# leggedrobotics/G-VOM

Hardware: AMD Instinct MI355X
Metric: M points/sec (process_pointcloud + combine_maps, 256^3 voxel grid); map Hz beside it (higher is better)
Workload: dtype int32 atomics + f32 ray state + f64 compares/maps; 1 GPU; 256x256x256 @0.2 m (metric grid), OS1-64 131,072-pt scan, buffer=1; buffer_size=1, poses=8, pose_motion=0.2 m per scan in +x (the window shifts every scan), input=device-resident f32 xyz, step=1 scan + 1 combine incl. the 4 maps in host memory, timing=2668 steps timed as one block after 5 warm-up steps

## Files before the change

### g-vom_amd/csrc/gvom_capi.hip

```cpp
#include "gvom_internal.h"
#include "gvom_ingest.h"
#include "../../include/gvom_hip.h"

#include <math.h>
#include <stdio.h>
#include <stdlib.h>
#include <string.h>
#include <time.h>
#include <unistd.h>
#include <immintrin.h>
#include <algorithm>
#include <atomic>
#include <mutex>
#include <string>
#include <vector>

#define VIS __attribute__((visibility("default")))

namespace {

struct Buf {
    void *p = nullptr;
    size_t bytes = 0;
    uint64_t gen = 0;
};

struct Slot {
    int32_t *state = nullptr;
    uint16_t *code16 = nullptr;
    uint32_t *tags = nullptr;
    uint32_t epoch = 0;
    Buf crows;
    Buf metrics, base, rowvox;
    int64_t origin[3] = {0, 0, 0};
    int64_t count = 0;
    bool filled = false;
    bool has_code16 = false;
    bool has_metrics = false;
    bool stats_valid = false;
    gvom_scan_stats stats = {0, 0, 0, 0};
};

struct Fused {
    int32_t *state = nullptr;
    uint32_t *tags = nullptr;
    uint32_t epoch = 0;
    Buf rows;
    Buf metrics;
    int64_t origin[3] = {0, 0, 0};
    int64_t count = 0;
    bool valid = false;
    bool has_metrics = false;
};

struct DevSet {
    char *mem = nullptr;
    size_t bytes = 0;
    int device = 0, xy = 0;
    int kind = 0, zs = 0;
    int64_t cap = 0;
    hipEvent_t ready = nullptr;
    int64_t id = -1;
    int exports = 0;
    std::vector<hipStream_t> rel_streams;
    std::vector<hipEvent_t> rel, rel_spare;
    bool orphan = false;
};
#define GVOM_MAX_DEVICE_SETS 8
#define GVOM_N_PRODUCT_KINDS 4
std::mutex g_set_mu;

struct DLDevice { int32_t device_type; int32_t device_id; };
struct DLDataType { uint8_t code; uint8_t bits; uint16_t lanes; };
struct DLTensor { void *data; DLDevice device; int32_t ndim; DLDataType dtype; int64_t *shape; int64_t *strides; uint64_t byte_offset; };
struct DLManagedTensor { DLTensor dl_tensor; void *manager_ctx; void (*deleter)(DLManagedTensor *); };
struct DLPackVersion { uint32_t major; uint32_t minor; };
struct DLManagedTensorVersioned { DLPackVersion version; void *manager_ctx; void (*deleter)(DLManagedTensorVersioned *); uint64_t flags; DLTensor dl_tensor; };
enum { kDLInt = 0, kDLUInt = 1, kDLFloat = 2, kDLROCM = 10 };

}

struct gvom_handle {
    gvom_params prm;
    int device = 0;
    int rank = 0, world = 1;
    bool sharded = false;
    int sy_lo = 0, sy_hi = 0;
    size_t V = 0, slabV = 0, cells2d = 0, ntiles = 0;
    int nseg = 1;
    uint32_t epoch = 0;
    hipStream_t stream = nullptr;
    std::mutex mu;
    std::mutex scan_mu;
    std::string err;

    uint32_t *hit = nullptr, *total = nullptr, *mh = nullptr;
    size_t acc_elems = 0;
    int tune_segs = 0, tune_ep_row = -2, tune_period = 0;
    int tune_prio = -1;
    int tune_ilv = 0;
    int last_knobs[5] = {0, 0, 0, 0, 1};
    int64_t last_n = -1;
    uint32_t probe_var_age = 0;
    int64_t probe_n = -1; uint32_t probe_age = 0;
    int tune_fuse1 = 0;
    int tune_flag_kernel = 0;
    int tune_churn = 0;
    uint64_t alloc_gen = 0;
    uint64_t handle_gen = 0;
    bool exported = false;
    bool holds_pooled = false;
    std::vector<Buf> retired;
    uint64_t fixed_gen[3] = {0, 0, 0};
    uint32_t *x_send_ids = nullptr, *x_recv_ids = nullptr;
    void *x_send_pay = nullptr, *x_recv_pay = nullptr;
    Buf x_send_eps, x_recv_eps;
    int64_t x_ep_cap = 0;
    std::vector<int64_t> x_recv_ep_off;
    uint32_t *x_qcnt = nullptr, *x_ecnt = nullptr, *x_spcnt = nullptr;
    unsigned long long *x_host = nullptr, *x_host_dev = nullptr;
    Buf x_send_sp, x_recv_sp;
    std::vector<int64_t> x_recv_sp_off;
    int pending_dtype = 0;
    size_t x_Q = 0, x_myQ = 0;
    ScanParams pending_P;
    unsigned resident_blocks = 2048;
    bool f32_sqrt = false;
    std::vector<Slot> slots;
    std::vector<int> ring;
    int staging = 0;
    int buffer_index = 0, last_buffer_index = 0;
    Buf in_pts, world_pts[2];
    uint32_t *counters = nullptr;
    uint32_t *counters_host = nullptr;
    uint32_t *counters_host_dev = nullptr;

    bool pending = false;
    bool pending_any = false;
    int64_t pending_origin[3] = {0, 0, 0};
    int64_t pending_n = 0;

    Fused fused[2];
    int cur = 0;
    bool has_combined = false;
    int64_t combined_cell_count = 0;
    MapDesc *descs_dev = nullptr, *descs_host = nullptr;
    uint32_t *blockcounts = nullptr;
    int fuse_blocks = 0;
    int cnt_blocks = 0;
    double *hmaps2 = nullptr;
    uint32_t *blockcounts2 = nullptr;
    bool spec_valid = false;
    int spec_nxt = 0, spec_slot = 0, spec_blocks = 0;
    uint32_t spec_epoch = 0;
    int64_t spec_origin[3] = {0, 0, 0};
    bool spec_has_metrics = false;
    Buf flink[2];
    bool fs_reads[2] = {false, false};
    FuseParams spec_FP;
    FuseDescs spec_KD;
    int tune_dirsort = 0;
    Buf dir_keys, dir_perm;
    uint32_t *dir_hist = nullptr;
    uint32_t dir_flip = 0;
    int last_dirsort = 0;
    int tune_encfuse = 0;
    int tune_fastdiv = -1;
    int fastdiv_ok = 0;
    int tune_eager = -1;
    int eager_waste = 0;
    int eager_stat[2] = {0, 0};
    int last_fuse = 0;
    bool last_scan_spec = false;
    bool solo_encoded = false;
    bool fresh_scan = false;

    double *hmaps = nullptr;
    double *height = nullptr, *inferred = nullptr;
    int hs = 0;
    double *slope_x = nullptr, *slope_y = nullptr, *rough = nullptr, *guessed = nullptr;
    hipStream_t own_stream = nullptr;
    hipStream_t stream_b = nullptr;
    hipStream_t stream_up = nullptr;
    hipEvent_t ev_up = nullptr;
    hipStream_t stream_s = nullptr;
    hipEvent_t ev_enc_s = nullptr, ev_fz_s = nullptr, ev_sdone = nullptr, ev_fsdone = nullptr;
    hipEvent_t ev_before[2] = {nullptr, nullptr};
    bool before_valid[2] = {false, false};
    uint32_t stats_scan = 0;
    bool stats_prev_committed = true;
    bool s_pending = false, fs_pending = false;
    hipEvent_t ev_fused = nullptr, ev_mapped = nullptr, ev_done = nullptr;
    std::mutex combine_mu;
    bool pending_combine = false;
    uint32_t combine_seq = 0;
    double last_wait_ns[2] = {0.0, 0.0};
    bool mapped_unjoined = false;
    hipEvent_t ev_fuse_b = nullptr;
    bool fuse_b_unjoined = false;
    uint64_t fuse_b_slots = 0;
    bool scan_inflight = false;
    std::vector<void *> out_bufs;
    void *last_checked_out = nullptr;
    void *out_host = nullptr;
    char *out_host_dev = nullptr;
    uint32_t scan_seq = 0;
    bool ev_scan = false, ev_fuse = false, ev_map = false;
    bool maps_valid = false;

    double ego[3] = {0, 0, 0};
    int in_off[3] = {0, 1, 2};
    bool in_f32 = false;

    Buf tl;
    int tl_grid[2] = {0, 0};
    double host_ns[8] = {0, 0, 0, 0, 0, 0, 0, 0};
    long host_calls = 0;
    bool host_timing = false;
    bool stats = false;
    bool stats_auto = false;
    int stats_idle = 0;
    bool stats_release = false;
    int acc_pad = 7, sxq = 0;
    bool profiling = false;
    hipEvent_t ev[8] = {nullptr};
    float stage_ms[GVOM_N_STAGES] = {0, 0, 0, 0, 0};
    std::vector<DevSet *> dsets;
    int64_t dset_seq = 0;
    std::vector<DevSet *> psets;
    int64_t pset_seq = 0;
    int tune_occ_clear = 0;
    bool count_pending = false;
    hipEvent_t ev_dcount = nullptr;
    Buf ri_model, ri_raw, ri_poses;
    void *ri_poses_pin = nullptr;
    size_t ri_poses_pin_bytes = 0;
    int32_t ri_H = 0, ri_W = 0;
    double ri_scale = 0.0, ri_min = 0.0, ri_max = 0.0;
};

namespace {

inline double now_ns() { timespec t; clock_gettime(CLOCK_MONOTONIC, &t); return t.tv_sec * 1e9 + t.tv_nsec; }
#define HT(h, slot, t0) do { if ((h)->host_timing) { double n_ = now_ns(); (h)->host_ns[slot] += n_ - (t0); (t0) = n_; } } while (0)

#define HIPCHK(h, call)                                                                         \
    do {                                                                                        \
        hipError_t e_ = (call);                                                                 \
        if (e_ != hipSuccess) {                                                                 \
            char b_[512];                                                                       \
            snprintf(b_, sizeof b_, "%s failed: %s (%s:%d)", #call, hipGetErrorString(e_),      \
                     __FILE__, __LINE__);                                                       \
            (h)->err = b_;                                                                      \
            return GVOM_ERR_HIP;                                                                \
        }                                                                                       \
    } while (0)

static std::atomic<uint64_t> g_alloc_generation{0};

inline size_t exportable_size(size_t bytes) { const size_t g = (size_t)2 << 20; return ((bytes ? bytes : 1) + g - 1) / g * g; }

#define GVOM_POOL_WARN_BYTES ((size_t)16 << 30)
struct ExportPool {
    std::mutex m;
    std::vector<Buf> v;
    size_t bytes = 0;
    bool warned = false;
};
static ExportPool g_pool;
void pool_put(void *p, size_t bytes, uint64_t gen)
{
    if (!p) return;
    std::lock_guard<std::mutex> lk(g_pool.m);
    Buf b; b.p = p; b.bytes = bytes; b.gen = gen;
    g_pool.v.push_back(b);
    g_pool.bytes += bytes;
    if (g_pool.bytes > GVOM_POOL_WARN_BYTES && !g_pool.warned) {
        g_pool.warned = true;
        fprintf(stderr, "libgvom_hip: %zu MiB of device memory that other processes may have mapped are parked (never freed while "
                        "the process lives; re-used by later sharded handles of the same sizes): create fewer exported handles per process\n",
                g_pool.bytes >> 20);
    }
}
hipError_t pool_get(size_t bytes, void **p, uint64_t *gen, bool *reused = nullptr)
{
    {
        std::lock_guard<std::mutex> lk(g_pool.m);
        for (size_t k = 0; k < g_pool.v.size(); ++k)
            if (g_pool.v[k].bytes == bytes) {
                *p = g_pool.v[k].p; *gen = g_pool.v[k].gen;
                if (reused) *reused = true;
                g_pool.bytes -= bytes;
                g_pool.v.erase(g_pool.v.begin() + (long)k);
                return hipSuccess;
            }
    }
    *gen = ++g_alloc_generation;
    return hipMalloc(p, bytes);
}

int ensure(gvom_handle *h, Buf &b, size_t bytes)
{
    if (b.bytes >= bytes) return GVOM_OK;
    size_t want = bytes + bytes / 2 + 256;
    const bool exported = &b == &h->x_send_eps || &b == &h->x_send_sp;
    if (exported) want = exportable_size(want);
    if (b.p && exported) { h->retired.push_back(b); b.p = nullptr; }
    if (b.p) HIPCHK(h, hipFree(b.p));
    b.p = nullptr; b.bytes = 0;
    if (exported) HIPCHK(h, pool_get(want, &b.p, &b.gen, &h->holds_pooled));
    else { HIPCHK(h, hipMalloc(&b.p, want)); b.gen = ++g_alloc_generation; }
    b.bytes = want;
    if (&b == &h->x_send_eps || &b == &h->x_send_sp) h->alloc_gen = b.gen;
    return GVOM_OK;
}

int ensure_keep(gvom_handle *h, Buf &b, size_t bytes)
{
    if (b.bytes >= bytes) return GVOM_OK;
    const size_t want = bytes + bytes / 2 + 256;
    void *np = nullptr;
// ... 43 lines not shown
    P.sy_lo = h->sy_lo; P.sy_hi = h->sy_hi;
    P.off[0] = h->in_off[0]; P.off[1] = h->in_off[1]; P.off[2] = h->in_off[2];
    P.in_f32 = h->in_f32 ? 1 : 0;
    P.nseg = h->nseg;
    {
        auto lg = [](int v) { int k = 0; while ((1 << k) < v) ++k; return (1 << k) == v ? k : -1; };
        P.lg_nseg = lg(h->nseg); P.lg_zs = lg(p.z_size);
        if (P.lg_nseg < 0 || P.lg_zs < 0) P.lg_nseg = P.lg_zs = -1;
    }
    P.sxq = h->sxq;
    P.shard_world = h->world; P.shard_rank = h->rank; P.shard_rows = h->world > 1 ? p.xy_size / h->world : p.xy_size;
    P.stat_e = p.xy_eigen_dist;
    {
        const int maxsteps = (p.xy_size > p.z_size ? p.xy_size : p.z_size) / 2 + 2;
        const bool many = n_points / 64 > 3 * (int64_t)h->resident_blocks;
        int nsegs = many ? 3 : 5;
        if (h->tune_segs > 0) nsegs = h->tune_segs;
        if (nsegs > 9) nsegs = 9;
        if (nsegs > maxsteps / 8) nsegs = maxsteps / 8 > 0 ? maxsteps / 8 : 1;
        P.nsegs = nsegs;
        P.lc_period = h->tune_period > 0 ? h->tune_period : (many ? 12 : 16);
        if (P.lc_period > 32) P.lc_period = 32;
        P.ep_row = h->tune_ep_row >= -1 ? h->tune_ep_row : (many ? -1 : 0);
        if (P.ep_row > P.nsegs) P.ep_row = P.nsegs;
        P.prio_div = h->tune_prio >= 0 ? h->tune_prio : 8;
        P.f32_sqrt = h->f32_sqrt ? 1 : 0;
        P.ilv_lg = 0; P.ilv_len = n_points;
        {
            int K = h->tune_ilv > 1 ? h->tune_ilv : 1;
            if (h->tune_ilv == 0 && h->counters_host) {
                const unsigned long long w = *(volatile unsigned long long *)(h->counters_host + 8);
                if ((int64_t)(w >> 8) == n_points) K = 1 << (int)(w & 7ull);
            }
            if (K > 64 || (K & (K - 1)) != 0 || n_points <= 0 || n_points % K != 0) K = 1;
            while ((1 << P.ilv_lg) < K) ++P.ilv_lg;
            P.ilv_len = n_points / K;
            if (K > 1 && h->tune_period <= 0) P.lc_period = 24;
        }
        P.dbg = gvom_diag_env("GVOM_TRACE_DEBUG");
        const double w_last = nsegs <= 3 ? 0.35 : 0.6;
        const double unit = nsegs >= 3 ? (double)maxsteps / ((nsegs - 2) + 0.85 + w_last) : (double)maxsteps / nsegs;
        double acc = 0.0;
        for (int k = 0; k < 10; ++k) {
            P.seg_start[k] = (int)(acc + 0.5);
            acc += (nsegs < 3 || k < nsegs - 2) ? unit : (k == nsegs - 2 ? 0.85 * unit : (k == nsegs - 1 ? w_last * unit : unit));
        }
    }
    P.epoch = 0;
}

__attribute__((target("fma"))) static bool verify_fastdiv_all(double d, double r)
{
    for (uint32_t m = 0; m < (1u << 23); ++m) {
        const uint32_t bits = 0x3f800000u | m;
        float xf;
        memcpy(&xf, &bits, 4);
        const double x = (double)xf;
        const double q = x * r;
        const double e = __builtin_fma(-q, d, x);
        const double q2 = __builtin_fma(e, r, q);
        if (q2 != x / d) return false;
    }
    return true;
}
static bool verify_fastdiv(double d)
{
    static std::mutex mu;
    static std::vector<std::pair<double, bool>> known;
    if (!(d > 0x1p-64 && d < 0x1p64)) return false;
    if (!__builtin_cpu_supports("fma")) return false;
    std::lock_guard<std::mutex> lk(mu);
    for (const auto &k : known) if (k.first == d) return k.second;
    const bool ok = verify_fastdiv_all(d, 1.0 / d);
    known.emplace_back(d, ok);
    return ok;
}

int create_impl(const gvom_params *params, int device_id, int rank, int world, bool sharded, gvom_t **out)
{
    if (!params || !out) return GVOM_ERR_INVALID;
    *out = nullptr;
    if (params->xy_size <= 0 || params->z_size <= 0 || params->buffer_size <= 0 ||
        !(params->xy_resolution > 0) || !(params->z_resolution > 0) || world <= 0 || rank < 0 ||
        rank >= world)
        return GVOM_ERR_INVALID;
    if (params->buffer_size >= GVOM_MAX_SLOTS || params->z_size > 1024 || world > GVOM_MAX_SLOTS) return GVOM_ERR_CAPACITY;
    if (sharded && params->xy_size % (4 * world) != 0) return GVOM_ERR_INVALID;
    const double Vd = (double)params->xy_size * params->xy_size * params->z_size;
    if (Vd >= 2147483648.0) return GVOM_ERR_CAPACITY;
    int ndev = 0;
    if (hipGetDeviceCount(&ndev) != hipSuccess || ndev <= 0 || device_id < 0 || device_id >= ndev)
        return GVOM_ERR_NO_DEVICE;
    gvom_handle *h = new gvom_handle();
    h->alloc_gen = h->handle_gen = ++g_alloc_generation;
    h->prm = *params;
    h->device = device_id;
    h->rank = rank; h->world = world; h->sharded = sharded;
    h->stats = (params->reserved0 & GVOM_FLAG_VOXEL_STATISTICS) != 0;
    h->stats_auto = !h->stats && !sharded && (params->reserved0 & GVOM_FLAG_STATISTICS_ON_DEMAND) != 0;
    if (h->stats_auto) h->stats = true;
    h->f32_sqrt = (params->reserved0 & GVOM_FLAG_CUDA_F32_SQRT) != 0;
    h->fastdiv_ok = (verify_fastdiv(params->xy_resolution) ? 1 : 0) | (verify_fastdiv(params->z_resolution) ? 2 : 0);
    if (const char *v = getenv("GVOM_VOXEL_STATISTICS")) { h->stats = atoi(v) != 0; h->stats_auto = false; }
    if (sharded && h->stats && world > 1 && 2 * params->xy_eigen_dist + 1 > params->xy_size / world) { delete h; return GVOM_ERR_INVALID; }
    if (const char *v = getenv("GVOM_HOST_TIMING")) h->host_timing = atoi(v) != 0;
    const int xy = params->xy_size, zs = params->z_size;
    h->sy_lo = (int)((int64_t)xy * rank / world);
    h->sy_hi = (int)((int64_t)xy * (rank + 1) / world);
    h->V = (size_t)xy * xy * zs;
    h->slabV = (size_t)(h->sy_hi - h->sy_lo) * xy * zs;
    h->cells2d = (size_t)xy * xy;
    h->nseg = (xy + 63) / 64;
    h->ntiles = (size_t)xy * zs * h->nseg;
#define CK(call)                                                                                \
    do {                                                                                        \
        hipError_t e_ = (call);                                                                 \
        if (e_ != hipSuccess) {                                                                 \
            fprintf(stderr, "gvom_create: %s failed: %s\n", #call, hipGetErrorString(e_));      \
            gvom_destroy(h);                                                                    \
            return GVOM_ERR_HIP;                                                                \
        }                                                                                       \
    } while (0)
    CK(hipSetDevice(device_id));
    CK(hipStreamCreateWithFlags(&h->stream, hipStreamNonBlocking));
    h->own_stream = h->stream;
    {
        int lo = 0, hi = 0;
        CK(hipDeviceGetStreamPriorityRange(&lo, &hi));
        CK(hipStreamCreateWithPriority(&h->stream_b, hipStreamNonBlocking, hi));
    }
    CK(hipEventCreateWithFlags(&h->ev_fused, hipEventDisableTiming));
    CK(hipEventCreateWithFlags(&h->ev_mapped, hipEventDisableTiming));
    CK(hipEventCreateWithFlags(&h->ev_done, hipEventDisableTiming));
    CK(hipEventCreateWithFlags(&h->ev_fuse_b, hipEventDisableTiming));
    CK(hipStreamCreateWithFlags(&h->stream_up, hipStreamNonBlocking));
    CK(hipStreamCreateWithFlags(&h->stream_s, hipStreamNonBlocking));
    for (hipEvent_t *e : {&h->ev_enc_s, &h->ev_fz_s, &h->ev_sdone, &h->ev_fsdone, &h->ev_before[0], &h->ev_before[1]})
        CK(hipEventCreateWithFlags(e, hipEventDisableTiming));
    CK(hipEventCreateWithFlags(&h->ev_up, hipEventDisableTiming));
    h->sxq = (xy + 3) / 4 + h->acc_pad;
    const size_t acc_elems = (size_t)h->sxq * ((xy + 3) / 4) * zs * 16 + 256;
    h->acc_elems = acc_elems;
    CK(hipMalloc((void **)&h->hit, acc_elems * 4));
    CK(hipMalloc((void **)&h->total, acc_elems * 4));
    CK(hipMalloc((void **)&h->mh, acc_elems * 4));
    CK(hipMemsetAsync(h->hit, 0, acc_elems * 4, h->stream));
    CK(hipMemsetAsync(h->total, 0, acc_elems * 4, h->stream));
    CK(hipMemsetAsync(h->mh, 0, acc_elems * 4, h->stream));
    {
        hipDeviceProp_t pr;
        CK(hipGetDeviceProperties(&pr, device_id));
        h->resident_blocks = (unsigned)pr.multiProcessorCount * 8u;
    }
    h->slots.resize(params->buffer_size + 1);
    for (auto &s : h->slots) {
        CK(hipMalloc((void **)&s.state, h->V * 4));
        if ((params->xy_size & 3) == 0) CK(hipMalloc((void **)&s.code16, h->V * 2));
        CK(hipMalloc((void **)&s.tags, h->ntiles * 4));
        CK(hipMemsetAsync(s.tags, 0, h->ntiles * 4, h->stream));
    }
    h->ring.resize(params->buffer_size);
    for (int i = 0; i < params->buffer_size; ++i) h->ring[i] = i;
    h->staging = params->buffer_size;
    for (int k = 0; k < 2; ++k) {
        CK(hipMalloc((void **)&h->fused[k].state, h->V * 4));
        CK(hipMalloc((void **)&h->fused[k].tags, h->ntiles * 4));
        CK(hipMemsetAsync(h->fused[k].tags, 0, h->ntiles * 4, h->stream));
    }
    CK(hipMalloc((void **)&h->dir_hist, 3 * GVOM_DIRBINS * 4));
    CK(hipMemsetAsync(h->dir_hist, 0, 3 * GVOM_DIRBINS * 4, h->stream));
    CK(hipMalloc((void **)&h->counters, GVOM_CNT_WORDS * 4));
    CK(hipHostMalloc((void **)&h->counters_host, 64, hipHostMallocMapped | hipHostMallocCoherent));
    CK(hipHostGetDevicePointer((void **)&h->counters_host_dev, h->counters_host, 0));
    memset(h->counters_host, 0, 64);
    CK(hipMemsetAsync(h->counters, 0, GVOM_CNT_WORDS * 4, h->stream));
    CK(hipMalloc((void **)&h->descs_dev, sizeof(MapDesc) * (GVOM_MAX_SLOTS + 1)));
    CK(hipHostMalloc((void **)&h->descs_host, sizeof(MapDesc) * (GVOM_MAX_SLOTS + 1)));
    h->fuse_blocks = ((xy + 63) / 64) * (h->sy_hi - h->sy_lo);
    CK(hipMalloc((void **)&h->blockcounts, (size_t)(h->fuse_blocks > 0 ? h->fuse_blocks : 1) * 4));
    CK(hipMemsetAsync(h->blockcounts, 0, (size_t)(h->fuse_blocks > 0 ? h->fuse_blocks : 1) * 4, h->stream));
    h->cnt_blocks = h->fuse_blocks;
    if (!sharded && params->buffer_size == 1 && xy % 16 == 0 && zs >= 4) {
        CK(hipMalloc((void **)&h->blockcounts2, (size_t)(h->fuse_blocks > 0 ? h->fuse_blocks : 1) * 4));
        CK(hipMemsetAsync(h->blockcounts2, 0, (size_t)(h->fuse_blocks > 0 ? h->fuse_blocks : 1) * 4, h->stream));
        CK(hipMalloc((void **)&h->hmaps2, h->cells2d * 24));
    }
    h->hs = 3 * xy;
    if (sharded) CK(pool_get(exportable_size(h->cells2d * 24), (void **)&h->hmaps, &h->fixed_gen[2], &h->holds_pooled));
    else CK(hipMalloc((void **)&h->hmaps, h->cells2d * 24));
    h->height = h->hmaps; h->inferred = h->hmaps + xy;
    double **maps[4] = {&h->slope_x, &h->slope_y, &h->rough, &h->guessed};
    for (auto m : maps) CK(hipMalloc((void **)m, h->cells2d * 8));

    CK(hipHostMalloc(&h->out_host, h->cells2d * 20, hipHostMallocMapped | hipHostMallocCoherent));
    CK(hipHostGetDevicePointer((void **)&h->out_host_dev, h->out_host, 0));
    if (sharded) {
        h->x_Q = (size_t)(xy / 4) * zs * h->nseg;
        h->x_myQ = h->x_Q / world;
        CK(pool_get(exportable_size(h->x_Q * 4), (void **)&h->x_send_ids, &h->fixed_gen[0], &h->holds_pooled));
        CK(pool_get(exportable_size(h->x_Q * 1024), &h->x_send_pay, &h->fixed_gen[1], &h->holds_pooled));
        CK(hipMalloc((void **)&h->x_recv_ids, h->x_Q * 4));
        CK(hipMalloc(&h->x_recv_pay, h->x_Q * 1024));
        CK(hipMalloc((void **)&h->x_qcnt, (size_t)world * 64));
        CK(hipMalloc((void **)&h->x_ecnt, (size_t)world * 64));
        CK(hipMalloc((void **)&h->x_spcnt, (size_t)world * 64));
        CK(hipMemsetAsync(h->x_qcnt, 0, (size_t)world * 64, h->stream));
        CK(hipMemsetAsync(h->x_ecnt, 0, (size_t)world * 64, h->stream));
        CK(hipMemsetAsync(h->x_spcnt, 0, (size_t)world * 64, h->stream));
        CK(hipHostMalloc((void **)&h->x_host, (size_t)(3 * world + 2) * 8, hipHostMallocMapped | hipHostMallocCoherent));
        CK(hipHostGetDevicePointer((void **)&h->x_host_dev, h->x_host, 0));
        memset(h->x_host, 0, (size_t)(3 * world + 2) * 8);
        h->x_recv_ep_off.assign(world + 1, 0);
        h->x_recv_sp_off.assign(world + 1, 0);
    }
    for (auto &e : h->ev) CK(hipEventCreate(&e));
    CK(hipStreamSynchronize(h->stream));
#undef CK
    *out = h;
    return GVOM_OK;
}

static void stats_demand(gvom_handle *h)
{
    h->stats_idle = 0;
    if (h->stats_auto && !h->stats) { h->stats = true; h->stats_release = false; }
}

static void release_statistics_buffers(gvom_handle *h)
{
    h->stats_release = false;
    (void)hipStreamSynchronize(h->stream_s);
    h->s_pending = h->fs_pending = false;
    h->before_valid[0] = h->before_valid[1] = false;
    auto fb = [](Buf &b) { if (b.p) (void)hipFree(b.p); b.p = nullptr; b.bytes = 0; };
    for (auto &sl : h->slots) { fb(sl.metrics); fb(sl.base); fb(sl.rowvox); sl.has_metrics = false; }
    for (int k = 0; k < 2; ++k) { fb(h->fused[k].metrics); h->fused[k].has_metrics = false; }
    fb(h->world_pts[0]); fb(h->world_pts[1]); fb(h->flink[0]); fb(h->flink[1]);
    h->spec_has_metrics = false;
}

void scan_abort(gvom_handle *h)
{
    (void)hipMemsetAsync(h->hit, 0, h->acc_elems * 4, h->stream);
    (void)hipMemsetAsync(h->total, 0, h->acc_elems * 4, h->stream);
    (void)hipMemsetAsync(h->mh, 0, h->acc_elems * 4, h->stream);
    (void)hipMemsetAsync(h->counters, 0, GVOM_CNT_WORDS * 4, h->stream);
    if (h->stream_s) (void)hipStreamSynchronize(h->stream_s);
    h->s_pending = h->fs_pending = false;
    h->before_valid[0] = h->before_valid[1] = false;
    (void)hipStreamSynchronize(h->stream);
    (void)hipGetLastError();
    h->pending = false;
    h->scan_inflight = false;
}

int renumber_epochs(gvom_handle *h);

hipError_t sync_streams(gvom_handle *h)
{
    if (h->mapped_unjoined || h->fuse_b_unjoined) {
        hipError_t e = hipStreamSynchronize(h->stream_b);
        if (e != hipSuccess) return e;
        h->mapped_unjoined = false;
        h->fuse_b_unjoined = false;
    }
    if (h->s_pending || h->fs_pending) {
        hipError_t e = hipStreamSynchronize(h->stream_s);
        if (e != hipSuccess) return e;
        h->s_pending = h->fs_pending = false;
        h->before_valid[0] = h->before_valid[1] = false;
    }
    return hipStreamSynchronize(h->stream);
}
hipError_t join_fuse_stream(gvom_handle *h)
{
    if (!h->fuse_b_unjoined) return hipSuccess;
    h->fuse_b_unjoined = false;
    return hipStreamWaitEvent(h->stream, h->ev_fuse_b, 0);
}
hipError_t join_map_stream(gvom_handle *h)
{
    if (!h->mapped_unjoined) return hipSuccess;
    h->mapped_unjoined = false;
    h->fuse_b_unjoined = false;
    return hipStreamWaitEvent(h->stream, h->ev_mapped, 0);
}

hipError_t join_second_stream(gvom_handle *h)
{
    hipError_t e = join_map_stream(h);
    if (e == hipSuccess) e = join_fuse_stream(h);
    if (e == hipSuccess && h->s_pending) e = hipStreamWaitEvent(h->stream, h->ev_sdone, 0);
    return e;
}

int enqueue_scan_stats(gvom_handle *h, const ScanParams &P, int dtype, Slot &st, int64_t n, int64_t nrows, const void *extra, int64_t n_extra)
{
    const uint32_t par = h->stats_scan & 1u;
    HIPCHK(h, hipEventRecord(h->ev_before[par], h->stream_s));
    h->before_valid[par] = true;
    ++h->stats_scan;
    HIPCHK(h, hipEventRecord(h->ev_enc_s, h->stream));
    HIPCHK(h, hipStreamWaitEvent(h->stream_s, h->ev_enc_s, 0));
    HIPCHK(h, gvom_launch_stats(h->stream_s, P, dtype, h->world_pts[par].p, n, st.state, st.tags,
                                h->prm.xy_eigen_dist, h->prm.z_eigen_dist, (double *)st.base.p, (double *)st.metrics.p,
                                (const uint32_t *)st.rowvox.p, nrows, extra, n_extra));
    HIPCHK(h, hipEventRecord(h->ev_sdone, h->stream_s));
    h->s_pending = true;
    return GVOM_OK;
}

bool wait_published(gvom_handle *h, std::unique_lock<std::mutex> &lk, volatile unsigned long long *flag, uint32_t seq,
                    bool high_half, double *last_ns)
{
    auto done = [&]() { return (uint32_t)(high_half ? (*flag >> 32) : *flag) == seq; };
    lk.unlock();
    const double start = now_ns();
    bool slept = false;
    if (last_ns && *last_ns > 6.0e5 && !done()) {
        const double margin = *last_ns * 0.2 > 2.5e5 ? *last_ns * 0.2 : 2.5e5;
        usleep((useconds_t)((*last_ns - margin) * 1e-3));
        slept = true;
    }
    const bool overslept = slept && done();
    unsigned spins = 0;
    bool ok = true;
    while (!done()) {
        _mm_pause();
        if ((++spins & 0x3ff) == 0) {
            const double waited = now_ns() - start;
            if (waited > 2.0e9) { ok = false; break; }
            if (waited > 2.0e7) usleep(50);
        }
    }
    if (last_ns) {
        const double est = overslept ? *last_ns * 0.5 : now_ns() - start;
        *last_ns = est < 2.0e7 ? est : 2.0e7;
    }
    lk.lock();
    return ok;
}

void fill_fuse_frame(const gvom_handle *h, const int64_t origin[3], FuseParams &P)
{
    const gvom_params &p = h->prm;
    memset(&P, 0, sizeof P);
    P.xy = p.xy_size; P.zs = p.z_size;
    P.om[0] = (int)floor_mod(origin[0], p.xy_size);
    P.om[1] = (int)floor_mod(origin[1], p.xy_size);
    P.om[2] = (int)floor_mod(origin[2], p.z_size);
    P.sy_lo = h->sy_lo; P.sy_hi = h->sy_hi;
    P.nseg = h->nseg;
    P.hs = h->hs;
    for (int k = 0; k < 3; ++k) { P.origin[k] = (double)origin[k]; P.ego[k] = h->ego[k]; }
    P.xy_res = p.xy_resolution; P.z_res = p.z_resolution;
    P.radius2 = p.robot_radius * p.robot_radius;
    P.ground_to_lidar_height = p.ground_to_lidar_height;
}

int eager_launch(gvom_handle *h, const ScanParams &P, Slot &st, const int64_t origin[3], uint32_t seq)
{
    const gvom_params &p = h->prm;
    const int nxt = h->has_combined ? 1 - h->cur : 0;
    Fused &F = h->fused[nxt];
    const Fused *prev = (h->has_combined && h->fused[h->cur].valid) ? &h->fused[h->cur] : nullptr;
    FuseParams FP;
    fill_fuse_frame(h, origin, FP);
    FP.nslots = 1; FP.has_prev = prev ? 1 : 0;
    FP.nz = h->tune_encfuse & 15; FP.cpw = (h->tune_encfuse >> 4) & 1;
    MapDesc pd;
    memset(&pd, 0, sizeof pd);
    if (prev) {
        pd.state = prev->state; pd.rows = (const uint4 *)prev->rows.p;
        pd.d[0] = clamp_delta(origin[0] - prev->origin[0], p.xy_size);
        pd.d[1] = clamp_delta(origin[1] - prev->origin[1], p.xy_size);
        pd.d[2] = clamp_delta(origin[2] - prev->origin[2], p.z_size);
        pd.epoch = prev->epoch; pd.tags = prev->tags;
    }
    int nw, nblocks; size_t row_cap;
    gvom_encfuse_shape(p.xy_size, p.z_size, FP.nz, &nw, &nblocks, &row_cap);
    if (row_cap >= 2147483648ull) { h->err = "fused row space exceeds 31 bits"; return GVOM_ERR_CAPACITY; }
    int rc;
    if ((rc = ensure(h, F.rows, row_cap * 16))) return rc;
    F.valid = false;
    FP.epoch = ++h->epoch;
    if (h->fs_pending && h->fs_reads[nxt]) HIPCHK(h, hipStreamWaitEvent(h->stream, h->ev_fsdone, 0));
    h->spec_has_metrics = false;
    int32_t *flink = nullptr;
    if (h->stats) {
        if ((rc = ensure(h, h->flink[nxt], row_cap * 4))) return rc;
        flink = (int32_t *)h->flink[nxt].p;
        if ((rc = ensure(h, F.metrics, row_cap * 40))) return rc;
        h->spec_FP = FP;
        memset(&h->spec_KD, 0, sizeof h->spec_KD);
        MapDesc &sd = h->spec_KD.d[0];
        sd.state = st.state; sd.rows = (const uint4 *)st.crows.p; sd.epoch = st.epoch; sd.tags = st.tags; sd.metrics = st.metrics.p;
        if (prev) { h->spec_KD.d[1] = pd; h->spec_KD.d[1].metrics = prev->has_metrics ? prev->metrics.p : nullptr; h->spec_KD.d[1].link = flink; }
        h->spec_has_metrics = true;
    }
    HIPCHK(h, gvom_launch_encfuse(h->stream, P, FP, pd, flink, h->hit, h->total, h->mh, st.state, (uint4 *)st.crows.p, st.tags,
                                  F.state, (uint4 *)F.rows.p, F.tags, h->blockcounts2, h->hmaps2, h->hmaps2 + p.xy_size,
                                  h->counters, (unsigned long long *)h->counters_host_dev, seq));
    h->spec_valid = true; h->spec_nxt = nxt; h->spec_slot = h->staging; h->spec_blocks = nblocks; h->spec_epoch = FP.epoch;
    h->spec_origin[0] = origin[0]; h->spec_origin[1] = origin[1]; h->spec_origin[2] = origin[2];
    h->last_scan_spec = true;
    return GVOM_OK;
}

int scan_launch(gvom_handle *h, std::unique_lock<std::mutex> &lk, const void *dev_pts, int64_t n, int64_t stride_elems,
                int dtype, const double *tf, bool shard_local = false)
{
    const gvom_params &p = h->prm;
    int64_t origin[3];
    origin[0] = (int64_t)floor((h->ego[0] / p.xy_resolution) - p.xy_size / 2.0);
    origin[1] = (int64_t)floor((h->ego[1] / p.xy_resolution) - p.xy_size / 2.0);
    origin[2] = (int64_t)floor((h->ego[2] / p.z_resolution) - p.z_size / 2.0);
    int rc;
    if (h->epoch >= 0xFFFFFF00u && (rc = renumber_epochs(h))) return rc;
    ScanParams P;
    fill_scan_params(h, origin, tf, P, n);
    if (h->pending_combine && h->tune_prio < 0) P.prio_div = 0;
    h->last_knobs[0] = P.nsegs; h->last_knobs[1] = P.lc_period; h->last_knobs[2] = P.ep_row; h->last_knobs[3] = P.prio_div;
    h->last_knobs[4] = 1 << P.ilv_lg;
    Slot &st = h->slots[h->staging];
    if (h->fuse_b_unjoined && ((h->fuse_b_slots >> h->staging) & 1ull)) HIPCHK(h, join_fuse_stream(h));
    st.epoch = ++h->epoch;
    P.epoch = st.epoch;
    st.has_metrics = h->stats;
    h->scan_inflight = true;
    const size_t esz = dtype == GVOM_DTYPE_F32 ? 4 : 8;
    const size_t cap = std::max<size_t>(1, (size_t)n);
    if ((rc = ensure(h, st.crows, cap * 16))) return rc;
    Buf &wpts = h->world_pts[h->stats_scan & 1u];
    const size_t scap = h->sharded ? 2 * cap : cap;
    if (h->stats && ((rc = ensure(h, wpts, (size_t)(n > 0 ? n : 1) * 3 * esz)) || (rc = ensure(h, st.metrics, scap * 80)) ||
                     (rc = ensure(h, st.base, scap * 8 * GVOM_BASE_PITCH)) || (rc = ensure(h, st.rowvox, scap * 4)))) return rc;
    double t0 = now_ns();
    const uint32_t seq = ++h->scan_seq;
    if (h->profiling) HIPCHK(h, hipEventRecord(h->ev[0], h->stream));
    bool big = false;
    for (int k = 0; k < 3; ++k)
        if (origin[k] >= (1ll << 30) || origin[k] <= -(1ll << 30)) big = true;
    if (h->stats) {
        const uint32_t prev_par = (h->stats_scan + 1u) & 1u;
        if (!h->stats_prev_committed && h->s_pending) HIPCHK(h, hipStreamWaitEvent(h->stream, h->ev_sdone, 0));
        else if (h->before_valid[prev_par]) {
            if (hipEventQuery(h->ev_before[prev_par]) == hipSuccess) h->before_valid[prev_par] = false;
            else { (void)hipGetLastError(); HIPCHK(h, hipStreamWaitEvent(h->stream, h->ev_before[prev_par], 0)); }
        }
        HIPCHK(h, hipMemsetAsync(st.rowvox.p, 0xFF, st.rowvox.bytes, h->stream));
    }
    ShardExchange X;
    X.ep_send = nullptr; X.ep_cnt = nullptr; X.ep_cap = 0; X.sp_send = nullptr; X.sp_cnt = nullptr;
    if (h->sharded) {
#ifdef GVOM_HOOKS
        if (h->tune_churn > 0 && h->x_send_eps.p) {
            h->retired.push_back(h->x_send_eps);
            h->x_send_eps.p = nullptr; h->x_send_eps.bytes = 0;
        }
#endif
        if ((rc = ensure(h, h->x_send_eps, (size_t)h->world * (size_t)(n > 0 ? n : 1) * 8))) return rc;
        h->x_ep_cap = n > 0 ? n : 1;
        X.ep_send = (uint2 *)h->x_send_eps.p; X.ep_cnt = h->x_ecnt; X.ep_cap = (long)h->x_ep_cap;
        if (h->stats && h->world > 1) {
            if ((rc = ensure(h, h->x_send_sp, (size_t)h->world * (size_t)h->x_ep_cap * 3 * esz))) return rc;
            X.sp_send = h->x_send_sp.p; X.sp_cnt = h->x_spcnt;
        }
    }
    P.tl = nullptr; P.tl_words = 0;
#ifdef GVOM_DIAG
    if (gvom_diag_env("GVOM_TRACE_TIMELINE") && n > 0) {
        h->tl_grid[0] = (int)((n + 511) / 512); h->tl_grid[1] = P.nsegs + (P.ep_row >= 0 ? 1 : 0);
        P.prof_on = gvom_diag_env("GVOM_TRACE_STEPPROF");
        const size_t bytes = (size_t)h->tl_grid[0] * h->tl_grid[1] * 8 * 32 + 64 + ((size_t)h->tl_grid[0] * h->tl_grid[1] * 8 / 64 + 1) * 1024;
        P.tl_words = (long)h->tl_grid[0] * h->tl_grid[1] * 8 * 4;
        if ((rc = ensure(h, h->tl, bytes))) return rc;
        HIPCHK(h, hipMemsetAsync(h->tl.p, 0, bytes, h->stream));
        P.tl = (unsigned long long *)h->tl.p;
    }
#endif
    hipError_t le = hipSuccess;
    const unsigned long long probe_word = h->counters_host ? *(volatile unsigned long long *)(h->counters_host + 8) : 0ull;
    if (h->tune_ilv == 0 && n >= 8192) {
        const bool stable = n == h->last_n && (n != h->probe_n || ++h->probe_age >= 32);
        const bool varying = n != h->last_n && ++h->probe_var_age >= 8;
        if (stable || varying) {
            if (stable) { h->probe_n = n; h->probe_age = 0; }
            h->probe_var_age = 0;
            le = gvom_launch_layout_probe(h->stream, P, dtype, dev_pts, stride_elems, n, 2, (unsigned long long *)(h->counters_host_dev + 8));
            if (le != hipSuccess) { scan_abort(h); HIPCHK(h, le); }
        }
        h->last_n = n;
    }
    P.perm = nullptr;
    {
        int sort = h->tune_dirsort == 1 || h->tune_dirsort == 2 ? h->tune_dirsort : 0;
        if (h->tune_dirsort == 0 && h->tune_ilv == 0 && h->counters_host) {
            const unsigned long long w = probe_word;
            const int64_t np_ = (int64_t)(w >> 8);
            if (np_ > 0 && (np_ == n || (n > np_ - np_ / 4 && n < np_ + np_ / 4))) sort = (int)((w >> 3) & 3ull);
        }
        h->last_dirsort = 0;
        if (sort && n >= 256 && n < (1ll << 31)) {
            if ((rc = ensure(h, h->dir_keys, (size_t)n * 2)) || (rc = ensure(h, h->dir_perm, (size_t)n * 4))) return rc;
            uint32_t *hist = h->dir_hist + (h->dir_flip & 1u) * GVOM_DIRBINS, *next = h->dir_hist + ((h->dir_flip + 1u) & 1u) * GVOM_DIRBINS;
            ++h->dir_flip;
            le = gvom_launch_dirbin(h->stream, P, sort == 2 ? 2 : 1, dtype, dev_pts, stride_elems, n, (uint16_t *)h->dir_keys.p, hist, next,
                                    h->dir_hist + 2 * GVOM_DIRBINS, (uint32_t *)h->dir_perm.p);
            if (le != hipSuccess) { scan_abort(h); HIPCHK(h, le); }
            P.perm = (const uint32_t *)h->dir_perm.p;
            P.ilv_lg = 0; P.ilv_len = n;
            h->last_dirsort = sort == 2 ? 2 : 1;
            h->last_knobs[4] = 1;
        }
    }
    le = gvom_launch_trace(h->stream, P, X, dtype, big, dev_pts, stride_elems, n,
                                      h->stats ? wpts.p : nullptr, h->hit, h->total, h->mh, st.state,
                                      st.tags, h->counters, h->stats ? (double *)st.metrics.p : nullptr,
                                      h->stats ? (double *)st.base.p : nullptr,
                                      h->stats ? (uint32_t *)st.rowvox.p : nullptr);
    if (le != hipSuccess) { scan_abort(h); HIPCHK(h, le); }
    if (h->profiling) HIPCHK(h, hipEventRecord(h->ev[1], h->stream));
    const bool solo = shard_local && h->world == 1;
    h->solo_encoded = solo;
    if (shard_local && !solo) {
        le = gvom_launch_pack(h->stream, P, h->total, st.tags, h->x_send_ids, h->x_send_pay, h->x_qcnt, h->x_ecnt, h->x_spcnt,
                              h->counters, h->x_host_dev, seq);
        if (le != hipSuccess) { scan_abort(h); HIPCHK(h, le); }
        volatile unsigned long long *flag = (volatile unsigned long long *)(h->x_host + 2 * h->world + 1);
        if (!wait_published(h, lk, flag, seq, false, &h->last_wait_ns[0])) {
            hipError_t se = hipStreamSynchronize(h->stream);
            if (se != hipSuccess || (uint32_t)*flag != seq) {
                scan_abort(h);
                h->err = "sharded scan: pack counts were never published";
                return GVOM_ERR_HIP;
            }
        }
        h->pending_any = h->x_host[2 * h->world] != 0;
        h->pending_P = P;
        h->pending_dtype = dtype;
        st.count = -1;
        st.origin[0] = origin[0]; st.origin[1] = origin[1]; st.origin[2] = origin[2];
        st.stats_valid = false;
        st.stats.points = n;
        h->pending = true;
        h->pending_n = n;
        return GVOM_OK;
    }
    const bool eager = h->hmaps2 && h->tune_eager != 0 && (h->tune_eager == 1 || h->eager_waste < 3) && !gvom_diag_env("GVOM_TRACE_DEBUG");
    h->last_scan_spec = false;
    if (eager) {
        if ((rc = eager_launch(h, P, st, origin, seq))) { scan_abort(h); return rc; }
        st.has_code16 = false;
    } else {
        const bool codes = st.code16 && (p.buffer_size > 1 || h->tune_fuse1 == 1 || h->sharded);
        le = gvom_launch_encode(h->stream, P, h->hit, h->total, h->mh, st.state, codes ? st.code16 : nullptr, (uint4 *)st.crows.p,
                                st.tags, h->counters,
                                (unsigned long long *)h->counters_host_dev, seq, h->resident_blocks);
        if (le != hipSuccess) { scan_abort(h); HIPCHK(h, le); }
        st.has_code16 = codes;
    }
    if (h->profiling) { HIPCHK(h, hipEventRecord(h->ev[2], h->stream)); h->ev_scan = true; }
    if (h->stats && (rc = enqueue_scan_stats(h, P, dtype, st, n, n, nullptr, 0))) return rc;
    if (eager && h->spec_has_metrics) {
        Fused &F = h->fused[h->spec_nxt];
        HIPCHK(h, gvom_launch_fuse_stats(h->stream_s, h->spec_FP, h->spec_KD, nullptr, F.state, F.tags, (float *)F.metrics.p));
        HIPCHK(h, hipEventRecord(h->ev_fsdone, h->stream_s));
        HIPCHK(h, hipEventRecord(h->ev_sdone, h->stream_s));
        h->s_pending = h->fs_pending = true;
        h->fs_reads[h->spec_nxt] = true; h->fs_reads[1 - h->spec_nxt] = false;
    }
    HT(h, 0, t0);
    {
        volatile unsigned long long *flag = (volatile unsigned long long *)h->counters_host;
        if (!wait_published(h, lk, flag, seq, true, &h->last_wait_ns[0])) {
            hipError_t se = hipStreamSynchronize(h->stream);
            if (se != hipSuccess || (uint32_t)(*flag >> 32) != seq) {
                scan_abort(h);
                h->err = se != hipSuccess ? std::string("scan failed: ") + hipGetErrorString(se)
                                          : "scan completion was never published";
                return GVOM_ERR_HIP;
            }
        }
    }
    HT(h, 1, t0);
    if (h->host_timing) h->host_calls++;
    {
        const unsigned long long fl = *(volatile unsigned long long *)h->counters_host;
        h->pending_any = (fl & 0x80000000ull) != 0;
    }
    st.count = -1;
    st.origin[0] = origin[0]; st.origin[1] = origin[1]; st.origin[2] = origin[2];
    st.stats_valid = false;
    st.stats.points = n;
    h->pending = true;
    h->pending_n = n;
    return GVOM_OK;
}

void scan_commit(gvom_handle *h, bool accept)
{
    h->scan_inflight = false;
    if (!h->pending) return;
    h->pending = false;
    h->stats_prev_committed = accept;
    if (!accept) { h->spec_valid = false; h->last_scan_spec = false; return; }
    const int b = h->buffer_index;
    const int old = h->ring[b];
    h->ring[b] = h->staging;
    h->staging = old;
    h->slots[h->ring[b]].filled = true;
    h->fresh_scan = true;
    h->slots[old].filled = false;
    h->last_buffer_index = b;
    h->buffer_index = (b + 1 >= h->prm.buffer_size) ? 0 : b + 1;
}

int renumber_epochs(gvom_handle *h)
{
    HIPCHK(h, sync_streams(h));
    h->spec_valid = false;
    uint32_t next = 0;
    for (size_t k = 0; k < h->slots.size(); ++k) {
        Slot &sl = h->slots[k];
        const bool inflight = (int)k == h->staging && (h->scan_inflight || h->pending);
        const uint32_t fresh = (sl.filled || inflight) ? ++next : 0u;
        HIPCHK(h, gvom_launch_retag(h->stream, sl.tags, h->ntiles, sl.epoch, fresh));
        sl.epoch = fresh;
        if (inflight) h->pending_P.epoch = fresh;
    }
    for (int k = 0; k < 2; ++k) {
        Fused &f = h->fused[k];
        const uint32_t fresh = f.valid ? ++next : 0u;
        HIPCHK(h, gvom_launch_retag(h->stream, f.tags, h->ntiles, f.epoch, fresh));
        f.epoch = fresh;
    }
    h->epoch = next;
    HIPCHK(h, sync_streams(h));
    return GVOM_OK;
}

int scan_begin(gvom_handle *h, const double ego[3], const int64_t *off_bytes, size_t esz, bool widen_f32, bool defer, int64_t n)
{
    HIPCHK(h, hipSetDevice(h->device));
    for (int k = 0; k < 3; ++k) h->in_off[k] = off_bytes ? (int)(off_bytes[k] / (int64_t)esz) : k;
    h->in_f32 = widen_f32;
    h->ego[0] = ego[0]; h->ego[1] = ego[1]; h->ego[2] = ego[2];
    if (h->pending && h->sharded) scan_abort(h);
    h->pending = false;
    if (h->spec_valid) {
        h->spec_valid = false;
        if (h->eager_waste < 4) ++h->eager_waste;
        ++h->eager_stat[1];
    }
    if (h->sharded && !defer) { h->err = "a sharded handle scans through gvom_shard_scan_local / gvom_shard_scan_merge"; return GVOM_ERR_INVALID; }
    if (n == 0 && !defer) return GVOM_EMPTY_CLOUD;
    return GVOM_OK;
}

struct Upload { void *dst; const void *src; size_t bytes; };
int scan_upload(gvom_handle *h, std::unique_lock<std::mutex> &lk, const Upload *up, int count)
{
    if (hipStreamQuery(h->stream) == hipErrorNotReady) {
        lk.unlock();
        hipError_t ue = hipSuccess;
        for (int k = 0; k < count && ue == hipSuccess; ++k)
            ue = hipMemcpyAsync(up[k].dst, up[k].src, up[k].bytes, hipMemcpyHostToDevice, h->stream_up);
        lk.lock();
        HIPCHK(h, ue);
        HIPCHK(h, hipEventRecord(h->ev_up, h->stream_up));
        HIPCHK(h, hipStreamWaitEvent(h->stream, h->ev_up, 0));
    } else {
        (void)hipGetLastError();
        for (int k = 0; k < count; ++k)
            HIPCHK(h, hipMemcpyAsync(up[k].dst, up[k].src, up[k].bytes, hipMemcpyHostToDevice, h->stream));
    }
    return GVOM_OK;
}

int scan_finish(gvom_handle *h, std::unique_lock<std::mutex> &lk, const void *dev, int64_t n, int64_t stride_elems, int dtype,
                const double *tf, bool defer)
{
    int rc = scan_launch(h, lk, dev, n, stride_elems, dtype, tf, defer);
    if (rc) return rc;
    if (defer) return GVOM_OK;
    const bool accept = h->pending_any;
    scan_commit(h, accept);
    return accept ? GVOM_OK : GVOM_NO_OVERLAP;
}

int process_impl(gvom_handle *h, const void *xyz, bool on_device, int64_t n, int64_t row_stride_bytes,
                 int dtype, const double ego[3], const double *tf, bool defer, const int64_t *off_bytes = nullptr,
                 bool widen_f32 = false)
{
    if (!h || !ego || n < 0 || (dtype != GVOM_DTYPE_F32 && dtype != GVOM_DTYPE_F64))
        return GVOM_ERR_INVALID;
    const size_t esz = (dtype == GVOM_DTYPE_F32 || widen_f32) ? 4 : 8;
    if (widen_f32 && dtype != GVOM_DTYPE_F64) return GVOM_ERR_INVALID;
    if (n > 0 && (!xyz || row_stride_bytes < (int64_t)(3 * esz) || row_stride_bytes % esz != 0))
        return GVOM_ERR_INVALID;
    if (n >= 2147483647LL) return GVOM_ERR_CAPACITY;
    int64_t last_field = 2 * (int64_t)esz;
    if (off_bytes) {
        last_field = 0;
        for (int k = 0; k < 3; ++k) {
            if (off_bytes[k] < 0 || off_bytes[k] % (int64_t)esz != 0 || off_bytes[k] + (int64_t)esz > row_stride_bytes)
                return GVOM_ERR_INVALID;
            if (off_bytes[k] > last_field) last_field = off_bytes[k];
        }
    }
    std::lock_guard<std::mutex> scan_lk(h->scan_mu);
    std::unique_lock<std::mutex> lk(h->mu);
    int rc = scan_begin(h, ego, off_bytes, esz, widen_f32, defer, n);
    if (rc) return rc;
    const void *dev = xyz;
    if (!on_device && n > 0) {
        if ((rc = ensure(h, h->in_pts, (size_t)n * row_stride_bytes))) return rc;
        const Upload up = {h->in_pts.p, xyz, (size_t)(n - 1) * row_stride_bytes + (size_t)last_field + esz};
        if ((rc = scan_upload(h, lk, &up, 1))) return rc;
        dev = h->in_pts.p;
    }
    return scan_finish(h, lk, dev, n, row_stride_bytes / (int64_t)esz, dtype, tf, defer);
}

int range_image_impl(gvom_handle *h, const void *raw, bool on_device, int range_dtype, int64_t row_stride_bytes,
                     const double *col_poses, int cloud_dtype, const double ego[3], const double *tf)
{
    if (!h || !ego || !raw || (cloud_dtype != GVOM_DTYPE_F32 && cloud_dtype != GVOM_DTYPE_F64)) return GVOM_ERR_INVALID;
    if (range_dtype != GVOM_RANGE_U16 && range_dtype != GVOM_RANGE_U32 && range_dtype != GVOM_RANGE_F32) return GVOM_ERR_INVALID;
    const int64_t rsz = range_dtype == GVOM_RANGE_U16 ? 2 : 4;
    std::lock_guard<std::mutex> scan_lk(h->scan_mu);
    std::unique_lock<std::mutex> lk(h->mu);
    if (h->sharded) { h->err = "range images are not supported on a sharded handle"; return GVOM_ERR_INVALID; }
    if (h->ri_H <= 0) { h->err = "gvom_process_range_image: no sensor model (gvom_sensor_model_set)"; return GVOM_ERR_INVALID; }
    const int64_t H = h->ri_H, W = h->ri_W, n = H * W;
    if (row_stride_bytes < W * rsz || row_stride_bytes % rsz != 0) { h->err = "gvom_process_range_image: bad row stride"; return GVOM_ERR_INVALID; }
    int rc = scan_begin(h, ego, nullptr, 0, false, false, n);
    if (rc) return rc;
    const size_t tsz = cloud_dtype == GVOM_DTYPE_F32 ? 4 : 8;
    if ((rc = ensure(h, h->in_pts, (size_t)n * 3 * tsz))) return rc;
    Upload up[2];
    int ups = 0;
    if (col_poses) {
        const size_t bytes = (size_t)W * 96;
        if ((rc = ensure(h, h->ri_poses, bytes))) return rc;
        if (h->ri_poses_pin_bytes < bytes) {
            if (h->ri_poses_pin) HIPCHK(h, hipHostFree(h->ri_poses_pin));
            h->ri_poses_pin = nullptr; h->ri_poses_pin_bytes = 0;
            HIPCHK(h, hipHostMalloc(&h->ri_poses_pin, bytes + bytes / 2, hipHostMallocDefault));
            h->ri_poses_pin_bytes = bytes + bytes / 2;
        }
        memcpy(h->ri_poses_pin, col_poses, bytes);
        up[ups++] = {h->ri_poses.p, h->ri_poses_pin, bytes};
    }
    if (!on_device) {
        const size_t bytes = (size_t)(H - 1) * row_stride_bytes + (size_t)(W * rsz);
        if ((rc = ensure(h, h->ri_raw, bytes))) return rc;
        up[ups++] = {h->ri_raw.p, raw, bytes};
    }
    if (ups && (rc = scan_upload(h, lk, up, ups))) return rc;
    UnprojectParams U;
    U.raw = on_device ? raw : h->ri_raw.p; U.row_stride = row_stride_bytes;
    U.dir = (const double *)h->ri_model.p; U.off = U.dir + (size_t)n * 3;
    U.poses = col_poses ? (const double *)h->ri_poses.p : nullptr;
    U.out = h->in_pts.p;
    U.scale = h->ri_scale; U.min_range = h->ri_min; U.max_range = h->ri_max;
    U.W = (uint32_t)W; U.n = (uint32_t)n;
    HIPCHK(h, gvom_launch_unproject(h->stream, U, range_dtype, cloud_dtype));
    return scan_finish(h, lk, h->in_pts.p, n, 3, cloud_dtype, tf, false);
}

int choose_nz(int zs, int *zc, int *cpw)
{
    int nchunks = (zs + 15) / 16;
    if (nchunks < 1) nchunks = 1;
    if (nchunks > 16) nchunks = 16;
    *zc = (zs + nchunks - 1) / nchunks;
    nchunks = (zs + *zc - 1) / *zc;
    int want_waves = 4;
    *cpw = (nchunks + want_waves - 1) / want_waves;
// ... 153 lines not shown
    const size_t n2 = h->cells2d;
    int32_t *o_pos = (int32_t *)out_dev, *o_neg = o_pos + n2, *o_vis = o_neg + n2;
    double *o_rgh = (double *)(o_vis + n2);
    if (dev_set) {
        const size_t S = dev_map_stride(p.xy_size);
        P.out_dev = 1;
        o_rgh = (double *)out_dev;
        o_pos = (int32_t *)(o_rgh + 6 * S); o_neg = o_pos + S; o_vis = o_neg + S;
    }
    if (h->profiling) HIPCHK(h, hipEventRecord(h->ev[6], ms));
    HIPCHK(h, gvom_launch_map2d(ms, P, F.state, F.tags, (const uint4 *)F.rows.p,
                                h->height, h->inferred, h->slope_x,
                                h->slope_y, h->rough, h->guessed, o_pos, o_neg, o_rgh, o_vis,
                                h->blockcounts, h->cnt_blocks,
                                publish ? (unsigned long long *)(h->counters_host_dev + 2) : nullptr));
    if (h->profiling) { HIPCHK(h, hipEventRecord(h->ev[7], ms)); h->ev_map = true; }
    h->maps_valid = true;
    return GVOM_OK;
}

int posdens_impl(gvom_handle *h)
{
    const gvom_params &p = h->prm;
    const Fused &F = h->fused[h->cur];
    Map2dParams P;
    memset(&P, 0, sizeof P);
    P.xy = p.xy_size; P.zs = p.z_size;
    P.om[2] = (int)floor_mod(F.origin[2], p.z_size);
    P.y_lo = h->sy_lo; P.y_hi = h->sy_hi;
    P.origin_z = (double)F.origin[2];
    P.z_res = p.z_resolution;
    P.pos_thr = p.positive_obstacle_threshold; P.robot_height = p.robot_height;
    P.nseg = h->nseg; P.hs = h->hs; P.epoch = F.epoch;
    HIPCHK(h, gvom_launch_posdens(h->stream, P, F.state, F.tags, (const uint4 *)F.rows.p,
                                  h->hmaps, h->blockcounts, h->fuse_blocks,
                                  (unsigned long long *)(h->counters_host_dev + 2),
                                  (unsigned long long *)(h->counters + 10)));
    return GVOM_OK;
}

void collect_stage_ms(gvom_handle *h)
{
    if (h->ev_scan) {
        hipEventElapsedTime(&h->stage_ms[0], h->ev[0], h->ev[1]);
        hipEventElapsedTime(&h->stage_ms[1], h->ev[1], h->ev[2]);
        h->stage_ms[2] = 0.0f;
    }
    if (h->ev_fuse) hipEventElapsedTime(&h->stage_ms[3], h->ev[4], h->ev[5]);
    if (h->ev_map && hipEventSynchronize(h->ev[7]) == hipSuccess) hipEventElapsedTime(&h->stage_ms[4], h->ev[6], h->ev[7]);
    h->ev_scan = h->ev_fuse = h->ev_map = false;
    (void)hipGetLastError();
}

int finish_combine(gvom_handle *h, std::unique_lock<std::mutex> &lk, uint32_t seq)
{
    if (h->tune_flag_kernel) HIPCHK(h, gvom_launch_publish_seq(h->stream, (unsigned long long *)(h->counters_host_dev + 4), seq));
    HIPCHK(h, hipEventRecord(h->ev_done, h->stream));
    h->pending_combine = true;
    hipError_t e = hipSuccess;
    if (!wait_published(h, lk, (volatile unsigned long long *)(h->counters_host + 4), seq, false, &h->last_wait_ns[1])) {
        lk.unlock();
        e = hipEventSynchronize(h->ev_done);
        lk.lock();
    }
    h->pending_combine = false;
    HIPCHK(h, e);
    Fused &F = h->fused[h->cur];
    unsigned long long c;
    memcpy(&c, h->counters_host + 2, 8);
    F.count = (int64_t)c;
    h->combined_cell_count = F.count;
    h->count_pending = false;
    collect_stage_ms(h);
    return GVOM_OK;
}

int finish_combine(gvom_handle *h)
{
    HIPCHK(h, sync_streams(h));
    Fused &F = h->fused[h->cur];
    unsigned long long c;
    memcpy(&c, h->counters_host + 2, 8);
    F.count = (int64_t)c;
    h->combined_cell_count = F.count;
    h->count_pending = false;
    collect_stage_ms(h);
    return GVOM_OK;
}

int settle_count(gvom_handle *h)
{
    if (!h->count_pending) return GVOM_OK;
    HIPCHK(h, hipSetDevice(h->device));
    HIPCHK(h, hipEventSynchronize(h->ev_dcount));
    h->count_pending = false;
    Fused &F = h->fused[h->cur];
    unsigned long long c;
    memcpy(&c, h->counters_host + 2, 8);
    F.count = (int64_t)c;
    h->combined_cell_count = F.count;
    return GVOM_OK;
}

void set_free(DevSet *s)
{
    int dev = 0;
    hipGetDevice(&dev);
    hipSetDevice(s->device);
    for (hipEvent_t e : s->rel) { hipEventSynchronize(e); hipEventDestroy(e); }
    for (hipEvent_t e : s->rel_spare) hipEventDestroy(e);
    if (s->ready) { hipEventSynchronize(s->ready); hipEventDestroy(s->ready); }
    if (s->mem) hipFree(s->mem);
    hipSetDevice(dev);
    (void)hipGetLastError();
    delete s;
}

}

extern "C" {

VIS int gvom_create(const gvom_params *params, int device_id, gvom_t **out)
{
    return create_impl(params, device_id, 0, 1, false, out);
}

VIS int gvom_create_sharded(const gvom_params *params, int device_id, int rank, int world, gvom_t **out)
{
    return create_impl(params, device_id, rank, world, true, out);
}

VIS void gvom_destroy(gvom_t *h)
{
    if (!h) return;
    hipSetDevice(h->device);
    if (h->stream_b) hipStreamSynchronize(h->stream_b);
    if (h->stream) hipStreamSynchronize(h->stream);
    auto fb = [](Buf &b) { if (b.p) hipFree(b.p); b.p = nullptr; b.bytes = 0; };
    hipFree(h->hit); hipFree(h->total); hipFree(h->mh);
    auto park = [&](void *ptr, size_t bytes, uint64_t gen) {
        if (!ptr) return;
        if (h->exported || h->holds_pooled) pool_put(ptr, bytes, gen); else hipFree(ptr);
    };
    for (Buf &r : h->retired) park(r.p, r.bytes, r.gen);
    if (h->sharded) {
        park(h->x_send_ids, exportable_size(h->x_Q * 4), h->fixed_gen[0]); park(h->x_send_pay, exportable_size(h->x_Q * 1024), h->fixed_gen[1]);
        park(h->x_send_eps.p, h->x_send_eps.bytes, h->x_send_eps.gen); park(h->x_send_sp.p, h->x_send_sp.bytes, h->x_send_sp.gen);
        park(h->hmaps, exportable_size(h->cells2d * 24), h->fixed_gen[2]); h->hmaps = nullptr;
    }
    h->x_send_eps.p = nullptr; h->x_send_sp.p = nullptr;
    hipFree(h->x_recv_ids); hipFree(h->x_recv_pay);
    hipFree(h->x_qcnt); hipFree(h->x_ecnt); hipFree(h->x_spcnt); fb(h->x_recv_eps); fb(h->x_recv_sp);
    if (h->x_host) hipHostFree(h->x_host);
    for (auto &s : h->slots) { hipFree(s.state); hipFree(s.code16); hipFree(s.tags); fb(s.crows); fb(s.metrics); fb(s.base); fb(s.rowvox); }
    for (auto &f : h->fused) { hipFree(f.state); hipFree(f.tags); fb(f.rows); fb(f.metrics); }
    fb(h->in_pts); fb(h->ri_model); fb(h->ri_raw); fb(h->ri_poses); if (h->ri_poses_pin) hipHostFree(h->ri_poses_pin); fb(h->world_pts[0]); fb(h->world_pts[1]); fb(h->flink[0]); fb(h->flink[1]); fb(h->tl); fb(h->dir_keys); fb(h->dir_perm); hipFree(h->dir_hist);
    hipFree(h->counters); if (h->counters_host) hipHostFree(h->counters_host);
    hipFree(h->descs_dev); if (h->descs_host) hipHostFree(h->descs_host);
    hipFree(h->blockcounts); hipFree(h->blockcounts2); hipFree(h->hmaps2);
    hipFree(h->hmaps); hipFree(h->slope_x); hipFree(h->slope_y);
    hipFree(h->rough); hipFree(h->guessed);
    if (h->out_host) hipHostFree(h->out_host);
    {
        std::vector<DevSet *> idle;
        {
            std::lock_guard<std::mutex> g(g_set_mu);
            for (std::vector<DevSet *> *v : {&h->dsets, &h->psets})
                for (DevSet *s : *v) { if (s->exports > 0) s->orphan = true; else idle.push_back(s); }
        }
        for (DevSet *s : idle) set_free(s);
        h->dsets.clear(); h->psets.clear();
        if (h->ev_dcount) hipEventDestroy(h->ev_dcount);
    }
    for (auto &e : h->ev) if (e) hipEventDestroy(e);
    if (h->ev_fused) hipEventDestroy(h->ev_fused);
    if (h->ev_mapped) hipEventDestroy(h->ev_mapped);
    if (h->ev_done) hipEventDestroy(h->ev_done);
    if (h->ev_fuse_b) hipEventDestroy(h->ev_fuse_b);
    if (h->ev_up) hipEventDestroy(h->ev_up);
    if (h->stream_up) { hipStreamSynchronize(h->stream_up); hipStreamDestroy(h->stream_up); }
    if (h->stream_s) { hipStreamSynchronize(h->stream_s); hipStreamDestroy(h->stream_s); }
    for (hipEvent_t e : {h->ev_enc_s, h->ev_fz_s, h->ev_sdone, h->ev_fsdone, h->ev_before[0], h->ev_before[1]}) if (e) hipEventDestroy(e);
    if (h->stream_b) hipStreamDestroy(h->stream_b);
    if (h->own_stream) hipStreamDestroy(h->own_stream);
    delete h;
}

VIS int gvom_process_pointcloud(gvom_t *h, const void *xyz, int64_t n, int64_t row_stride_bytes,
                                int dtype, const double ego[3], const double *transform_4x4)
{
    return process_impl(h, xyz, false, n, row_stride_bytes, dtype, ego, transform_4x4, false);
}

VIS int gvom_process_pointcloud_device(gvom_t *h, const void *xyz_dev, int64_t n,
                                       int64_t row_stride_bytes, int dtype, const double ego[3],
                                       const double *transform_4x4)
{
    return process_impl(h, xyz_dev, true, n, row_stride_bytes, dtype, ego, transform_4x4, false);
}

VIS int gvom_process_pointcloud2(gvom_t *h, const void *data, int64_t n_points, int64_t point_step,
                                 int64_t off_x, int64_t off_y, int64_t off_z, int dtype,
                                 const double ego[3], const double *transform_4x4)
{
    const int64_t off[3] = {off_x, off_y, off_z};
    return process_impl(h, data, false, n_points, point_step, GVOM_DTYPE_F64, ego, transform_4x4, false, off,
                        dtype == GVOM_DTYPE_F32);
}

VIS int gvom_sensor_model_set(gvom_t *h, int32_t H, int32_t W, const double *dir, const double *off,
                              double range_scale, double min_range, double max_range)
{
    if (!h || H < 1 || W < 1 || (int64_t)H * W >= (1ll << 31) || !dir) return GVOM_ERR_INVALID;
    if (!(range_scale > 0.0) || !std::isfinite(range_scale) || std::isnan(min_range) || std::isnan(max_range)) return GVOM_ERR_INVALID;
    std::lock_guard<std::mutex> scan_lk(h->scan_mu);
    std::unique_lock<std::mutex> lk(h->mu);
    HIPCHK(h, hipSetDevice(h->device));
    HIPCHK(h, hipStreamSynchronize(h->stream));
    const size_t half = (size_t)H * W * 24;
    h->ri_H = h->ri_W = 0;
    int rc = ensure(h, h->ri_model, 2 * half);
    if (rc) return rc;
    char *m = (char *)h->ri_model.p;
    HIPCHK(h, hipMemcpyAsync(m, dir, half, hipMemcpyHostToDevice, h->stream));
    if (off) HIPCHK(h, hipMemcpyAsync(m + half, off, half, hipMemcpyHostToDevice, h->stream));
    else HIPCHK(h, hipMemsetAsync(m + half, 0, half, h->stream));
    HIPCHK(h, hipStreamSynchronize(h->stream));
    h->ri_H = H; h->ri_W = W;
    h->ri_scale = range_scale; h->ri_min = min_range; h->ri_max = max_range;
    return GVOM_OK;
}

VIS int gvom_process_range_image(gvom_t *h, const void *raw, int on_device, int range_dtype, int64_t row_stride_bytes,
                                 const double *col_poses, int cloud_dtype, const double ego[3], const double *transform_4x4)
{
    return range_image_impl(h, raw, on_device != 0, range_dtype, row_stride_bytes, col_poses, cloud_dtype, ego, transform_4x4);
}

VIS int gvom_shard_scan_local(gvom_t *h, const void *xyz, int on_device, int64_t n, int64_t row_stride_bytes,
                              int dtype, const double ego[3], const double *transform_4x4,
                              int64_t *send_quads, int64_t *send_eps, int *any_ingrid)
{
    if (!h || !h->sharded) return GVOM_ERR_INVALID;
    int rc = process_impl(h, xyz, on_device != 0, n, row_stride_bytes, dtype, ego, transform_4x4, true);
    if (rc) return rc;
    std::lock_guard<std::mutex> lk(h->mu);
    for (int d = 0; d < h->world; ++d) {
        if (send_quads) send_quads[d] = h->solo_encoded ? 0 : (int64_t)h->x_host[d];
        if (send_eps) send_eps[d] = h->solo_encoded ? 0 : (int64_t)h->x_host[h->world + d];
    }
    if (any_ingrid) *any_ingrid = h->pending_any ? 1 : 0;
    return GVOM_OK;
}

VIS int gvom_shard_recv_reserve(gvom_t *h, const int64_t *recv_eps)
{
    if (!h || !h->sharded || !recv_eps) return GVOM_ERR_INVALID;
    std::lock_guard<std::mutex> lk(h->mu);
    HIPCHK(h, hipSetDevice(h->device));
    int64_t tot = 0;
    for (int sidx = 0; sidx < h->world; ++sidx) {
        h->x_recv_ep_off[sidx] = tot;
        if (recv_eps[sidx] < 0) return GVOM_ERR_INVALID;
        tot += sidx == h->rank ? 0 : recv_eps[sidx];
    }
    h->x_recv_ep_off[h->world] = tot;
    return ensure(h, h->x_recv_eps, (size_t)(tot > 0 ? tot : 1) * 8);
}

VIS int gvom_shard_stats_counts(gvom_t *h, int64_t *send_returns)
{
    if (!h || !h->sharded || !send_returns) return GVOM_ERR_INVALID;
    std::lock_guard<std::mutex> lk(h->mu);
    for (int d = 0; d < h->world; ++d) send_returns[d] = (h->stats && h->pending && !h->solo_encoded) ? (int64_t)h->x_host[2 * h->world + 2 + d] : 0;
    return GVOM_OK;
}

VIS int gvom_shard_stats_reserve(gvom_t *h, const int64_t *recv_returns, int dtype)
{
    if (!h || !h->sharded || !recv_returns || (dtype != GVOM_DTYPE_F32 && dtype != GVOM_DTYPE_F64)) return GVOM_ERR_INVALID;
    std::lock_guard<std::mutex> lk(h->mu);
    HIPCHK(h, hipSetDevice(h->device));
    if (h->pending_n > 0 && dtype != h->pending_dtype) { h->err = "the ranks' clouds differ in type"; return GVOM_ERR_INVALID; }
    h->pending_dtype = dtype;
    int64_t tot = 0;
    for (int sidx = 0; sidx < h->world; ++sidx) {
        h->x_recv_sp_off[sidx] = tot;
        if (recv_returns[sidx] < 0) return GVOM_ERR_INVALID;
        tot += sidx == h->rank ? 0 : recv_returns[sidx];
    }
    h->x_recv_sp_off[h->world] = tot;
    const size_t esz3 = (h->pending_dtype == GVOM_DTYPE_F32 ? 4 : 8) * 3;
    return ensure(h, h->x_recv_sp, (size_t)(tot > 0 ? tot : 1) * esz3);
}

VIS int gvom_shard_buffer(gvom_t *h, int which, int peer, void **ptr, int64_t *capacity_bytes)
{
    if (!h || !h->sharded || !ptr || peer < 0 || peer >= h->world) return GVOM_ERR_INVALID;
    std::lock_guard<std::mutex> lk(h->mu);
    const size_t myQ = h->x_myQ;
    int64_t cap = 0;
    switch (which) {
    case GVOM_XBUF_SEND_IDS: *ptr = h->x_send_ids + (size_t)peer * myQ; cap = (int64_t)myQ * 4; break;
    case GVOM_XBUF_SEND_QUADS: *ptr = (char *)h->x_send_pay + (size_t)peer * myQ * 1024; cap = (int64_t)myQ * 1024; break;
    case GVOM_XBUF_SEND_EPS: *ptr = (char *)h->x_send_eps.p + (size_t)peer * (size_t)h->x_ep_cap * 8; cap = h->x_ep_cap * 8; break;
    case GVOM_XBUF_RECV_IDS: *ptr = h->x_recv_ids + (size_t)peer * myQ; cap = (int64_t)myQ * 4; break;
    case GVOM_XBUF_RECV_QUADS: *ptr = (char *)h->x_recv_pay + (size_t)peer * myQ * 1024; cap = (int64_t)myQ * 1024; break;
// ... 942 lines not shown
    if (!h->has_combined) return GVOM_NO_DATA;
    HIPCHK(h, hipSetDevice(h->device));
    const Fused &F = h->fused[h->cur];
    OccParams P;
    occ_params(h, F, P);
    uint8_t *tmp = nullptr;
    HIPCHK(h, hipMalloc((void **)&tmp, h->V));
    hipError_t e = join_second_stream(h);
    if (e == hipSuccess) e = gvom_launch_occupancy(h->stream, P, F.state, F.tags, tmp, h->tune_occ_clear != 0);
    if (e == hipSuccess) e = sync_streams(h);
    if (e == hipSuccess) e = hipMemcpy(out_xyz, tmp, h->V, hipMemcpyDeviceToHost);
    hipFree(tmp);
    HIPCHK(h, e);
    return GVOM_OK;
}

static int debug_maps(gvom_t *h, float *out7, float *out3)
{
    if (!h) return GVOM_ERR_INVALID;
    std::lock_guard<std::mutex> lk(h->mu);
    if (!h->has_combined || !h->maps_valid) return GVOM_NO_DATA;
    HIPCHK(h, hipSetDevice(h->device));
    const Fused &F = h->fused[h->cur];
    const size_t n2 = h->cells2d;
    float *tmp = nullptr;
    HIPCHK(h, hipMalloc((void **)&tmp, n2 * 7 * 4));
    double org[3] = {(double)F.origin[0], (double)F.origin[1], (double)F.origin[2]};
    hipError_t e = join_second_stream(h);
    if (e == hipSuccess) e = gvom_launch_debug_height(h->stream, h->prm.xy_size, (int)floor_mod(F.origin[0], h->prm.xy_size),
                                            (int)floor_mod(F.origin[1], h->prm.xy_size), org,
                                            h->prm.xy_resolution, h->prm.z_resolution, h->height, h->hs, h->rough,
                                            h->slope_x, h->slope_y, out7 ? tmp : nullptr, h->guessed,
                                            out3 ? tmp : nullptr);
    if (e == hipSuccess) e = sync_streams(h);
    if (e == hipSuccess) e = hipMemcpy(out7 ? out7 : out3, tmp, n2 * (out7 ? 7 : 3) * 4, hipMemcpyDeviceToHost);
    hipFree(tmp);
    HIPCHK(h, e);
    return GVOM_OK;
}

VIS int gvom_debug_voxel_map(gvom_t *h, float *out, int64_t max_rows, int64_t *rows)
{
    return gvom_debug_voxel_eigen(h, out, nullptr, max_rows, rows);
}

VIS int gvom_debug_voxel_eigen(gvom_t *h, float *out, float *eigen, int64_t max_rows, int64_t *rows)
{
    if (!h || !out || max_rows < 0) return GVOM_ERR_INVALID;
    std::lock_guard<std::mutex> lk(h->mu);
    stats_demand(h);
    if (!h->has_combined || !h->fused[h->cur].has_metrics) return GVOM_NO_DATA;
    HIPCHK(h, hipSetDevice(h->device));
    const gvom_params &p = h->prm;
    const Fused &F = h->fused[h->cur];
    Map2dParams P;
    memset(&P, 0, sizeof P);
    P.xy = p.xy_size; P.zs = p.z_size;
    P.om[0] = (int)floor_mod(F.origin[0], p.xy_size);
    P.om[1] = (int)floor_mod(F.origin[1], p.xy_size);
    P.om[2] = (int)floor_mod(F.origin[2], p.z_size);
    P.y_lo = h->sy_lo; P.y_hi = h->sy_hi;
    P.xy_res = p.xy_resolution; P.z_res = p.z_resolution;
    P.nseg = h->nseg; P.epoch = F.epoch;
    float *tmp = nullptr;
    const size_t mr = (size_t)(max_rows > 0 ? max_rows : 1);
    HIPCHK(h, hipMalloc((void **)&tmp, mr * 44));
    float *tmp_e = eigen ? tmp + mr * 8 : nullptr;
    hipError_t e = join_second_stream(h);
    if (e == hipSuccess) e = hipMemsetAsync(h->counters + 12, 0, 8, h->stream);
    if (e == hipSuccess)
        e = gvom_launch_voxel_cloud(h->stream, P, (double)F.origin[0], (double)F.origin[1], (double)F.origin[2],
                                    F.state, F.tags, (const uint4 *)F.rows.p,
                                    (const float *)F.metrics.p, tmp, tmp_e, max_rows,
                                    (unsigned long long *)(h->counters + 12));
    unsigned long long cnt = 0;
    if (e == hipSuccess) e = sync_streams(h);
    if (e == hipSuccess) e = hipMemcpy(&cnt, h->counters + 12, 8, hipMemcpyDeviceToHost);
    const int64_t nrows = (int64_t)cnt < max_rows ? (int64_t)cnt : max_rows;
    if (e == hipSuccess && nrows > 0) e = hipMemcpy(out, tmp, (size_t)nrows * 32, hipMemcpyDeviceToHost);
    if (e == hipSuccess && nrows > 0 && eigen) e = hipMemcpy(eigen, tmp_e, (size_t)nrows * 12, hipMemcpyDeviceToHost);
    hipFree(tmp);
    HIPCHK(h, e);
    if (rows) *rows = (int64_t)cnt;
    return GVOM_OK;
}

VIS int gvom_debug_height_map(gvom_t *h, float *out) { return out ? debug_maps(h, out, nullptr) : GVOM_ERR_INVALID; }
VIS int gvom_debug_inferred_height_map(gvom_t *h, float *out) { return out ? debug_maps(h, nullptr, out) : GVOM_ERR_INVALID; }

VIS int gvom_get_scan_stats(gvom_t *h, gvom_scan_stats *out)
{
    if (!h || !out) return GVOM_ERR_INVALID;
    int slot;
    {
        std::lock_guard<std::mutex> lk(h->mu);
        slot = h->last_buffer_index;
        if (!h->slots[h->ring[slot]].filled) return GVOM_NO_DATA;
    }
    const size_t V = h->V;
    std::vector<int32_t> hit(V), total(V);
    int64_t cells = 0;
    int rc = gvom_read_dense(h, slot, nullptr, hit.data(), nullptr, nullptr, nullptr, &cells);
    if (rc) return rc;
    std::vector<int32_t> state(V);
    rc = gvom_read_dense(h, slot, state.data(), nullptr, total.data(), nullptr, nullptr, nullptr);
    if (rc) return rc;
    int64_t sh = 0, st = 0;
    for (size_t i = 0; i < V; ++i) {
        sh += hit[i];
        st += state[i] >= 0 ? (int64_t)total[i] : (int64_t)(-(int64_t)state[i] - 1);
    }
    std::lock_guard<std::mutex> lk(h->mu);
    out->points = h->slots[h->ring[slot]].stats.points;
    out->cells = cells; out->sum_hit = sh; out->sum_total = st;
    return GVOM_OK;
}

VIS int gvom_last_stage_ms(gvom_t *h, float ms[GVOM_N_STAGES])
{
    if (!h || !ms) return GVOM_ERR_INVALID;
    std::lock_guard<std::mutex> lk(h->mu);
    if (h->ev_scan || h->ev_fuse || h->ev_map) {
        HIPCHK(h, hipSetDevice(h->device));
        HIPCHK(h, sync_streams(h));
        collect_stage_ms(h);
    }
    for (int k = 0; k < GVOM_N_STAGES; ++k) ms[k] = h->stage_ms[k];
    return GVOM_OK;
}

VIS int gvom_host_timing(gvom_t *h, double us[8])
{
    if (!h || !us) return GVOM_ERR_INVALID;
    std::lock_guard<std::mutex> lk(h->mu);
    for (int k = 0; k < 8; ++k) us[k] = h->host_calls ? h->host_ns[k] / h->host_calls / 1e3 : 0.0;
    return GVOM_OK;
}

VIS int gvom_set_tuning(gvom_t *h, const char *name, int value)
{
    if (!h || !name) return GVOM_ERR_INVALID;
    std::lock_guard<std::mutex> lk(h->mu);
    if (!strcmp(name, "segs")) h->tune_segs = value;
    else if (!strcmp(name, "ep_row")) h->tune_ep_row = value;
    else if (!strcmp(name, "period")) h->tune_period = value;
    else if (!strcmp(name, "prio")) h->tune_prio = value;
    else if (!strcmp(name, "interleave")) h->tune_ilv = value;
    else if (!strcmp(name, "flag_kernel")) h->tune_flag_kernel = value;
    else if (!strcmp(name, "fuse1")) h->tune_fuse1 = value;
    else if (!strcmp(name, "encfuse")) h->tune_encfuse = value;
    else if (!strcmp(name, "dirsort")) h->tune_dirsort = value;
    else if (!strcmp(name, "fastdiv")) h->tune_fastdiv = value;
    else if (!strcmp(name, "eager")) { h->tune_eager = value; h->eager_waste = 0; }
    else if (!strcmp(name, "occupancy_clear")) h->tune_occ_clear = value;
    else if (!strcmp(name, "exported")) h->exported = value != 0;
#ifdef GVOM_HOOKS
    else if (!strcmp(name, "churn")) h->tune_churn = value;
    else if (!strcmp(name, "epoch_bias")) h->epoch += (uint32_t)value;
#endif
    else return GVOM_ERR_INVALID;
    return GVOM_OK;
}

VIS int gvom_get_tuning(gvom_t *h, const char *name, int *value)
{
    if (!h || !name || !value) return GVOM_ERR_INVALID;
    std::lock_guard<std::mutex> lk(h->mu);
    static const char *const names[5] = {"segs", "period", "ep_row", "prio", "interleave"};
    for (int k = 0; k < 5; ++k)
        if (!strcmp(name, names[k])) { *value = h->last_knobs[k]; return GVOM_OK; }
    if (!strcmp(name, "dirsort")) { *value = h->last_dirsort; return GVOM_OK; }
    if (!strcmp(name, "eager_adopted")) { *value = h->eager_stat[0]; return GVOM_OK; }
    if (!strcmp(name, "eager_dropped")) { *value = h->eager_stat[1]; return GVOM_OK; }
    if (!strcmp(name, "fuse_kernel")) { *value = h->last_fuse; return GVOM_OK; }
    if (!strcmp(name, "device_map_sets")) { *value = (int)h->dsets.size(); return GVOM_OK; }
    if (!strcmp(name, "device_product_sets")) { *value = (int)h->psets.size(); return GVOM_OK; }
    if (!strcmp(name, "occupancy_clear")) { *value = h->tune_occ_clear; return GVOM_OK; }
    if (!strcmp(name, "range_image")) { *value = h->ri_H > 0 ? 1 : 0; return GVOM_OK; }
    if (!strcmp(name, "fastdiv")) { *value = h->tune_fastdiv == 0 ? 0 : h->fastdiv_ok; return GVOM_OK; }
    return GVOM_ERR_INVALID;
}

VIS int gvom_set_profiling(gvom_t *h, int on)
{
    if (!h) return GVOM_ERR_INVALID;
    std::lock_guard<std::mutex> lk(h->mu);
    h->profiling = on != 0;
    return GVOM_OK;
}

VIS void *gvom_stream(gvom_t *h) { return h ? (void *)h->stream : nullptr; }
VIS uint64_t gvom_alloc_generation(gvom_t *h) { return h ? h->alloc_gen : 0; }
VIS int gvom_shard_renew_region(gvom_t *h, int which)
{
    if (!h || !h->sharded) return GVOM_ERR_INVALID;
    std::lock_guard<std::mutex> lk(h->mu);
    HIPCHK(h, hipSetDevice(h->device));
    void **pp = nullptr;
    size_t bytes = 0;
    uint64_t *gen = nullptr;
    switch (which) {
    case GVOM_XBUF_SEND_IDS: pp = (void **)&h->x_send_ids; bytes = exportable_size(h->x_Q * 4); gen = &h->fixed_gen[0]; break;
    case GVOM_XBUF_SEND_QUADS: pp = &h->x_send_pay; bytes = exportable_size(h->x_Q * 1024); gen = &h->fixed_gen[1]; break;
    case GVOM_XBUF_SEND_EPS: pp = &h->x_send_eps.p; bytes = h->x_send_eps.bytes; gen = &h->x_send_eps.gen; break;
    case GVOM_XBUF_SEND_RETURNS: pp = &h->x_send_sp.p; bytes = h->x_send_sp.bytes; gen = &h->x_send_sp.gen; break;
    case -1: pp = (void **)&h->hmaps; bytes = exportable_size(h->cells2d * 24); gen = &h->fixed_gen[2]; break;
    default: return GVOM_ERR_INVALID;
    }
    if (!*pp || !bytes) return GVOM_NO_DATA;
    void *np = nullptr;
    HIPCHK(h, hipMalloc(&np, bytes));
    HIPCHK(h, hipStreamSynchronize(h->stream));
    HIPCHK(h, hipMemcpy(np, *pp, bytes, hipMemcpyDeviceToDevice));
    HIPCHK(h, hipDeviceSynchronize());
    Buf old; old.p = *pp; old.bytes = bytes; old.gen = *gen;
    h->retired.push_back(old);
    *pp = np;
    *gen = ++g_alloc_generation;
    if (which == -1) { h->height = h->hmaps; h->inferred = h->hmaps + h->prm.xy_size; }
    if (which == GVOM_XBUF_SEND_EPS || which == GVOM_XBUF_SEND_RETURNS) h->alloc_gen = *gen;
    return GVOM_OK;
}

VIS uint64_t gvom_region_generation(gvom_t *h, int which)
{
    if (!h) return 0;
    if (which == GVOM_XBUF_SEND_EPS) return h->x_send_eps.gen ? h->x_send_eps.gen : h->handle_gen;
    if (which == GVOM_XBUF_SEND_RETURNS) return h->x_send_sp.gen ? h->x_send_sp.gen : h->handle_gen;
    if (which == GVOM_XBUF_SEND_IDS && h->fixed_gen[0]) return h->fixed_gen[0];
    if (which == GVOM_XBUF_SEND_QUADS && h->fixed_gen[1]) return h->fixed_gen[1];
    if (which == -1 && h->fixed_gen[2]) return h->fixed_gen[2];
    return h->handle_gen;
}

VIS const char *gvom_last_error(gvom_t *h) { return h ? h->err.c_str() : "null handle"; }

VIS int gvom_backend_info(char *buf, size_t len)
{
    if (!buf || len == 0) return GVOM_ERR_INVALID;
    int ndev = 0;
    if (hipGetDeviceCount(&ndev) != hipSuccess || ndev <= 0) {
        snprintf(buf, len, "libgvom_hip abi %d (gfx950 code object); no HIP device visible", GVOM_ABI_VERSION);
        return GVOM_ERR_NO_DEVICE;
    }
    hipDeviceProp_t pr;
    if (hipGetDeviceProperties(&pr, 0) != hipSuccess) return GVOM_ERR_HIP;
    snprintf(buf, len, "libgvom_hip abi %d; device0=%s arch=%s CUs=%d; %d device(s)", GVOM_ABI_VERSION,
             pr.name, pr.gcnArchName, pr.multiProcessorCount, ndev);
    return GVOM_OK;
}

VIS int gvom_abi_version(void) { return GVOM_ABI_VERSION; }

#ifdef GVOM_DIAG
VIS int gvom_diag_timeline(gvom_t *h, unsigned long long *out, int64_t max_words, int grid[2])
{
    if (!h || !out || !grid) return GVOM_ERR_INVALID;
    std::lock_guard<std::mutex> lk(h->mu);
    HIPCHK(h, hipSetDevice(h->device));
    HIPCHK(h, sync_streams(h));
    grid[0] = h->tl_grid[0]; grid[1] = h->tl_grid[1];
    const int64_t words = (int64_t)grid[0] * grid[1] * 8 * 4 + 8 +
                          ((int64_t)grid[0] * grid[1] * 8 / 64 + 1) * 128;
    if (!h->tl.p || words <= 8) return GVOM_NO_DATA;
    HIPCHK(h, hipMemcpy(out, h->tl.p, (size_t)(words < max_words ? words : max_words) * 8, hipMemcpyDeviceToHost));
    return GVOM_OK;
}
#endif

}
```

### g-vom_amd/csrc/gvom_fuse.hip

```cpp
#include "gvom_device.h"

template <int ENC_T>
__global__ __launch_bounds__(ENC_T) void k_encode(const ScanParams P, uint32_t t_begin, uint32_t t_end,
                                                uint32_t *hit, uint32_t *total, uint32_t *mh, int32_t *state,
                                                uint16_t *code16, uint4 *crows,
                                                const uint32_t *__restrict__ tags, uint32_t epoch,
                                                uint32_t *counters, unsigned long long *host_flag,
                                                uint32_t seq)
{
    const int xy = P.xy, nseg = P.nseg;
    if (blockIdx.x == 0 && threadIdx.x == 0) {
        const uint32_t any = counters[GVOM_CNT_INGRID] ? 0x80000000u : 0u;
        counters[GVOM_CNT_INGRID] = 0;
        __hip_atomic_store(host_flag, ((unsigned long long)seq << 32) | any, __ATOMIC_RELEASE,
                           __HIP_MEMORY_SCOPE_SYSTEM);
    }
    const int lane = threadIdx.x & (WAVE - 1);
    const uint32_t wid = __builtin_amdgcn_readfirstlane((blockIdx.x * blockDim.x + threadIdx.x) >> 6);
    const uint32_t nw = (gridDim.x * blockDim.x) >> 6;
    const int p4 = lane >> 2, r = lane & 3;
    const bool vec_state = (xy & 3) == 0;
    for (uint32_t u0 = t_begin + wid * 2; u0 < t_end; u0 += nw * 2) {
        uint32_t dmask;
        {
// ... 647 lines not shown
    }
    const uint32_t colbase = (uint32_t)sy * P.zs * P.xy + (col_ok ? sxb : 0);
    const uint32_t tbase = (uint32_t)sy * P.zs * P.nseg + blockIdx.x;
    uint32_t running = 0;
    int zfree[4] = {INT_MAX, INT_MAX, INT_MAX, INT_MAX};
    s_zh[w][lane] = ((unsigned long long)INT_MAX << 32) | 0x3f800000ull;
    s_zf[w][lane] = (uint32_t)INT_MAX;
    const uint32_t rbase = ((blockIdx.y * gridDim.x + blockIdx.x) * (uint32_t)P.nz + w) * (uint32_t)(WAVE * P.zc * P.cpw);

    {
        const int cc_l = lane >> 4, k_l = lane & 15;
        const int zl = (cc_l * P.nz + w) * P.zc + k_l;
        const bool valid_l = cc_l < P.cpw && k_l < P.zc && zl < P.zs;
        const uint32_t tl = tbase + (uint32_t)wrap_add(valid_l ? zl : 0, P.om[2], P.zs) * P.nseg;
        const uint32_t ts = ((gptr_u32)descs[0].tags)[tl];
        const uint32_t tp = has_prev ? ((gptr_u32)descs[1].tags)[tl] : 0u;
        const unsigned long long ms = __ballot(valid_l && ts == descs[0].epoch);
        const unsigned long long mp = __ballot(has_prev && valid_l && tp == descs[1].epoch);
        if (lane == 0) { s_live[w][0] = ms; s_live[w][1] = mp; }
    }
    const gptr_i32 ss = (gptr_i32)descs[0].state;
    const gptr_i32 sp = (gptr_i32)descs[has_prev ? 1 : 0].state;

    for (int cc = 0; cc < P.cpw; ++cc) {
        const int z0 = (cc * P.nz + w) * P.zc;
        if (z0 >= P.zs) break;
        const int z1 = min(z0 + P.zc, P.zs);
        const uint32_t lives = (uint32_t)(s_live[w][0] >> (16 * cc)) & 0xffffu;
        const uint32_t livep = (uint32_t)(s_live[w][1] >> (16 * cc)) & 0xffffu;
        if (__builtin_amdgcn_readfirstlane(lives | livep) == 0) continue;

        uint32_t roff[4];
        v4i vs[4], vp[4];
#pragma unroll
        for (int j = 0; j < 4; ++j) {
            const int zq = z0 + 4 * j + q;
            roff[j] = colbase + (uint32_t)wrap_add(zq < P.zs ? zq : 0, P.om[2], P.zs) * P.xy;
            vs[j] = *(gptr_v4i)(ss + (((lives >> (4 * j + q)) & 1u) ? roff[j] : (uint32_t)(4 * lane)));
            vp[j] = *(gptr_v4i)(sp + (((livep >> (4 * j + q)) & 1u) ? roff[j] : (uint32_t)(4 * lane)));
        }
        uint32_t n = 0;
        auto emit = [&]() {
            for (uint32_t base = 0; base < n; base += WAVE) {
                const uint32_t t = base + (uint32_t)lane;
                const bool on = t < n;
                const uint32_t e = s_list[w][on ? t : 0u];
                const int sts = on ? s_sts[w][t] : -1, stp = on ? s_stp[w][t] : -1;
                const int ci = (int)(e & 3u), go = (int)((e >> 2) & 15u), qo = (int)((e >> 6) & 3u), jo = (int)(e >> 8);
                const int zv = z0 + 4 * jo + qo;
                const int col = 4 * go + ci;
                const int sxc = blockIdx.x * WAVE + col;
                const uint32_t off = (uint32_t)sy * P.zs * P.xy + (uint32_t)wrap_add(zv, P.om[2], P.zs) * P.xy + (uint32_t)sxc;
                const v4u rs = ((gptr_v4u)descs[0].rows)[sts >= 0 ? (uint32_t)sts : 0u];
                const v4u rp = ((gptr_v4u)descs[has_prev ? 1 : 0].rows)[stp >= 0 ? (uint32_t)stp : 0u];
                uint32_t hh = 0, tt = 0, mm = 0x3f800000u;
                if (sts >= 0) { hh += rs.x; tt += rs.y; mm = min(mm, rs.z); }
                if (stp >= 0) { hh += rp.x; tt += rp.y; mm = min(mm, rp.z); }
                const unsigned long long ob = __ballot(on);
                if (on) {
                    const uint32_t row = rbase + running + (uint32_t)__popcll(ob & lanemask_lt());
                    fstate[off] = (int32_t)row;
                    frows[row] = make_uint4(hh, tt, mm, 0u);
                    atomicMin(&s_zh[w][col], ((unsigned long long)(uint32_t)zv << 32) | mm);
                }
                running += (uint32_t)__popcll(ob);
            }
            n = 0;
        };
#pragma unroll
        for (int j = 0; j < 4; ++j) {
            const int zq = z0 + 4 * j + q;
            const bool zs_in = ((lives >> (4 * j + q)) & 1u) && zq < z1 && zq + dsz >= 0 && zq + dsz < P.zs;
            const bool zp_in = ((livep >> (4 * j + q)) & 1u) && zq < z1 && zq + dpz >= 0 && zq + dpz < P.zs;
            const int a[4] = {vs[j].x, vs[j].y, vs[j].z, vs[j].w}, b[4] = {vp[j].x, vp[j].y, vp[j].z, vp[j].w};
            int c[4];
            uint32_t occ = 0;
            int sts_[4], stp_[4];
#pragma unroll
            for (int i = 0; i < 4; ++i) {
                const int st = (zs_in && ((oks >> i) & 1u)) ? a[i] : -1;
                const int pv = (zp_in && ((okp >> i) & 1u)) ? b[i] : -1;
                sts_[i] = st; stp_[i] = pv;
                c[i] = -1;
                if (st >= 0) occ |= 1u << i;
                else if (st < -1) c[i] = add_free(c[i], st + 1);
                if (!((occ >> i) & 1u)) {
                    if (pv >= 0 && c[i] >= -11) occ |= 1u << i;
                    else if (pv < -1) c[i] = add_free(c[i], pv + 1);
                }
            }
            if (!col_ok) occ = 0;
            const bool inside = col_ok && zq < z1;
            const bool nonempty = occ != 0u || c[0] != -1 || c[1] != -1 || c[2] != -1 || c[3] != -1;
            const unsigned long long nb = __ballot(inside && nonempty);
            if (((nb >> (16 * q)) & 0xffffull) && !GVOM_DBG(P, 1)) {
                if (g == 0 && zq < z1) ftags[tbase + (uint32_t)wrap_add(zq, P.om[2], P.zs) * P.nseg] = P.epoch;
                if (inside) {
                    *reinterpret_cast<int4 *>(fstate + roff[j]) = make_int4(c[0], c[1], c[2], c[3]);
#pragma unroll
                    for (int i = 0; i < 4; ++i)
                        if (!((occ >> i) & 1u) && c[i] < -1 && zfree[i] == INT_MAX) zfree[i] = zq;
                }
            }
            if (__any(occ != 0u)) {
#pragma unroll
                for (int i = 0; i < 4; ++i) {
                    const bool o = (occ >> i) & 1u;
                    const unsigned long long bm = __ballot(o);
                    if (o) {
                        const uint32_t at = n + (uint32_t)__popcll(bm & lanemask_lt());
                        s_list[w][at] = (uint16_t)(((uint32_t)j << 8) | ((uint32_t)lane << 2) | (uint32_t)i);
                        s_sts[w][at] = sts_[i]; s_stp[w][at] = stp_[i];
                    }
                    n += (uint32_t)__popcll(bm);
                    if (n > FUSE1_LIST - WAVE) emit();
                }
            }
        }
        if (n) emit();
    }

#pragma unroll
    for (int i = 0; i < 4; ++i)
        if (zfree[i] != INT_MAX) atomicMin(&s_zf[w][4 * g + i], (uint32_t)zfree[i]);
    if (lane == 0) s_cnt[w] = running;
    __syncthreads();
    if (threadIdx.x == 0) {
        uint32_t tot = 0;
        for (int k = 0; k < P.nz; ++k) tot += s_cnt[k];
        blockcounts[blockIdx.y * gridDim.x + blockIdx.x] = tot;
    }
    const int sx = blockIdx.x * WAVE + lane;
    if (w == 0 && sx < P.xy && !GVOM_DBG(P, 16)) {
        const int x = wrap_sub(sx, P.om[0], P.xy);
        unsigned long long zh = ((unsigned long long)INT_MAX << 32) | 0x3f800000ull;
        uint32_t zfu = (uint32_t)INT_MAX;
        for (int k = 0; k < P.nz; ++k) { zh = min(zh, s_zh[k][lane]); zfu = min(zfu, s_zf[k][lane]); }
        const int zo = (int)(zh >> 32), zf = (int)zfu;
        const uint32_t hb = (uint32_t)zh;
        double hval = -1000.0;
        const double xp = ((P.origin[0] + (double)x) * P.xy_res) - P.ego[0];
        const double yp = ((P.origin[1] + (double)y) * P.xy_res) - P.ego[1];
        if (xp * xp + yp * yp <= P.radius2) hval = P.ego[2] - P.ground_to_lidar_height;
        if (zo != INT_MAX)
            hval = (((double)__uint_as_float(hb) + (double)zo) + P.origin[2]) * P.z_res;
        height[(size_t)sy * P.hs + sx] = hval;
        inferred[(size_t)sy * P.hs + sx] =
            (zf != INT_MAX) ? ((double)zf + P.origin[2]) * P.z_res : -1000.0;
    }
}

#define ENCFUSE_MAXIT 8
#define ENCFUSE_LIST 128
__global__ __launch_bounds__(512) __attribute__((amdgpu_waves_per_eu(7, 8))) void k_encfuse(
    const ScanParams P, const FuseParams F, const MapDesc prev, int32_t *flink, uint32_t *hit, uint32_t *total, uint32_t *mh,
    int32_t *state, uint4 *crows, const uint32_t *__restrict__ stags, int32_t *fstate, uint4 *frows, uint32_t *ftags,
    uint32_t *blockcounts, double *height, double *inferred, uint32_t *counters, unsigned long long *host_flag, uint32_t seq)
{
    __shared__ unsigned long long s_zh[8][WAVE];
    __shared__ uint32_t s_zf[8][WAVE];
    __shared__ uint32_t s_cnt[8];
    __shared__ uint32_t s_eL[8][ENCFUSE_LIST], s_eA[8][ENCFUSE_LIST], s_eh[8][ENCFUSE_LIST], s_et[8][ENCFUSE_LIST], s_em[8][ENCFUSE_LIST];
    __shared__ int32_t s_ep[8][ENCFUSE_LIST];
    if (blockIdx.x == 0 && threadIdx.x == 0) {
        const uint32_t any = counters[GVOM_CNT_INGRID] ? 0x80000000u : 0u;
        counters[GVOM_CNT_INGRID] = 0;
        __hip_atomic_store(host_flag, ((unsigned long long)seq << 32) | any, __ATOMIC_RELEASE, __HIP_MEMORY_SCOPE_SYSTEM);
    }
    const int lane = threadIdx.x & (WAVE - 1);
    const int w = __builtin_amdgcn_readfirstlane(threadIdx.x >> 6);
    const int nw = (int)(blockDim.x >> 6);
    const int xy = P.xy, zs = P.zs, nseg = P.nseg;
    const uint32_t nbx = (uint32_t)xy >> 4;
    uint32_t M = blockIdx.x;
    if ((gridDim.x & 15u) == 0u && !(F.cpw & 1)) { const uint32_t slot = M >> 3, xcd = M & 7u; M = ((slot >> 1) << 4) + (xcd << 1) + (slot & 1u); }
    const uint32_t bx = M % nbx, Q = M / nbx;
    const int zl = lane >> 4, p4 = (lane >> 2) & 3, r = lane & 3;
    const uint32_t sx0 = bx * 16u + (uint32_t)p4 * 4u, sy = Q * 4u + (uint32_t)r;
    const uint32_t seg = sx0 >> 6;
    const uint32_t col0 = (uint32_t)(r * 16 + p4 * 4);
    const int y = wrap_sub((int)sy, F.om[1], xy);
    const bool has_prev = F.has_prev != 0;
    const int dpx = has_prev ? prev.d[0] : 0, dpy = has_prev ? prev.d[1] : 0, dpz = has_prev ? prev.d[2] : 0;
    uint32_t okp = 0;
    {
        const bool yp = has_prev && y + dpy >= 0 && y + dpy < xy;
#pragma unroll
        for (int i = 0; i < 4; ++i) {
            const int xw = wrap_sub((int)sx0 + i, F.om[0], xy);
            if (yp && xw + dpx >= 0 && xw + dpx < xy) okp |= 1u << i;
        }
    }
    const gptr_i32 sp = has_prev ? (gptr_i32)prev.state : (gptr_i32)state;
    const gptr_u32 ptags = has_prev ? (gptr_u32)prev.tags : (gptr_u32)stags;
    const gptr_v4u prows = has_prev ? (gptr_v4u)prev.rows : (gptr_v4u)crows;
    const int niter = (zs + 4 * nw - 1) / (4 * nw);
    const uint32_t rbase = (M * (uint32_t)nw + (uint32_t)w) * (uint32_t)(niter * 256);
    uint32_t running = 0, n = 0;
    uint32_t zf[4] = {(uint32_t)INT_MAX, (uint32_t)INT_MAX, (uint32_t)INT_MAX, (uint32_t)INT_MAX};
    s_zh[w][lane] = ((unsigned long long)INT_MAX << 32) | 0x3f800000ull;
    auto emit = [&]() {
        __builtin_amdgcn_fence(__ATOMIC_ACQ_REL, "wavefront");
        __builtin_amdgcn_wave_barrier();
        for (uint32_t base = 0; base < n; base += WAVE) {
            const uint32_t e = base + (uint32_t)lane;
            const bool on = e < n;
            const uint32_t ei = on ? e : 0u;
            const uint32_t L = s_eL[w][ei], A = s_eA[w][ei], h_ = s_eh[w][ei], t_ = s_et[w][ei], meta = s_em[w][ei];
            const int stp = on ? s_ep[w][ei] : -1;
            const bool so = on && ((meta >> 16) & 1u);
            const int32_t row_s = state[so ? L : 0u];
            const uint32_t mraw = mh[so ? A : 0u];
            const v4u rp = prows[stp >= 0 ? (uint32_t)stp : 0u];
            uint32_t hh = 0, tt = 0, mn = 0x3f800000u;
            if (so) {
                const uint32_t mbits = 0x3f800000u - mraw;
                crows[row_s] = make_uint4(h_, t_, mbits, 0u);
                mh[A] = 0u;
                hh += h_; tt += t_; mn = min(mn, mbits);
            }
            if (stp >= 0) { hh += rp.x; tt += rp.y; mn = min(mn, rp.z); }
            const unsigned long long ob = __ballot(on);
            if (on) {
                const uint32_t row = rbase + running + (uint32_t)__popcll(ob & lanemask_lt());
                frows[row] = make_uint4(hh, tt, mn, 0u);
                fstate[L] = (int32_t)row;
                if (flink) flink[row] = stp;
                atomicMin(&s_zh[w][(meta >> 10) & 63u], ((unsigned long long)(meta & 1023u) << 32) | mn);
            }
            running += (uint32_t)__popcll(ob);
        }
        n = 0;
        __builtin_amdgcn_wave_barrier();
    };

    for (int it0 = 0; it0 < niter; it0 += ENCFUSE_MAXIT) {
        uint32_t tv_[ENCFUSE_MAXIT];
#pragma unroll
        for (int k = 0; k < ENCFUSE_MAXIT; ++k) {
            const int szt = ((it0 + k) * nw + w) * 4 + ((lane >> 2) & 3);
            const bool okt = it0 + k < niter && lane < 32 && szt < zs && (lane < 16 || has_prev);
            const uint32_t ti = ((Q * 4u + (uint32_t)(lane & 3)) * (uint32_t)zs + (uint32_t)(okt ? szt : 0)) * (uint32_t)nseg + seg;
            tv_[k] = okt ? (lane < 16 ? stags[ti] : ptags[ti]) : 0u;
        }
        uint32_t lmv = 0u;
#pragma unroll
        for (int k = 0; k < ENCFUSE_MAXIT; ++k) {
            const uint32_t b_ = (uint32_t)__ballot(it0 + k < niter && lane < 32 && tv_[k] != 0u && tv_[k] == (lane < 16 ? P.epoch : prev.epoch));
            if (lane == k) lmv = b_;
        }
        const int kend = min(ENCFUSE_MAXIT, niter - it0);
#pragma unroll 1
        for (int k = 0; k < kend; ++k) {
            const uint32_t m = (uint32_t)__builtin_amdgcn_readlane((int)lmv, k);
            if (m == 0u) continue;
            const int sz = ((it0 + k) * nw + w) * 4 + zl;
            const bool zok = sz < zs;
            const bool live_s = zok && ((m >> (zl * 4 + r)) & 1u);
            const bool live_p = zok && ((m >> (16 + zl * 4 + r)) & 1u);
            const uint32_t A0 = acc_idx((int)sx0, (int)sy, zok ? sz : 0, zs, P.sxq);
            const uint32_t L0 = (sy * (uint32_t)zs + (uint32_t)(zok ? sz : 0)) * (uint32_t)xy + sx0;
            const v4u hv = *(gptr_v4u)(hit + (live_s ? A0 : (uint32_t)(4 * lane)));
            const v4u tv = *(gptr_v4u)(total + (live_s ? A0 : (uint32_t)(4 * lane)));
            const v4i pv = *(gptr_v4i)(sp + (live_p ? L0 : (uint32_t)(4 * lane)));
            const int zw = wrap_sub(zok ? sz : 0, F.om[2], zs);
            const bool zp_in = live_p && zw + dpz >= 0 && zw + dpz < zs;
            const uint32_t h[4] = {hv.x, hv.y, hv.z, hv.w};
            const uint32_t t[4] = {tv.x + hv.x, tv.y + hv.y, tv.z + hv.z, tv.w + hv.w};
            const int b[4] = {pv.x, pv.y, pv.z, pv.w};
            const uint32_t any_h = live_s ? (h[0] | h[1] | h[2] | h[3]) : 0u;
            const uint32_t any_t = live_s ? (tv.x | tv.y | tv.z | tv.w) : 0u;
            int st[4], c[4], stp[4];
            uint32_t occ = 0, socc = 0;
#pragma unroll
            for (int i = 0; i < 4; ++i) {
                st[i] = live_s ? -(int32_t)t[i] - 1 : -1;
                if (live_s && h[i] > 0u) socc |= 1u << i;
                stp[i] = (zp_in && ((okp >> i) & 1u)) ? b[i] : -1;
                c[i] = -1;
                if ((socc >> i) & 1u) occ |= 1u << i;
                else if (st[i] < -1) c[i] = add_free(c[i], st[i] + 1);
                if (!((occ >> i) & 1u)) {
                    if (stp[i] >= 0 && c[i] >= -11) occ |= 1u << i;
                    else if (stp[i] < -1) c[i] = add_free(c[i], stp[i] + 1);
                }
            }
            if (live_s) {
                if (socc == 0u) *reinterpret_cast<int4 *>(state + L0) = make_int4(st[0], st[1], st[2], st[3]);
                else {
#pragma unroll
                    for (int i = 0; i < 4; ++i) if (!((socc >> i) & 1u)) state[L0 + i] = st[i];
                }
                if (any_t) *reinterpret_cast<uint4 *>(total + A0) = make_uint4(0, 0, 0, 0);
                if (any_h) *reinterpret_cast<uint4 *>(hit + A0) = make_uint4(0, 0, 0, 0);
            }
            if (live_s || live_p) {
                if (occ == 0u) *reinterpret_cast<int4 *>(fstate + L0) = make_int4(c[0], c[1], c[2], c[3]);
                else {
#pragma unroll
                    for (int i = 0; i < 4; ++i) if (!((occ >> i) & 1u)) fstate[L0 + i] = c[i];
                }
                if ((sx0 & 63u) == 0u) ftags[(sy * (uint32_t)zs + (uint32_t)sz) * (uint32_t)nseg + seg] = F.epoch;
#pragma unroll
                for (int i = 0; i < 4; ++i)
                    if (!((occ >> i) & 1u) && c[i] < -1) zf[i] = min(zf[i], (uint32_t)zw);
            }
            if (__builtin_amdgcn_readfirstlane((int)(__ballot(occ != 0u) != 0ull))) {
#pragma unroll
                for (int i = 0; i < 4; ++i) {
                    const bool o = (occ >> i) & 1u;
                    const unsigned long long bm = __ballot(o);
                    if (o) {
                        const uint32_t at = n + (uint32_t)__popcll(bm & lanemask_lt());
                        s_eL[w][at] = L0 + (uint32_t)i; s_eA[w][at] = A0 + (uint32_t)i; s_eh[w][at] = h[i]; s_et[w][at] = t[i];
                        s_ep[w][at] = stp[i];
                        s_em[w][at] = (uint32_t)zw | ((col0 + (uint32_t)i) << 10) | (((socc >> i) & 1u) << 16);
                    }
                    n += (uint32_t)__popcll(bm);
                    if (n > ENCFUSE_LIST - WAVE) emit();
                }
            }
        }
    }
    if (n) emit();

#pragma unroll
    for (int i = 0; i < 4; ++i) {
        zf[i] = min(zf[i], (uint32_t)__shfl_xor((int)zf[i], 16));
        zf[i] = min(zf[i], (uint32_t)__shfl_xor((int)zf[i], 32));
    }
    if (zl == 0) {
#pragma unroll
        for (int i = 0; i < 4; ++i) s_zf[w][col0 + i] = zf[i];
    }
    if (lane == 0) s_cnt[w] = running;
    __syncthreads();
    if (threadIdx.x == 0) {
        uint32_t tot = 0;
        for (int k = 0; k < nw; ++k) tot += s_cnt[k];
        blockcounts[M] = tot;
    }
    if (w == 0) {
        const int csx = (int)(bx * 16u) + (lane & 15), csy = (int)(Q * 4u) + (lane >> 4);
        unsigned long long zhm = ((unsigned long long)INT_MAX << 32) | 0x3f800000ull;
        uint32_t zfm = (uint32_t)INT_MAX;
        for (int k = 0; k < nw; ++k) { zhm = min(zhm, s_zh[k][lane]); zfm = min(zfm, s_zf[k][lane]); }
        const int x = wrap_sub(csx, F.om[0], xy), yy = wrap_sub(csy, F.om[1], xy);
        const int zo = (int)(zhm >> 32), zfi = (int)zfm;
        double hval = -1000.0;
        const double xp = ((F.origin[0] + (double)x) * F.xy_res) - F.ego[0];
        const double yp = ((F.origin[1] + (double)yy) * F.xy_res) - F.ego[1];
        if (xp * xp + yp * yp <= F.radius2) hval = F.ego[2] - F.ground_to_lidar_height;
        if (zo != INT_MAX) hval = (((double)__uint_as_float((uint32_t)zhm) + (double)zo) + F.origin[2]) * F.z_res;
        height[(size_t)csy * F.hs + csx] = hval;
        inferred[(size_t)csy * F.hs + csx] = (zfi != INT_MAX) ? ((double)zfi + F.origin[2]) * F.z_res : -1000.0;
    }
}

hipError_t gvom_launch_encode(hipStream_t s, const ScanParams &P, uint32_t *hit, uint32_t *total, uint32_t *mh,
                              int32_t *state, uint16_t *code16, uint4 *crows, const uint32_t *tags,
                              uint32_t *counters, unsigned long long *host_flag, uint32_t seq, unsigned resident_blocks)
{
    const uint32_t q_lo = (uint32_t)P.sy_lo >> 2, q_hi = ((uint32_t)P.sy_hi + 3) >> 2;
    const uint32_t t_begin = q_lo * P.zs * P.nseg, t_end = q_hi * P.zs * P.nseg;
    const uint32_t ntiles = t_end - t_begin;
    const unsigned T = ntiles <= 262144u ? 64u : 256u;
    unsigned enc_blocks = (ntiles + (T / 32) - 1) / (T / 32);
    const unsigned enc_cap = (resident_blocks > 0 ? 4u * resident_blocks : 8192u) * 256u / T;
    if (enc_blocks > enc_cap) enc_blocks = enc_cap;
    if (enc_blocks < 1) enc_blocks = 1;
    if (T == 64u)
        hipLaunchKernelGGL(k_encode<64>, dim3(enc_blocks), dim3(64), 0, s, P, t_begin, t_end, hit, total, mh, state,
                           code16, crows, tags, P.epoch, counters, host_flag, seq);
    else
        hipLaunchKernelGGL(k_encode<256>, dim3(enc_blocks), dim3(256), 0, s, P, t_begin, t_end, hit, total, mh, state,
                           code16, crows, tags, P.epoch, counters, host_flag, seq);
    return hipGetLastError();
}

__global__ void k_publish_seq(unsigned long long *host_flag, uint32_t seq)
{
    __hip_atomic_store(host_flag, (unsigned long long)seq, __ATOMIC_RELEASE, __HIP_MEMORY_SCOPE_SYSTEM);
}
hipError_t gvom_launch_publish_seq(hipStream_t s, unsigned long long *host_flag, uint32_t seq)
{
    hipLaunchKernelGGL(k_publish_seq, dim3(1), dim3(1), 0, s, host_flag, seq);
    return hipGetLastError();
}

__global__ void k_retag(uint32_t *tags, size_t n, uint32_t old_epoch, uint32_t new_epoch)
{
    for (size_t i = (size_t)blockIdx.x * blockDim.x + threadIdx.x; i < n; i += (size_t)gridDim.x * blockDim.x)
        tags[i] = (new_epoch != 0u && tags[i] == old_epoch) ? new_epoch : 0u;
}

hipError_t gvom_launch_retag(hipStream_t s, uint32_t *tags, size_t n, uint32_t old_epoch, uint32_t new_epoch)
{
    hipLaunchKernelGGL(k_retag, dim3(1024), dim3(256), 0, s, tags, n, old_epoch, new_epoch);
    return hipGetLastError();
}

hipError_t gvom_launch_fuse(hipStream_t s, const FuseParams &P, const FuseDescs &KD,
                            const MapDesc *descs_dev, int32_t *fstate, uint4 *frows,
                            uint32_t *ftags, uint32_t *blockcounts,
                            double *height, double *inferred, int *route)
{
    const dim3 grid((P.xy + 63) / 64, P.sy_hi - P.sy_lo);
    if (grid.y == 0) return hipSuccess;
#define FUSE_LAUNCH(...) hipLaunchKernelGGL((__VA_ARGS__), grid, dim3(64 * P.nz), 0, s, P, KD, descs_dev, fstate, frows, \
                                          ftags, blockcounts, height, inferred)
    const bool mem = descs_dev != nullptr;
    if (P.one_slot) {
        hipLaunchKernelGGL(k_fuse1, grid, dim3(64 * P.nz), 0, s, P, KD, fstate, frows, ftags, blockcounts, height, inferred);
        *route = GVOM_ROUTE_FUSE1;
        return hipGetLastError();
    }
    if (P.zc == 16 && (P.xy & 3) == 0 && !GVOM_DBG(P, 8)) {
        if (P.nslots <= 2) { if (mem) FUSE_LAUNCH(k_fuse4<2, true>); else FUSE_LAUNCH(k_fuse4<2, false>); *route = GVOM_ROUTE_FUSE4_2; }
        else { if (mem) FUSE_LAUNCH(k_fuse4<4, true>); else FUSE_LAUNCH(k_fuse4<4, false>); *route = GVOM_ROUTE_FUSE4_4; }
    } else if (P.zc <= 16) {
        if (mem) FUSE_LAUNCH(k_fuse<true, true>); else FUSE_LAUNCH(k_fuse<true, false>);
        *route = GVOM_ROUTE_FUSE_SHORT;
    } else {
        if (mem) FUSE_LAUNCH(k_fuse<false, true>); else FUSE_LAUNCH(k_fuse<false, false>);
        *route = GVOM_ROUTE_FUSE_TALL;
    }
    if (mem) *route |= GVOM_ROUTE_DESCS_MEM;
#undef FUSE_LAUNCH
    return hipGetLastError();
}

void gvom_encfuse_shape(int xy, int zs, int nw_override, int *nw, int *nblocks, size_t *row_cap)
{
    int w = (zs + 3) / 4;
    if (w > 4) w = 4;
    if (w < 1) w = 1;
    if (nw_override > 0 && nw_override <= w) w = nw_override;
    const int niter = (zs + 4 * w - 1) / (4 * w);
    *nw = w; *nblocks = (xy / 16) * (xy / 4);
    *row_cap = (size_t)*nblocks * (size_t)w * (size_t)niter * 256;
}
hipError_t gvom_launch_encfuse(hipStream_t s, const ScanParams &P, const FuseParams &F, const MapDesc &prev, int32_t *flink, uint32_t *hit,
                               uint32_t *total, uint32_t *mh, int32_t *state, uint4 *crows, const uint32_t *stags,
                               int32_t *fstate, uint4 *frows, uint32_t *ftags, uint32_t *blockcounts, double *height,
                               double *inferred, uint32_t *counters, unsigned long long *host_flag, uint32_t seq)
{
    int nw, nblocks; size_t cap;
    gvom_encfuse_shape(P.xy, P.zs, F.nz, &nw, &nblocks, &cap);
    hipLaunchKernelGGL(k_encfuse, dim3((unsigned)nblocks), dim3(64u * (unsigned)nw), 0, s, P, F, prev, flink, hit, total, mh, state, crows,
                       stags, fstate, frows, ftags, blockcounts, height, inferred, counters, host_flag, seq);
    return hipGetLastError();
}
```

### g-vom_amd/csrc/gvom_internal.h

```cpp
#pragma once
#include <hip/hip_runtime.h>
#include <stdint.h>

#define GVOM_MAX_SLOTS 64

#include <stdlib.h>
#include <string.h>
#if defined(GVOM_DIAG) || defined(GVOM_TEST_HOOKS)
#define GVOM_HOOKS 1
#endif
#ifdef GVOM_DIAG
#define GVOM_DBG(P, bits) ((P).dbg & (bits))
static inline int gvom_diag_env(const char *name) { const char *v = getenv(name); return v ? atoi(v) : 0; }
#else
#define GVOM_DBG(P, bits) 0
static inline int gvom_diag_env(const char *) { return 0; }
#endif

#define GVOM_CNT_INGRID 64
#define GVOM_CNT_MAPDONE 32
#define GVOM_CNT_WORDS 192

struct ScanParams {
    double xy_res, z_res;
    double min_d2;
    double origin[3];
    double tf[12];
    float  pt0[3];
    float  rinv[2];
    double drcp[2];
    int    fastdiv;
    float  win_lo[3], win_hi[3];
    int    has_tf;
    int    xy, zs;
    int    om[3];
    int    sy_lo, sy_hi;
    int    nseg;
    int    lg_nseg, lg_zs;
    int    nsegs;
    int    seg_start[10];
    int    ep_row;
    int    prio_div;
    int    lc_period;
    int    ilv_lg;
    long   ilv_len;
    const uint32_t *perm;
    int    f32_sqrt;
    int    sxq;
    uint32_t epoch;
    int    off[3];
    int    in_f32;
    int    stat_e;
    int    shard_world, shard_rank, shard_rows;
    int    dbg;
    int    prof_on;
    long   tl_words;
    unsigned long long *tl;
};

struct ShardExchange {
    uint2    *ep_send;
    uint32_t *ep_cnt;
    long      ep_cap;
    void     *sp_send;
    uint32_t *sp_cnt;
};

#define GVOM_PACK_CHUNK 64
#define GVOM_BASE_PITCH 16
struct ShardUnpack { uint32_t q_off[GVOM_MAX_SLOTS + 1]; };

struct MapDesc {
    const int32_t  *state;
    const uint4 *rows;
    int d[3];
    uint32_t epoch;
    const uint32_t *tags;
    const void *metrics;
    union {
        const uint16_t *code16;
        const int32_t *link;
    };
};

#define GVOM_KARG_DESCS 17
struct FuseDescs { MapDesc d[GVOM_KARG_DESCS]; };

struct FuseParams {
    int xy, zs;
    int om[3];
    int nslots;
    int has_prev;
    int sy_lo, sy_hi;
    int nseg;
    int hs;
    uint32_t epoch;
    int nz;
    int zc;
    int cpw;
    int one_slot;
    int dbg;
    double origin[3];
    double ego[3];
    double xy_res, z_res;
    double radius2;
    double ground_to_lidar_height;
};

struct Map2dParams {
    int xy, zs;
    int om[3];
    int y_lo, y_hi;
    int nseg;
    int hs;
    int gathered_pos;
    uint32_t epoch;
    int dbg;
    int out_yx;
    double origin_z;
    double xy_res, z_res;
    double pos_thr, neg_thr, slope_thr, robot_height;
    int occ;
    double occ_density_thr, occ_min_rough, occ_max_rough;
    unsigned long long *done_flag;
    uint32_t *done_count;
    uint32_t done_seq;
    int out_dev;
};
__host__ __device__ __forceinline__ size_t dev_map_stride(int xy) { return ((size_t)xy * xy + 31) & ~(size_t)31; }

#define GVOM_OCC_ZC 128
struct OccParams {
    int xy, zs;
    int om[3];
    int y_lo, y_hi;
    int nseg;
    uint32_t epoch;
};

hipError_t gvom_launch_trace(hipStream_t s, const ScanParams &P, const ShardExchange &X, int dtype, bool big_origin, const void *pts,
                             int64_t stride_elems, int64_t n, void *world, uint32_t *hit,
                             uint32_t *total, uint32_t *mh, int32_t *state, uint32_t *tags,
                             uint32_t *counters, double *stat_sums, double *stat_base,
                             uint32_t *stat_rowvox);
hipError_t gvom_launch_pack(hipStream_t s, const ScanParams &P, uint32_t *total, const uint32_t *tags, uint32_t *send_ids,
                            void *send_pay, uint32_t *qcnt, uint32_t *ecnt, uint32_t *spcnt, uint32_t *counters,
                            unsigned long long *host_out, uint32_t seq);
hipError_t gvom_launch_unpack(hipStream_t s, const ScanParams &P, const ShardUnpack &X, const uint32_t *ids_all,
                              const void *pay_all, uint32_t my_quads, uint32_t ne, const void *eps, long row_base,
                              uint32_t *hit, uint32_t *total, uint32_t *mh, int32_t *state, uint32_t *tags,
                              double *stat_sums, double *stat_base, uint32_t *stat_rowvox);
hipError_t gvom_launch_encode(hipStream_t s, const ScanParams &P, uint32_t *hit, uint32_t *total, uint32_t *mh,
                              int32_t *state, uint16_t *code16, uint4 *crows, const uint32_t *tags,
                              uint32_t *counters, unsigned long long *host_flag, uint32_t seq, unsigned resident_blocks);
hipError_t gvom_launch_layout_probe(hipStream_t s, const ScanParams &P, int dtype, const void *pts, int64_t stride_elems, int64_t n,
                                    int max_lg, unsigned long long *host_word);
hipError_t gvom_launch_publish_seq(hipStream_t s, unsigned long long *host_flag, uint32_t seq);
#define GVOM_DIRBINS 8192
hipError_t gvom_launch_dirbin(hipStream_t s, const ScanParams &P, int mode, int dtype, const void *pts, int64_t stride_elems, int64_t n,
                              uint16_t *keys, uint32_t *hist, uint32_t *hist_next, uint32_t *cursor, uint32_t *perm);
enum { GVOM_ROUTE_FUSE1 = 1, GVOM_ROUTE_FUSE4_2 = 2, GVOM_ROUTE_FUSE4_4 = 3, GVOM_ROUTE_FUSE_SHORT = 4, GVOM_ROUTE_FUSE_TALL = 5,
       GVOM_ROUTE_ENCFUSE = 6, GVOM_ROUTE_DESCS_MEM = 16 };
hipError_t gvom_launch_fuse(hipStream_t s, const FuseParams &P, const FuseDescs &KD,
                            const MapDesc *descs_dev, int32_t *fstate, uint4 *frows,
                            uint32_t *ftags, uint32_t *blockcounts, double *height, double *inferred, int *route);
void gvom_encfuse_shape(int xy, int zs, int nw_override, int *nw, int *nblocks, size_t *row_cap);
hipError_t gvom_launch_encfuse(hipStream_t s, const ScanParams &P, const FuseParams &F, const MapDesc &prev, int32_t *flink, uint32_t *hit,
                               uint32_t *total, uint32_t *mh, int32_t *state, uint4 *crows, const uint32_t *stags,
                               int32_t *fstate, uint4 *frows, uint32_t *ftags, uint32_t *blockcounts, double *height,
                               double *inferred, uint32_t *counters, unsigned long long *host_flag, uint32_t seq);
hipError_t gvom_launch_map2d(hipStream_t s, const Map2dParams &P, const int32_t *fstate, const uint32_t *ftags,
                             const uint4 *frows, const double *height,
                             const double *inferred, double *slope_x, double *slope_y,
                             double *rough, double *guessed, int32_t *out_pos, int32_t *out_neg,
                             double *out_rough, int32_t *out_vis, const uint32_t *blockcounts,
                             int nblocks, unsigned long long *host_counter);
hipError_t gvom_launch_stats(hipStream_t s, const ScanParams &P, int dtype, const void *world, int64_t n,
                             const int32_t *state, const uint32_t *tags, int xy_e, int z_e, double *base,
                             double *sums, const uint32_t *rowvox, int64_t nrows, const void *extra, int64_t n_extra);
hipError_t gvom_launch_fuse_stats(hipStream_t s, const FuseParams &P, const FuseDescs &KD, const MapDesc *descs_dev,
                                  const int32_t *fstate, const uint32_t *ftags, float *fmetrics);
hipError_t gvom_launch_voxel_cloud(hipStream_t s, const Map2dParams &P, double o0, double o1, double o2,
                                   const int32_t *fstate, const uint32_t *ftags, const uint4 *frows,
                                   const float *fmetrics, float *out, float *eig, int64_t max_rows,
                                   unsigned long long *row_counter);
hipError_t gvom_launch_gather_rows10(hipStream_t s, int is_f64, const void *src, const int32_t *rows, int64_t n, void *out);
hipError_t gvom_launch_retag(hipStream_t s, uint32_t *tags, size_t n, uint32_t old_epoch, uint32_t new_epoch);
hipError_t gvom_launch_read_dense(hipStream_t s, int xy, int zs, const int om[3], int sy_lo, int sy_hi,
                                  const uint32_t *tags, uint32_t epoch, const int32_t *state, const uint4 *crows,
                                  int32_t *o_state,
                                  int32_t *o_hit, int32_t *o_total, float *o_minh, int32_t *o_row);
hipError_t gvom_launch_occupancy(hipStream_t s, const OccParams &P, const int32_t *fstate, const uint32_t *ftags, uint8_t *out,
                                 bool clear_first);
hipError_t gvom_launch_unwrap_f64(hipStream_t s, int xy, int om0, int om1, const double *in, int in_stride, double *out_xy);
hipError_t gvom_launch_posdens(hipStream_t s, const Map2dParams &P, const int32_t *fstate,
                               const uint32_t *ftags, const uint4 *frows,
                               double *hmaps, const uint32_t *blockcounts, int nblocks,
                               unsigned long long *host_counter, unsigned long long *dev_counter);
hipError_t gvom_launch_debug_height(hipStream_t s, int xy, int om0, int om1, const double origin[3], double xy_res,
                                    double z_res, const double *height, int hs, const double *rough,
                                    const double *sx, const double *sy, float *out7,
                                    const double *guessed, float *out3);
```

### g-vom_amd/csrc/gvom_trace.hip

```cpp
#include "gvom_device.h"

#define LC_EMPTY 0xFFFFFFFFu
#define LC_LD(p) __hip_atomic_load((p), __ATOMIC_RELAXED, __HIP_MEMORY_SCOPE_WAVEFRONT)
#define LC_ST(p, v) __hip_atomic_store((p), (v), __ATOMIC_RELAXED, __HIP_MEMORY_SCOPE_WAVEFRONT)
#define LC_KEYPOS(s) ((((s) & 3u) << 4) | ((s) >> 2))
__device__ __forceinline__ void lc_flush(const ScanParams &P, uint32_t *keys, uint32_t *cnt, uint32_t *total, int lane)
{
    const int g = lane >> 4, c = lane & 15;
#pragma unroll
    for (int half = 0; half < 2; ++half) {
        uint32_t v[8], k[8];
#pragma unroll
        for (int q = 0; q < 2; ++q) {
            const v4i kk = *(const v4i *)&keys[g * 16 + half * 8 + q * 4];
            k[q * 4 + 0] = (uint32_t)kk.x; k[q * 4 + 1] = (uint32_t)kk.y; k[q * 4 + 2] = (uint32_t)kk.z; k[q * 4 + 3] = (uint32_t)kk.w;
        }
#pragma unroll
        for (int it = 0; it < 8; ++it) v[it] = LC_LD(&cnt[(half * 8 + it) * 64 + lane]);
#pragma unroll
        for (int it = 0; it < 8; ++it) {
            if (v[it] != 0u) {
                if (!GVOM_DBG(P, 1)) atomicAdd(&total[(k[it] << 4) + (uint32_t)c], v[it]);
                LC_ST(&cnt[(half * 8 + it) * 64 + lane], 0u);
            }
        }
    }
    LC_ST(&keys[lane], LC_EMPTY);
}

template <typename T>
__device__ __forceinline__ void load_return(const ScanParams &P, const T *__restrict__ in, long stride, long i,
                                            T &x, T &y, T &z)
{
    if (sizeof(T) == 8 && P.in_f32) {
        const float *p = reinterpret_cast<const float *>(in) + i * stride;
        x = (T)p[P.off[0]]; y = (T)p[P.off[1]]; z = (T)p[P.off[2]];
    } else {
        const T *p = in + i * stride;
        x = p[P.off[0]]; y = p[P.off[1]]; z = p[P.off[2]];
    }
    if (P.has_tf) {
        const double dx = (double)x, dy = (double)y, dz = (double)z;
        const double o0 = ((dx * P.tf[0] + dy * P.tf[1]) + dz * P.tf[2]) + P.tf[3];
        const double o1 = ((dx * P.tf[4] + dy * P.tf[5]) + dz * P.tf[6]) + P.tf[7];
        const double o2 = ((dx * P.tf[8] + dy * P.tf[9]) + dz * P.tf[10]) + P.tf[11];
        x = (T)o0; y = (T)o1; z = (T)o2;
    }
}

template <bool LIT>
__device__ __forceinline__ bool window_voxel(const ScanParams &P, float px, float py, float pz,
                                             uint32_t &wx, uint32_t &wy, uint32_t &wz,
                                             uint32_t o0 = 0, uint32_t o1 = 0, uint32_t o2 = 0, uint32_t uxy_ = 0, uint32_t zpad = 0)
{
    if (LIT) {
        const double fx = floor((double)px - P.origin[0]);
        const double fy = floor((double)py - P.origin[1]);
        const double fz = floor((double)pz - P.origin[2]);
        const bool in = fx >= 0.0 && fx < (double)P.xy && fy >= 0.0 && fy < (double)P.xy && fz >= 0.0 && fz < (double)P.zs;
        wx = in ? (uint32_t)(int)fx : 0u; wy = in ? (uint32_t)(int)fy : 0u; wz = in ? (uint32_t)(int)fz : 0u;
        return in;
    }
    wx = (uint32_t)cvt_floor_i32(px) - o0;
    wy = (uint32_t)cvt_floor_i32(py) - o1;
    wz = (uint32_t)cvt_floor_i32(pz) - o2;
    return max(max(wx, wy), __builtin_elementwise_add_sat(wz, zpad)) < uxy_;
}
__device__ __forceinline__ uint32_t ray_steps(double lim, double step_len, double inv_step, uint32_t cap)
{
    if (!(0.0 < lim)) return 0u;
    const double q = lim * inv_step;
    if (!(q < (double)cap + 2.0)) return cap + 1u;
    const double jc = ceil(q);
    const double e = (jc * jc) * step_len * 0x1p-51 + step_len * 0x1p-50;
    const double lo = (jc - 1.0) * step_len, hi = jc * step_len;
    if (lo + e < lim && hi - e >= lim) return (uint32_t)jc;
    uint32_t n = 0;
    double length = 0.0;
    while (length < lim && n <= cap) { length += step_len; ++n; }
    return n;
}

template <typename T>
__device__ __forceinline__ double div_by_res(T x, double d, double r, bool fast)
{
    if (sizeof(T) == 4 && fast) {
        const double xd = (double)x;
        const double q = xd * r;
        const double e = __builtin_fma(-q, d, xd);
        const double q2 = __builtin_fma(e, r, q);
        return (fabs(xd) < INFINITY && xd != 0.0) ? q2 : q;
    }
    return (double)x / d;
}

struct Endpoint { bool ingrid; uint32_t L, A, mbits; int sy; };
template <typename T>
__device__ __forceinline__ Endpoint endpoint_of(const ScanParams &P, bool pass, T x, T y, T z)
{
    Endpoint E;
    E.ingrid = false; E.L = 0; E.A = 0; E.mbits = 0; E.sy = 0;
    if (pass) {
        const double fx = floor(div_by_res<T>(x, P.xy_res, P.drcp[0], P.fastdiv & 1) - P.origin[0]);
        const double fy = floor(div_by_res<T>(y, P.xy_res, P.drcp[0], P.fastdiv & 1) - P.origin[1]);
        const double az = div_by_res<T>(z, P.z_res, P.drcp[1], P.fastdiv & 2) - P.origin[2];
        const double fz = floor(az);
        if (fx >= 0.0 && fx < (double)P.xy && fy >= 0.0 && fy < (double)P.xy && fz >= 0.0 && fz < (double)P.zs) {
            E.ingrid = true;
            const int sx = wrap_add((int)fx, P.om[0], P.xy);
            const int sy = wrap_add((int)fy, P.om[1], P.xy);
            const int sz = wrap_add((int)fz, P.om[2], P.zs);
            E.sy = sy;
            E.L = ((uint32_t)sy * P.zs + sz) * P.xy + sx;
            E.A = acc_idx(sx, sy, sz, P.zs, P.sxq);
            E.mbits = 0x3f800000u - __float_as_uint((float)(az - fz));
        }
    }
    return E;
}

__device__ __forceinline__ void endpoint_commit(const ScanParams &P, int lane, long row, bool ingrid, uint32_t L, uint32_t A,
                                                uint32_t mbits, uint32_t *hit, uint32_t *total, uint32_t *mh, int32_t *state,
                                                uint32_t *tags, double *stat_sums, double *stat_base, uint32_t *stat_rowvox)
{
    const uint32_t key = ingrid ? A : (0xFFFFFF00u | (uint32_t)lane);
    const uint32_t leftk = (uint32_t)__builtin_amdgcn_update_dpp((int)~key, (int)key, 0x138 , 0xf, 0xf, false);
    const bool ehead = ingrid && leftk != key;
    const unsigned long long followers = lanes(ingrid) & ~lanes(ehead);
    if (ingrid && mbits && !GVOM_DBG(P, 4)) atomicMax(&mh[A], mbits);
    if (ehead && !GVOM_DBG(P, 4)) {
        const uint32_t run = (uint32_t)__ffsll((long long)~((followers >> lane) >> 1));
        atomicAdd(&hit[A], run);
        tags[(L / P.xy) * P.nseg + ((L % P.xy) >> 6)] = P.epoch;
        state[L] = (int32_t)row;
        if (stat_sums) {
            for (int m = 0; m < 10; ++m) { stat_sums[(size_t)row * 10 + m] = 0.0; stat_base[(size_t)row * GVOM_BASE_PITCH + m] = 0.0; }
            stat_rowvox[row] = L;
        }
    }
}

struct RaySetup { float incx, incy, incz; double step_len, inv_step, lim; bool finite; };
template <typename T>
__device__ __forceinline__ RaySetup ray_setup(const ScanParams &P, T x, T y, T z)
{
    const float e0 = (float)div_by_res<T>(x, P.xy_res, P.drcp[0], P.fastdiv & 1);
    const float e1 = (float)div_by_res<T>(y, P.xy_res, P.drcp[0], P.fastdiv & 1);
    const float e2 = (float)div_by_res<T>(z, P.z_res, P.drcp[1], P.fastdiv & 2);
    float s0 = e0 - P.pt0[0], s1 = e1 - P.pt0[1], s2 = e2 - P.pt0[2];
    const float ss = (s0 * s0 + s1 * s1) + s2 * s2;
    const double ray_length = P.f32_sqrt ? (double)sqrtf(ss) : sqrt((double)ss);
    s0 = (float)((double)s0 / ray_length);
    s1 = (float)((double)s1 / ray_length);
    s2 = (float)((double)s2 / ray_length);
    const float a0 = fabsf(s0), a1 = fabsf(s1), a2 = fabsf(s2);
    const float smax = py_maxf(a0, py_maxf(a1, a2));
    int si = 0;
    if (smax == a1) si = 1;
    if (smax == a2) si = 2;
    const float sd  = si == 0 ? s0 : (si == 1 ? s1 : s2);
    const float so1 = si == 0 ? s1 : (si == 1 ? s2 : s0);
    const float so2 = si == 0 ? s2 : (si == 1 ? s0 : s1);
    const float adom = fabsf(sd);
    const float dir = sd / adom;
    const float inc1 = so1 / adom;
    const float inc2 = so2 / adom;
    const double step_len = fabs(1.0 / (double)sd);
    const double lim = ray_length - 1.0;
    const float incx = si == 0 ? dir : (si == 1 ? inc2 : inc1);
    const float incy = si == 0 ? inc1 : (si == 1 ? dir : inc2);
    const float incz = si == 0 ? inc2 : (si == 1 ? inc1 : dir);
    const bool finite = fabsf(incx) < INFINITY && fabsf(incy) < INFINITY && fabsf(incz) < INFINITY;
    RaySetup R;
    R.incx = incx; R.incy = incy; R.incz = incz; R.step_len = step_len; R.inv_step = fabs((double)sd); R.lim = lim; R.finite = finite;
    return R;
}

struct WalkConsts { uint32_t uxy, uzs, usxq, unseg, om0, om1, om2, o0, o1, o2, zpad, epoch;
#ifdef GVOM_DIAG
    unsigned long long *prof;
    uint32_t prof_n;
#endif
};
__device__ __forceinline__ WalkConsts walk_consts(const ScanParams &P)
{
    WalkConsts C;
    C.uxy = (uint32_t)P.xy; C.uzs = (uint32_t)P.zs; C.usxq = (uint32_t)P.sxq; C.unseg = (uint32_t)P.nseg;
    C.om0 = (uint32_t)P.om[0]; C.om1 = (uint32_t)P.om[1]; C.om2 = (uint32_t)P.om[2];
    C.o0 = (uint32_t)(int)P.origin[0]; C.o1 = (uint32_t)(int)P.origin[1]; C.o2 = (uint32_t)(int)P.origin[2];
    C.zpad = C.uxy - C.uzs; C.epoch = P.epoch;
    return C;
}

template <bool LIT, bool P2, bool NOWIN>
__device__ __forceinline__ void walk_steps(const ScanParams &P, int lane, uint32_t &j, uint32_t cnt, float &px_, float &py_, float &pz,
                                           float incx, float incy, float incz, bool &active, int steps,
                                           uint32_t *lck, uint32_t *lcc, uint32_t *total, uint32_t *tags, const WalkConsts &C)
{
    const uint32_t uxy = C.uxy, uzs = C.uzs, usxq = C.usxq, unseg = C.unseg, om0 = C.om0, om1 = C.om1, om2 = C.om2;
    const uint32_t o0 = C.o0, o1 = C.o1, o2 = C.o2, zpad = C.zpad, epoch = C.epoch;
    lds_u32 *const keys3 = (lds_u32 *)lck;
    lds_u32 *const cnt3 = (lds_u32 *)lcc;
    glb_u32 *const total1 = (glb_u32 *)total;
    uint32_t memo = LC_EMPTY;
    uint32_t ju = (uint32_t)__builtin_amdgcn_readfirstlane((int)j);
    const uint32_t cnt_run = min(cnt, ju + (uint32_t)steps);
    unsigned long long alive = lanes(active);
    v2f pxy = {px_, py_};
    const v2f incxy = {incx, incy};
    uint32_t leftk = 0xFFFFFFFFu;
    unsigned long long cmask;
#ifdef GVOM_DIAG
    WalkConsts &CW = const_cast<WalkConsts &>(C);
#define PROF_STAMP(k) do { if (CW.prof && CW.prof_n < 32u) { const unsigned long long t_ = __builtin_amdgcn_s_memtime(); if (lane == 0) CW.prof[CW.prof_n * 4u + (k)] = t_; } } while (0)
#else
#define PROF_STAMP(k) do { } while (0)
#endif
    do {
        PROF_STAMP(0);
        ++ju;
        pxy += incxy; pz += incz;
        uint32_t sx, sy, sz;
        uint32_t wx, wy, wz;
        if (NOWIN && P2) {
            sx = ((uint32_t)cvt_floor_i32(pxy.x) + (om0 - o0)) & (uxy - 1u);
            sy = ((uint32_t)cvt_floor_i32(pxy.y) + (om1 - o1)) & (uxy - 1u);
            sz = ((uint32_t)cvt_floor_i32(pz) + (om2 - o2)) & (uzs - 1u);
            cmask = alive;
        } else {
            const bool inwin = window_voxel<LIT>(P, pxy.x, pxy.y, pz, wx, wy, wz, o0, o1, o2, uxy, zpad);
            if (P2) { sx = (wx + om0) & (uxy - 1u); sy = (wy + om1) & (uxy - 1u); sz = (wz + om2) & (uzs - 1u); }
            else { sx = min(wx + om0, wx + om0 - uxy); sy = min(wy + om1, wy + om1 - uxy); sz = min(wz + om2, wz + om2 - uzs); }
            cmask = NOWIN ? alive : (lanes(inwin) & alive);
        }
        const uint32_t line = mad24s(mad24s(sy >> 2, uzs, sz), usxq, sx >> 2);
        const uint32_t low4 = ((sy & 3u) << 2) | (sx & 3u);
        const uint32_t Ls = (line << 4) | low4;
        leftk = (uint32_t)__builtin_amdgcn_update_dpp((int)leftk, (int)Ls, 0x138 , 0xf, 0xf, false);
        const unsigned long long hm = (lanes(leftk != Ls) | ~(cmask << 1) | (1ull << 32)) & cmask;
        const unsigned long long ends = ((hm | ~cmask) >> 1) | (1ull << 63) | (1ull << 31);
        PROF_STAMP(1);
        if (__builtin_amdgcn_inverse_ballot_w64(hm) && !GVOM_DBG(P, 16)) {
            const uint32_t lrow = Ls >> 2;
            const bool miss = lrow != memo;
            const uint32_t hh = ((sz & 3u) << 4) | (((sy >> 2) & 3u) << 2) | ((sx >> 2) & 3u);
            uint32_t was = LC_EMPTY;
            if (miss) {
                __hip_atomic_compare_exchange_strong(&keys3[LC_KEYPOS(hh)], &was, line, __ATOMIC_RELAXED, __ATOMIC_RELAXED,
                                                     __HIP_MEMORY_SCOPE_WORKGROUP);
                if (!GVOM_DBG(P, 2)) tags[mad24s(mad24s(sy, uzs, sz), unseg, sx >> 6)] = epoch;
            }
            const uint32_t run = 1u + (uint32_t)__builtin_ctz((uint32_t)(ends >> lane));
            const bool ok = (was == LC_EMPTY) | (was == line);
            memo = ok ? lrow : memo;
            if (!GVOM_DBG(P, 128))
            __hip_atomic_fetch_add(&cnt3[ok ? hh * 16u + low4 : 1024u], run, __ATOMIC_RELAXED, __HIP_MEMORY_SCOPE_WORKGROUP);
            if (!ok) __hip_atomic_fetch_add(&total1[Ls], run, __ATOMIC_RELAXED, __HIP_MEMORY_SCOPE_AGENT);
        }
        PROF_STAMP(2);
        alive = cmask & lanes(ju < cnt_run);
        PROF_STAMP(3);
#ifdef GVOM_DIAG
        if (CW.prof) ++CW.prof_n;
#endif
    } while (alive != 0ull);
#undef PROF_STAMP
    j = ju;
    px_ = pxy.x; py_ = pxy.y;
    active = ((cmask >> lane) & 1ull) != 0ull && ju < cnt;
    lc_flush(P, lck, lcc, total, lane);
}

__device__ __forceinline__ void prio_by_remaining(uint32_t rem, uint32_t div)
{
    const uint32_t q = rem / div;
    if (q >= 3u) __builtin_amdgcn_s_setprio(3);
    else if (q == 2u) __builtin_amdgcn_s_setprio(2);
    else if (q == 1u) __builtin_amdgcn_s_setprio(1);
    else __builtin_amdgcn_s_setprio(0);
}

template <bool BIG>
__device__ __forceinline__ void walk_item(const ScanParams &P, int lane, uint32_t j, uint32_t cnt, float px, float py, float pz,
                                          float incx, float incy, float incz, bool active, int steps, int period,
                                          uint32_t *lck, uint32_t *lcc, uint32_t *total, uint32_t *tags, uint32_t jend, const WalkConsts &C)
{
    const bool p2 = ((P.xy & (P.xy - 1)) | (P.zs & (P.zs - 1))) == 0;
    while (steps > 0 && lanes(active) != 0ull) {
        const int run = min(steps, period);
        steps -= run;
        if (P.prio_div > 0) {
            const uint32_t ju = (uint32_t)__builtin_amdgcn_readfirstlane((int)j);
            prio_by_remaining(jend > ju ? jend - ju : 0u, (uint32_t)P.prio_div);
        }
        bool lit = BIG || P.zs > P.xy;
        bool nowin = false;
        if (!lit) {
            const float fs = (float)min((uint32_t)run, cnt - j);
            const float ax = px + incx, ay = py + incy, az = pz + incz;
            const float qx = px + fs * incx, qy = py + fs * incy, qz = pz + fs * incz;
            const float lx = fminf(ax, qx), hx = fmaxf(ax, qx), ly = fminf(ay, qy), hy = fmaxf(ay, qy), lz = fminf(az, qz), hz = fmaxf(az, qz);
            const bool nz = (lx <= 1e-4f && hx >= -1e-4f && !(incx >= 0.0f && ax >= 0.0f)) ||
                            (ly <= 1e-4f && hy >= -1e-4f && !(incy >= 0.0f && ay >= 0.0f)) ||
                            (lz <= 1e-4f && hz >= -1e-4f && !(incz >= 0.0f && az >= 0.0f));
            lit = lanes(active & nz) != 0ull;
            const bool safe = lx >= P.win_lo[0] && hx <= P.win_hi[0] && ly >= P.win_lo[1] && hy <= P.win_hi[1] && lz >= P.win_lo[2] && hz <= P.win_hi[2];
            nowin = p2 && !lit && lanes(active & !safe) == 0ull;
        }
        if (lit) {
            if (p2) walk_steps<true, true, false>(P, lane, j, cnt, px, py, pz, incx, incy, incz, active, run, lck, lcc, total, tags, C);
            else walk_steps<true, false, false>(P, lane, j, cnt, px, py, pz, incx, incy, incz, active, run, lck, lcc, total, tags, C);
        } else if (nowin) {
            walk_steps<false, true, true>(P, lane, j, cnt, px, py, pz, incx, incy, incz, active, run, lck, lcc, total, tags, C);
        } else {
            if (p2) walk_steps<false, true, false>(P, lane, j, cnt, px, py, pz, incx, incy, incz, active, run, lck, lcc, total, tags, C);
            else walk_steps<false, false, false>(P, lane, j, cnt, px, py, pz, incx, incy, incz, active, run, lck, lcc, total, tags, C);
        }
    }
}

#ifdef GVOM_DIAG
#define TL_MARK(P, widx, k) do { if ((P).tl && (threadIdx.x & 63) == 0) (P).tl[(size_t)(widx) * 4 + (k)] = __builtin_amdgcn_s_memrealtime(); } while (0)
#define TL_WHERE(P, widx, pos) do { if ((P).tl && (threadIdx.x & 63) == 0) (P).tl[(size_t)(widx) * 4 + 3] = \
    (unsigned long long)(__builtin_amdgcn_s_getreg((31 << 11) | 4) & 0xffffu) | ((unsigned long long)(__builtin_amdgcn_s_getreg((31 << 11) | 20) & 15u) << 32) | \
    ((unsigned long long)(pos) << 40); } while (0)
#else
#define TL_MARK(P, widx, k) do { } while (0)
#define TL_WHERE(P, widx, pos) do { } while (0)
#endif

template <typename T, bool BIG>
__device__ __forceinline__ void trace_item(const ScanParams &P, const ShardExchange &X, const T *__restrict__ in, long stride, long n,
                                           T *__restrict__ world, uint32_t *hit, uint32_t *total, uint32_t *mh, int32_t *state,
                                           uint32_t *tags, uint32_t *counters, double *stat_sums, double *stat_base,
                                           uint32_t *stat_rowvox, int row, long bundle, int lane, uint32_t *lck, uint32_t *lcc,
                                           size_t widx, const WalkConsts &C)
{
    const long pos = bundle * 64 + lane;
    const bool live = pos < n;
    const long i = P.perm ? (live ? (long)P.perm[pos] : pos) : (P.ilv_lg ? (pos & ((1L << P.ilv_lg) - 1)) * P.ilv_len + (pos >> P.ilv_lg) : pos);
    T x = 0, y = 0, z = 0;
    if (live) load_return(P, in, stride, i, x, y, z);
    const T d2 = (x * x + y * y) + z * z;
    const bool pass = live && !((double)d2 < P.min_d2);
    const bool ep_here = P.ep_row >= 0 ? row == P.ep_row : row == 0;
    if (ep_here) {
        if (live && world) { world[3 * i + 0] = x; world[3 * i + 1] = y; world[3 * i + 2] = z; }
        const Endpoint E = endpoint_of<T>(P, pass, x, y, z);
        if (lanes(E.ingrid) != 0ull && lane == 0) counters[GVOM_CNT_INGRID] = 1u;
        bool mine = E.ingrid;
        if (P.shard_world > 1) {
            const int d = E.sy / P.shard_rows;
            const bool foreign = E.ingrid && d != P.shard_rank;
            mine = E.ingrid && !foreign;
            unsigned long long fm = lanes(foreign);
            while (fm != 0ull) {
                const int first = __ffsll((long long)fm) - 1;
                const int dd = __builtin_amdgcn_readlane(d, first);
                const unsigned long long m = lanes(foreign && d == dd);
                uint32_t base = 0;
                if (lane == first) base = atomicAdd(&X.ep_cnt[dd * 16], (uint32_t)__popcll(m));
                base = (uint32_t)__builtin_amdgcn_readlane((int)base, first);
                if (foreign && d == dd) X.ep_send[(size_t)dd * X.ep_cap + base + (uint32_t)__popcll(m & lanemask_lt())] = make_uint2(E.L, E.mbits);
                fm &= ~m;
            }
            if (X.sp_send) {
                int t0 = -1, t1 = -1;
                const double ay = floor((double)y / P.xy_res - P.origin[1]);
                if (pass && fabs(ay) < 1e9) {
                    const int yb = (int)ay, lo = max(yb - P.stat_e, 0), hi = min(yb + P.stat_e, P.xy - 1);
                    if (lo <= hi) {
                        t0 = wrap_add(lo, P.om[1], P.xy) / P.shard_rows;
                        t1 = wrap_add(hi, P.om[1], P.xy) / P.shard_rows;
                        if (t1 == t0) t1 = -1;
                    }
                }
#pragma unroll 1
                for (int pass_k = 0; pass_k < 2; ++pass_k) {
                    const int d = pass_k == 0 ? t0 : t1;
                    const bool go = d >= 0 && d != P.shard_rank;
                    unsigned long long gm = lanes(go);
                    while (gm != 0ull) {
                        const int first = __ffsll((long long)gm) - 1;
                        const int dd = __builtin_amdgcn_readlane(d, first);
                        const unsigned long long m = lanes(go && d == dd);
                        uint32_t base = 0;
                        if (lane == first) base = atomicAdd(&X.sp_cnt[dd * 16], (uint32_t)__popcll(m));
                        base = (uint32_t)__builtin_amdgcn_readlane((int)base, first);
                        if (go && d == dd) {
                            T *dst = (T *)X.sp_send + ((size_t)dd * X.ep_cap + base + (uint32_t)__popcll(m & lanemask_lt())) * 3;
                            dst[0] = x; dst[1] = y; dst[2] = z;
                        }
                        gm &= ~m;
                    }
                }
            }
        }
        endpoint_commit(P, lane, i, mine, E.L, E.A, E.mbits, hit, total, mh, state, tags, stat_sums, stat_base, stat_rowvox);
        if (P.ep_row >= 0) { TL_MARK(P, widx, 2); return; }
    }
    int seg = P.ep_row >= 0 ? row - (row > P.ep_row ? 1 : 0) : row;
    uint32_t j0 = 0;
#ifdef GVOM_DIAG
    if (seg >= P.nsegs) { seg = P.nsegs; j0 = 0x3ffffff0u; }
    else
#endif
    j0 = (uint32_t)P.seg_start[seg];
    if (P.prio_div > 0) __builtin_amdgcn_s_setprio(3);
    if (seg > 0) {
        const float ax = (float)x * P.rinv[0], ay = (float)y * P.rinv[0], az = (float)z * P.rinv[1];
        const float ux = ax - P.pt0[0], uy = ay - P.pt0[1], uz = az - P.pt0[2];
        const float r = sqrtf((ux * ux + uy * uy) + uz * uz);
        const float mag = ((fabsf(ax) + fabsf(ay)) + fabsf(az)) + ((fabsf(ux) + fabsf(uy)) + fabsf(uz));
        const bool dead = !pass || (r + (r * 1e-5f + mag * 4e-6f) <= (float)j0 + 0.9f);
        if (lanes(!dead) == 0ull) { TL_MARK(P, widx, 2); return; }
    }
    const RaySetup R = ray_setup<T>(P, x, y, z);
    float px = P.pt0[0], py = P.pt0[1], pz = P.pt0[2];
    bool run = pass && R.finite;
    if (run) {
        uint32_t wx, wy, wz;
        run = window_voxel<true>(P, px + R.incx, py + R.incy, pz + R.incz, wx, wy, wz);
    }
    const uint32_t cnt = (run && !GVOM_DBG(P, 8)) ? ray_steps(R.lim, R.step_len, R.inv_step, 0x7ffffff0u) : 0u;
    const bool active = j0 < cnt;
    if (lanes(active) == 0ull) { TL_MARK(P, widx, 2); return; }
    {
        v2f pxy = {px, py};
        const v2f incxy = {R.incx, R.incy};
        for (uint32_t k = j0; k > 0; --k) { pxy += incxy; pz += R.incz; }
        px = pxy.x; py = pxy.y;
    }
    const int steps = seg == P.nsegs - 1 ? 0x3fffffff : P.seg_start[seg + 1] - (int)j0;
    uint32_t jend = 0;
    if (P.prio_div > 0) {
        uint32_t m = active ? min(cnt, j0 + (uint32_t)min(steps, 1 << 20)) : 0u;
#pragma unroll
        for (int o = 32; o > 0; o >>= 1) m = max(m, (uint32_t)__shfl_xor((int)m, o));
        jend = (uint32_t)__builtin_amdgcn_readfirstlane((int)m);
    }
    TL_MARK(P, widx, 1);
    walk_item<BIG>(P, lane, j0, cnt, px, py, pz, R.incx, R.incy, R.incz, active, steps, P.lc_period, lck, lcc, total, tags, jend, C);
    TL_MARK(P, widx, 2);
}

template <typename T, bool BIG, int WPB>
__global__ __launch_bounds__(64 * WPB) __attribute__((amdgpu_waves_per_eu(8, 8))) void k_trace(
    const ScanParams P, const ShardExchange X, const T *__restrict__ in, long stride, long n, T *__restrict__ world,
    uint32_t *hit, uint32_t *total, uint32_t *mh, int32_t *state, uint32_t *tags, uint32_t *counters, double *stat_sums,
    double *stat_base, uint32_t *stat_rowvox)
{
    const int lane = threadIdx.x & (WAVE - 1);
    const int row = (int)blockIdx.y;
    const long bundle = (long)blockIdx.x * WPB + (threadIdx.x >> 6);
    const size_t widx = ((size_t)blockIdx.y * gridDim.x + blockIdx.x) * WPB + (threadIdx.x >> 6);
    TL_MARK(P, widx, 0); TL_WHERE(P, widx, blockIdx.y * gridDim.x + blockIdx.x);
    __shared__ __attribute__((aligned(16))) uint32_t s_keys[WPB * 64];
    __shared__ uint32_t s_cnt[WPB * 1040];
    uint32_t *lck = s_keys + (threadIdx.x >> 6) * 64;
    uint32_t *lcc = s_cnt + (threadIdx.x >> 6) * 1040;
    if (row != P.ep_row) {
        LC_ST(&lck[lane], LC_EMPTY);
#pragma unroll
        for (int q = 0; q < 16; ++q) LC_ST(&lcc[q * 64 + lane], 0u);
    }
    WalkConsts WC = walk_consts(P);
#ifdef GVOM_DIAG
    WC.prof = (P.tl && P.prof_on && (widx & 63) == 0 && row != P.ep_row) ? P.tl + P.tl_words + 8 + (widx >> 6) * 128 : nullptr;
    WC.prof_n = 0;
#endif
    trace_item<T, BIG>(P, X, in, stride, n, world, hit, total, mh, state, tags, counters, stat_sums, stat_base, stat_rowvox,
                       row, bundle, lane, lck, lcc, widx, WC);
}

__global__ __launch_bounds__(256) void k_pack(const ScanParams P, uint32_t *total, const uint32_t *__restrict__ tags,
                                              uint32_t *send_ids, uint4 *send_pay, uint32_t *qcnt)
{
    __shared__ uint32_t s_list[GVOM_PACK_CHUNK];
    __shared__ uint32_t s_count, s_base;
    const int lane = threadIdx.x & (WAVE - 1), wv = threadIdx.x >> 6;
    int d = (int)blockIdx.y;
    if (d >= P.shard_rank) ++d;
    const uint32_t nseg = (uint32_t)P.nseg, zs = (uint32_t)P.zs;
    const uint32_t u_begin = ((uint32_t)(d * P.shard_rows) >> 2) * zs * nseg;
    const uint32_t u_end = ((uint32_t)((d + 1) * P.shard_rows) >> 2) * zs * nseg;
    if (wv == 0) {
        const uint32_t u = u_begin + blockIdx.x * GVOM_PACK_CHUNK + (uint32_t)lane;
        bool dirty = false;
        if (u < u_end) {
            const uint32_t seg = u % nseg, sz = (u / nseg) % zs, q = u / (nseg * zs);
#pragma unroll
            for (int r = 0; r < 4; ++r) dirty = dirty || tags[((q * 4 + r) * zs + sz) * nseg + seg] == P.epoch;
        }
        const unsigned long long dm = lanes(dirty);
        if (dirty) s_list[__popcll(dm & lanemask_lt())] = u;
        if (lane == 0) {
            const uint32_t count = (uint32_t)__popcll(dm);
            s_count = count;
            s_base = count ? atomicAdd(&qcnt[d * 16], count) : 0u;
        }
    }
    __syncthreads();
    const uint32_t count = s_count;
    if (count == 0) return;
    uint32_t *ids = send_ids + u_begin;
    uint4 *pay = send_pay + (size_t)u_begin * 64;
    const int p4 = lane >> 2, r = lane & 3;
    for (uint32_t k = (uint32_t)wv; k < count; k += 4) {
        const uint32_t uq = s_list[k];
        const uint32_t seg = uq % nseg, sz = (uq / nseg) % zs, q = uq / (nseg * zs);
        const uint32_t sx0 = seg * 64 + p4 * 4, sy = q * 4 + r;
        const bool ok = sx0 < (uint32_t)P.xy;
        uint4 tv = make_uint4(0, 0, 0, 0);
        const uint32_t A0 = ok ? acc_idx((int)sx0, (int)sy, (int)sz, P.zs, P.sxq) : 0u;
        if (ok) tv = *reinterpret_cast<const uint4 *>(total + A0);
        pay[(size_t)(s_base + k) * 64 + lane] = tv;
        if (ok && (tv.x | tv.y | tv.z | tv.w)) *reinterpret_cast<uint4 *>(total + A0) = make_uint4(0, 0, 0, 0);
        if (lane == 0) ids[s_base + k] = uq;
    }
}

__global__ void k_shard_publish(int world, uint32_t *qcnt, uint32_t *ecnt, uint32_t *spcnt, uint32_t *counters,
                                unsigned long long *host_out, uint32_t seq)
{
    const int d = threadIdx.x;
    if (d < world) {
        __hip_atomic_store(&host_out[d], (unsigned long long)qcnt[d * 16], __ATOMIC_RELAXED, __HIP_MEMORY_SCOPE_SYSTEM);
        __hip_atomic_store(&host_out[world + d], (unsigned long long)ecnt[d * 16], __ATOMIC_RELAXED, __HIP_MEMORY_SCOPE_SYSTEM);
        __hip_atomic_store(&host_out[2 * world + 2 + d], (unsigned long long)spcnt[d * 16], __ATOMIC_RELAXED, __HIP_MEMORY_SCOPE_SYSTEM);
        qcnt[d * 16] = 0; ecnt[d * 16] = 0; spcnt[d * 16] = 0;
    }
    __syncthreads();
    if (d == 0) {
        __hip_atomic_store(&host_out[2 * world], (unsigned long long)(counters[GVOM_CNT_INGRID] ? 1u : 0u), __ATOMIC_RELAXED,
                           __HIP_MEMORY_SCOPE_SYSTEM);
        __hip_atomic_store(&host_out[2 * world + 1], (unsigned long long)seq, __ATOMIC_RELEASE, __HIP_MEMORY_SCOPE_SYSTEM);
    }
}

__global__ __launch_bounds__(256) void k_unpack_quads(const ScanParams P, const ShardUnpack X, const uint32_t *__restrict__ ids_all,
                                                      const uint32_t *__restrict__ pay_all, uint32_t my_quads, uint32_t *total,
                                                      uint32_t *tags)
{
    const int lane = threadIdx.x & (WAVE - 1);
    const uint32_t w = __builtin_amdgcn_readfirstlane((blockIdx.x * blockDim.x + threadIdx.x) >> 6);
    if (w >= X.q_off[P.shard_world]) return;
    int src = 0;
    while (w >= X.q_off[src + 1]) ++src;
    const uint32_t k = w - X.q_off[src];
    const uint32_t nseg = (uint32_t)P.nseg, zs = (uint32_t)P.zs;
    const uint32_t uq = ids_all[(size_t)src * my_quads + k];
    const uint32_t *pay = pay_all + ((size_t)src * my_quads + k) * 256;
    const uint32_t seg = uq % nseg, sz = (uq / nseg) % zs, q = uq / (nseg * zs);
    if (seg * 64 >= (uint32_t)P.xy || q * 4 + 3 >= (uint32_t)P.xy) return;
    const uint32_t base = acc_idx((int)(seg * 64), (int)(q * 4), (int)sz, P.zs, P.sxq);
    uint32_t rows = 0;
#pragma unroll
    for (int i = 0; i < 4; ++i) {
        const uint32_t v = pay[i * 64 + lane];
        if (v) atomicAdd(&total[base + (uint32_t)(i * 64 + lane)], v);
        const unsigned long long m = lanes(v != 0u);
#pragma unroll
        for (int r = 0; r < 4; ++r) if (m & (0x000F000F000F000Full << (4 * r))) rows |= 1u << r;
    }
    if (lane < 4 && ((rows >> lane) & 1u)) tags[((q * 4 + (uint32_t)lane) * zs + sz) * nseg + seg] = P.epoch;
}

__global__ __launch_bounds__(256) void k_unpack_eps(const ScanParams P, uint32_t ne, const uint2 *__restrict__ eps, long row_base,
                                                    uint32_t *hit, uint32_t *total, uint32_t *mh, int32_t *state, uint32_t *tags,
                                                    double *stat_sums, double *stat_base, uint32_t *stat_rowvox)
{
    const int lane = threadIdx.x & (WAVE - 1);
    const uint32_t i = blockIdx.x * blockDim.x + threadIdx.x;
    const bool live = i < ne;
    uint32_t L = 0, A = 0, mbits = 0;
    if (live) {
        const uint2 e = eps[i];
        L = e.x; mbits = e.y;
        const uint32_t sx = L % (uint32_t)P.xy, rz = L / (uint32_t)P.xy;
        A = acc_idx((int)sx, (int)(rz / (uint32_t)P.zs), (int)(rz % (uint32_t)P.zs), P.zs, P.sxq);
    }
    endpoint_commit(P, lane, row_base + (long)i, live, L, A, mbits, hit, total, mh, state, tags, stat_sums, stat_base, stat_rowvox);
}

hipError_t gvom_launch_trace(hipStream_t s, const ScanParams &P, const ShardExchange &X, int dtype, bool big_origin, const void *pts,
                             int64_t stride_elems, int64_t n, void *world, uint32_t *hit,
                             uint32_t *total, uint32_t *mh, int32_t *state, uint32_t *tags,
                             uint32_t *counters, double *stat_sums, double *stat_base,
                             uint32_t *stat_rowvox)
{
    if (n <= 0) return hipSuccess;
#define TRACE_LAUNCH(TT, BB, WW)                                                                             \
    hipLaunchKernelGGL((k_trace<TT, BB, WW>), dim3((unsigned)((n + 64 * WW - 1) / (64 * WW)), (unsigned)P.nsegs + (P.ep_row >= 0 ? 1u : 0u) + ((unsigned)GVOM_DBG(P, 0xF00) >> 8)), dim3(64 * WW), 0, s, P, X, (const TT *)pts, \
                       (long)stride_elems, (long)n, (TT *)world, hit, total, mh, state, tags, counters,     \
                       stat_sums, stat_base, stat_rowvox)
    if (dtype == 0) { if (big_origin) TRACE_LAUNCH(float, true, 8); else TRACE_LAUNCH(float, false, 8); }
    else { if (big_origin) TRACE_LAUNCH(double, true, 8); else TRACE_LAUNCH(double, false, 8); }
#undef TRACE_LAUNCH
    return hipGetLastError();
}

hipError_t gvom_launch_pack(hipStream_t s, const ScanParams &P, uint32_t *total, const uint32_t *tags, uint32_t *send_ids,
                            void *send_pay, uint32_t *qcnt, uint32_t *ecnt, uint32_t *spcnt, uint32_t *counters,
                            unsigned long long *host_out, uint32_t seq)
{
    const uint32_t slab_quads = ((uint32_t)P.shard_rows >> 2) * (uint32_t)P.zs * (uint32_t)P.nseg;
    if (P.shard_world > 1 && slab_quads > 0)
        hipLaunchKernelGGL(k_pack, dim3((slab_quads + GVOM_PACK_CHUNK - 1) / GVOM_PACK_CHUNK, (unsigned)P.shard_world - 1u),
                           dim3(256), 0, s, P, total, tags, send_ids, (uint4 *)send_pay, qcnt);
    hipLaunchKernelGGL(k_shard_publish, dim3(1), dim3(64), 0, s, P.shard_world, qcnt, ecnt, spcnt, counters, host_out, seq);
    return hipGetLastError();
}

hipError_t gvom_launch_unpack(hipStream_t s, const ScanParams &P, const ShardUnpack &X, const uint32_t *ids_all,
                              const void *pay_all, uint32_t my_quads, uint32_t ne, const void *eps, long row_base,
                              uint32_t *hit, uint32_t *total, uint32_t *mh, int32_t *state, uint32_t *tags,
                              double *stat_sums, double *stat_base, uint32_t *stat_rowvox)
{
    const uint32_t nq = X.q_off[P.shard_world];
    if (nq) hipLaunchKernelGGL(k_unpack_quads, dim3((nq + 3) / 4), dim3(256), 0, s, P, X, ids_all, (const uint32_t *)pay_all,
                               my_quads, total, tags);
    if (ne) hipLaunchKernelGGL(k_unpack_eps, dim3((ne + 255) / 256), dim3(256), 0, s, P, ne, (const uint2 *)eps, row_base, hit,
                               total, mh, state, tags, stat_sums, stat_base, stat_rowvox);
    return hipGetLastError();
}

template <typename T>
__device__ __forceinline__ uint32_t dirbin_key(const ScanParams &P, int mode, const T *__restrict__ in, long stride, long i)
{
    T x, y, z;
    load_return(P, in, stride, i, x, y, z);
    const float ux = (float)x * P.rinv[0] - P.pt0[0], uy = (float)y * P.rinv[0] - P.pt0[1], uz = (float)z * P.rinv[1] - P.pt0[2];
    if (mode == 2) {
        const float r = sqrtf((ux * ux + uy * uy) + uz * uz);
        if (!(r > 0.0f) || !(r < INFINITY)) return 0u;
        const uint32_t row = (uint32_t)min(255, max(0, (int)((uz / r + 1.0f) * 128.0f)));
        const uint32_t sec = (uint32_t)min(31, max(0, (int)((atan2f(uy, ux) + 3.14159265f) * (32.0f / 6.2831853f))));
        return row * 32u + sec;
    }
    const float ax = fabsf(ux), ay = fabsf(uy), az = fabsf(uz);
    uint32_t face;
    float a, u, v;
    if (ax >= ay && ax >= az) { face = ux < 0.0f ? 1u : 0u; a = ax; u = uy; v = uz; }
    else if (ay >= az) { face = uy < 0.0f ? 3u : 2u; a = ay; u = uz; v = ux; }
    else { face = uz < 0.0f ? 5u : 4u; a = az; u = ux; v = uy; }
    if (!(a > 0.0f) || !(a < INFINITY)) return 0u;
    const uint32_t qu = (uint32_t)min(15, max(0, (int)((u / a + 1.0f) * 8.0f)));
    const uint32_t qv = (uint32_t)min(15, max(0, (int)((v / a + 1.0f) * 8.0f)));
    auto part = [](uint32_t t) { t = (t | (t << 2)) & 0x33u; return (t | (t << 1)) & 0x55u; };
    return face * 256u + (part(qu) | (part(qv) << 1));
}
template <typename T, int DIRBIN_ITEMS, int NBINS>
__global__ __launch_bounds__(256) void k_dirbin_hist(const ScanParams P, int mode, const T *__restrict__ in, long stride, long n, uint16_t *keys,
                                                     uint32_t *hist, uint32_t *cursor)
{
    __shared__ uint32_t s_h[NBINS];
    for (int b = threadIdx.x; b < NBINS; b += 256) s_h[b] = 0u;
    if (blockIdx.x == 0) for (int b = threadIdx.x; b < NBINS; b += 256) cursor[b] = 0u;
    __syncthreads();
    const long base = (long)blockIdx.x * (256 * DIRBIN_ITEMS);
#pragma unroll
    for (int k = 0; k < DIRBIN_ITEMS; ++k) {
        const long i = base + k * 256 + threadIdx.x;
        if (i < n) {
            const uint32_t key = dirbin_key(P, mode, in, stride, i);
            keys[i] = (uint16_t)key;
            atomicAdd(&s_h[key], 1u);
        }
    }
    __syncthreads();
    for (int b = threadIdx.x; b < NBINS; b += 256) { const uint32_t c = s_h[b]; if (c) atomicAdd(&hist[b], c); }
}
template <int DIRBIN_ITEMS, int NBINS>
__global__ __launch_bounds__(256) void k_dirbin_scatter(long n, const uint16_t *__restrict__ keys, const uint32_t *__restrict__ hist,
                                                        uint32_t *hist_next, uint32_t *cursor, uint32_t *perm)
{
    constexpr int BPT = NBINS / 256;
    __shared__ uint32_t s_start[NBINS];
    __shared__ uint32_t s_cnt[NBINS];
    __shared__ uint32_t s_part[256];
    uint32_t acc = 0;
    for (int k = 0; k < BPT; ++k) { const uint32_t c = hist[threadIdx.x * BPT + k]; s_start[threadIdx.x * BPT + k] = c; acc += c; s_cnt[threadIdx.x * BPT + k] = 0u; }
    if (blockIdx.x == 0) for (int k = threadIdx.x; k < GVOM_DIRBINS; k += 256) hist_next[k] = 0u;
    uint32_t inc = acc;
    const int ln = threadIdx.x & 63;
#pragma unroll
    for (int o = 1; o < 64; o <<= 1) { const uint32_t v = (uint32_t)__shfl_up((int)inc, o); if (ln >= o) inc += v; }
    if (ln == 63) s_part[threadIdx.x >> 6] = inc;
    __syncthreads();
    for (int wv = 0; wv < (int)(threadIdx.x >> 6); ++wv) inc += s_part[wv];
    uint32_t run = inc - acc;
    for (int k = 0; k < BPT; ++k) { const uint32_t c = s_start[threadIdx.x * BPT + k]; s_start[threadIdx.x * BPT + k] = run; run += c; }
    __syncthreads();
    const long base = (long)blockIdx.x * (256 * DIRBIN_ITEMS);
    uint32_t key[DIRBIN_ITEMS], rank[DIRBIN_ITEMS];
#pragma unroll
    for (int k = 0; k < DIRBIN_ITEMS; ++k) {
        const long i = base + k * 256 + threadIdx.x;
        key[k] = i < n ? (uint32_t)keys[i] : 0xffffu;
        rank[k] = key[k] != 0xffffu ? atomicAdd(&s_cnt[key[k]], 1u) : 0u;
    }
    __syncthreads();
    for (int b = threadIdx.x; b < NBINS; b += 256) {
        const uint32_t c = s_cnt[b];
        if (c) s_start[b] += atomicAdd(&cursor[b], c);
    }
    __syncthreads();
#pragma unroll
    for (int k = 0; k < DIRBIN_ITEMS; ++k) {
        const long i = base + k * 256 + threadIdx.x;
        if (key[k] != 0xffffu) perm[s_start[key[k]] + rank[k]] = (uint32_t)i;
    }
}
hipError_t gvom_launch_dirbin(hipStream_t s, const ScanParams &P, int mode, int dtype, const void *pts, int64_t stride_elems, int64_t n,
                              uint16_t *keys, uint32_t *hist, uint32_t *hist_next, uint32_t *cursor, uint32_t *perm)
{
    if (n <= 0) return hipSuccess;
#define DIRBIN_LAUNCH(IT, NB)                                                                                                  \
    do {                                                                                                                       \
        const unsigned blocks = (unsigned)((n + 256 * IT - 1) / (256 * IT));                                                   \
        if (dtype == 0) hipLaunchKernelGGL((k_dirbin_hist<float, IT, NB>), dim3(blocks), dim3(256), 0, s, P, mode, (const float *)pts, (long)stride_elems, (long)n, keys, hist, cursor); \
        else hipLaunchKernelGGL((k_dirbin_hist<double, IT, NB>), dim3(blocks), dim3(256), 0, s, P, mode, (const double *)pts, (long)stride_elems, (long)n, keys, hist, cursor);          \
        hipLaunchKernelGGL((k_dirbin_scatter<IT, NB>), dim3(blocks), dim3(256), 0, s, (long)n, keys, hist, hist_next, cursor, perm);  \
    } while (0)
    if (mode == 2) { if (n <= 524288) DIRBIN_LAUNCH(2, 8192); else DIRBIN_LAUNCH(8, 8192); }
    else if (n <= 131072) DIRBIN_LAUNCH(1, 1536); else if (n <= 524288) DIRBIN_LAUNCH(2, 1536); else DIRBIN_LAUNCH(8, 1536);
#undef DIRBIN_LAUNCH
    return hipGetLastError();
}

template <typename T>
__global__ __launch_bounds__(64) void k_layout_probe(const ScanParams P, const T *__restrict__ in, long stride, long n, int max_lg,
                                                     unsigned long long *host_word)
{
    const int lane = threadIdx.x;
    int best = 0;
    int scattered = 0;
    if (n >= 8192) {
        const long q = (n / 64) * lane + n / 128;
        float d0[3] = {0.0f, 0.0f, 0.0f}, e1 = 0.0f, ez = 0.0f;
        bool good = true;
#pragma unroll
        for (int k = 0; k < 3; ++k) {
            T x, y, z;
            load_return(P, in, stride, q + (k == 0 ? 0 : (k == 1 ? 1 : 63)), x, y, z);
            const float ux = (float)x * P.rinv[0] - P.pt0[0], uy = (float)y * P.rinv[0] - P.pt0[1], uz = (float)z * P.rinv[1] - P.pt0[2];
            const float r = sqrtf((ux * ux + uy * uy) + uz * uz);
// ... 42 lines not shown
```

Baseline: 1329 M points/s.

## Track endpoint-hit tiles separately so fusion skips hit loads for miss-only tiles

```diff
diff --git a/g-vom_amd/csrc/gvom_capi.hip b/g-vom_amd/csrc/gvom_capi.hip
--- a/g-vom_amd/csrc/gvom_capi.hip
+++ b/g-vom_amd/csrc/gvom_capi.hip
@@ -1,5 +1,6 @@
 #include "gvom_internal.h"
 #include "gvom_ingest.h"
+#include "gvom_plan.h"
 #include "../../include/gvom_hip.h"
 
 #include <math.h>
@@ -29,6 +30,7 @@
     int32_t *state = nullptr;
     uint16_t *code16 = nullptr;
     uint32_t *tags = nullptr;
+    uint32_t *htags = nullptr;
     uint32_t epoch = 0;
     Buf crows;
     Buf metrics, base, rowvox;
@@ -167,6 +169,7 @@
     int tune_encfuse = 0;
     int tune_fastdiv = -1;
     int fastdiv_ok = 0;
+    int tune_hitskip = 1;
     int tune_eager = -1;
     int eager_waste = 0;
     int eager_stat[2] = {0, 0};
@@ -516,12 +519,17 @@
         CK(hipGetDeviceProperties(&pr, device_id));
         h->resident_blocks = (unsigned)pr.multiProcessorCount * 8u;
     }
+    const HandlePlan plan = gvom_plan_handle(sharded, params->buffer_size, xy, zs);
     h->slots.resize(params->buffer_size + 1);
     for (auto &s : h->slots) {
         CK(hipMalloc((void **)&s.state, h->V * 4));
         if ((params->xy_size & 3) == 0) CK(hipMalloc((void **)&s.code16, h->V * 2));
         CK(hipMalloc((void **)&s.tags, h->ntiles * 4));
         CK(hipMemsetAsync(s.tags, 0, h->ntiles * 4, h->stream));
+        if (plan.htags) {
+            CK(hipMalloc((void **)&s.htags, h->ntiles * 4));
+            CK(hipMemsetAsync(s.htags, 0, h->ntiles * 4, h->stream));
+        }
     }
     h->ring.resize(params->buffer_size);
     for (int i = 0; i < params->buffer_size; ++i) h->ring[i] = i;
@@ -544,7 +552,7 @@
     CK(hipMalloc((void **)&h->blockcounts, (size_t)(h->fuse_blocks > 0 ? h->fuse_blocks : 1) * 4));
     CK(hipMemsetAsync(h->blockcounts, 0, (size_t)(h->fuse_blocks > 0 ? h->fuse_blocks : 1) * 4, h->stream));
     h->cnt_blocks = h->fuse_blocks;
-    if (!sharded && params->buffer_size == 1 && xy % 16 == 0 && zs >= 4) {
+    if (plan.eager) {
         CK(hipMalloc((void **)&h->blockcounts2, (size_t)(h->fuse_blocks > 0 ? h->fuse_blocks : 1) * 4));
         CK(hipMemsetAsync(h->blockcounts2, 0, (size_t)(h->fuse_blocks > 0 ? h->fuse_blocks : 1) * 4, h->stream));
         CK(hipMalloc((void **)&h->hmaps2, h->cells2d * 24));
@@ -763,7 +771,7 @@
         h->spec_has_metrics = true;
     }
     HIPCHK(h, gvom_launch_encfuse(h->stream, P, FP, pd, flink, h->hit, h->total, h->mh, st.state, (uint4 *)st.crows.p, st.tags,
-                                  F.state, (uint4 *)F.rows.p, F.tags, h->blockcounts2, h->hmaps2, h->hmaps2 + p.xy_size,
+                                  h->tune_hitskip ? st.htags : nullptr, F.state, (uint4 *)F.rows.p, F.tags, h->blockcounts2, h->hmaps2, h->hmaps2 + p.xy_size,
                                   h->counters, (unsigned long long *)h->counters_host_dev, seq));
     h->spec_valid = true; h->spec_nxt = nxt; h->spec_slot = h->staging; h->spec_blocks = nblocks; h->spec_epoch = FP.epoch;
     h->spec_origin[0] = origin[0]; h->spec_origin[1] = origin[1]; h->spec_origin[2] = origin[2];
@@ -880,7 +888,7 @@
     }
     le = gvom_launch_trace(h->stream, P, X, dtype, big, dev_pts, stride_elems, n,
                                       h->stats ? wpts.p : nullptr, h->hit, h->total, h->mh, st.state,
-                                      st.tags, h->counters, h->stats ? (double *)st.metrics.p : nullptr,
+                                      st.tags, st.htags, h->counters, h->stats ? (double *)st.metrics.p : nullptr,
                                       h->stats ? (double *)st.base.p : nullptr,
                                       h->stats ? (uint32_t *)st.rowvox.p : nullptr);
     if (le != hipSuccess) { scan_abort(h); HIPCHK(h, le); }
@@ -990,6 +998,7 @@
         const bool inflight = (int)k == h->staging && (h->scan_inflight || h->pending);
         const uint32_t fresh = (sl.filled || inflight) ? ++next : 0u;
         HIPCHK(h, gvom_launch_retag(h->stream, sl.tags, h->ntiles, sl.epoch, fresh));
+        if (sl.htags) HIPCHK(h, gvom_launch_retag(h->stream, sl.htags, h->ntiles, sl.epoch, fresh));
         sl.epoch = fresh;
         if (inflight) h->pending_P.epoch = fresh;
     }
@@ -1449,7 +1458,7 @@
     hipFree(h->x_recv_ids); hipFree(h->x_recv_pay);
     hipFree(h->x_qcnt); hipFree(h->x_ecnt); hipFree(h->x_spcnt); fb(h->x_recv_eps); fb(h->x_recv_sp);
     if (h->x_host) hipHostFree(h->x_host);
-    for (auto &s : h->slots) { hipFree(s.state); hipFree(s.code16); hipFree(s.tags); fb(s.crows); fb(s.metrics); fb(s.base); fb(s.rowvox); }
+    for (auto &s : h->slots) { hipFree(s.state); hipFree(s.code16); hipFree(s.tags); hipFree(s.htags); fb(s.crows); fb(s.metrics); fb(s.base); fb(s.rowvox); }
     for (auto &f : h->fused) { hipFree(f.state); hipFree(f.tags); fb(f.rows); fb(f.metrics); }
     fb(h->in_pts); fb(h->ri_model); fb(h->ri_raw); fb(h->ri_poses); if (h->ri_poses_pin) hipHostFree(h->ri_poses_pin); fb(h->world_pts[0]); fb(h->world_pts[1]); fb(h->flink[0]); fb(h->flink[1]); fb(h->tl); fb(h->dir_keys); fb(h->dir_perm); hipFree(h->dir_hist);
     hipFree(h->counters); if (h->counters_host) hipHostFree(h->counters_host);
@@ -2698,6 +2707,7 @@
     else if (!strcmp(name, "dirsort")) h->tune_dirsort = value;
     else if (!strcmp(name, "fastdiv")) h->tune_fastdiv = value;
     else if (!strcmp(name, "eager")) { h->tune_eager = value; h->eager_waste = 0; }
+    else if (!strcmp(name, "hitskip")) h->tune_hitskip = value != 0;
     else if (!strcmp(name, "occupancy_clear")) h->tune_occ_clear = value;
     else if (!strcmp(name, "exported")) h->exported = value != 0;
 #ifdef GVOM_HOOKS
@@ -2723,6 +2733,7 @@
     if (!strcmp(name, "device_product_sets")) { *value = (int)h->psets.size(); return GVOM_OK; }
     if (!strcmp(name, "occupancy_clear")) { *value = h->tune_occ_clear; return GVOM_OK; }
     if (!strcmp(name, "range_image")) { *value = h->ri_H > 0 ? 1 : 0; return GVOM_OK; }
+    if (!strcmp(name, "hitskip")) { *value = h->tune_hitskip; return GVOM_OK; }
     if (!strcmp(name, "fastdiv")) { *value = h->tune_fastdiv == 0 ? 0 : h->fastdiv_ok; return GVOM_OK; }
     return GVOM_ERR_INVALID;
 }
diff --git a/g-vom_amd/csrc/gvom_fuse.hip b/g-vom_amd/csrc/gvom_fuse.hip
--- a/g-vom_amd/csrc/gvom_fuse.hip
+++ b/g-vom_amd/csrc/gvom_fuse.hip
@@ -823,16 +823,18 @@
 
 #define ENCFUSE_MAXIT 8
 #define ENCFUSE_LIST 128
-__global__ __launch_bounds__(512) __attribute__((amdgpu_waves_per_eu(7, 8))) void k_encfuse(
+template <int NWC>
+__global__ __launch_bounds__(64 * NWC) __attribute__((amdgpu_waves_per_eu(7, 8))) void k_encfuse(
     const ScanParams P, const FuseParams F, const MapDesc prev, int32_t *flink, uint32_t *hit, uint32_t *total, uint32_t *mh,
-    int32_t *state, uint4 *crows, const uint32_t *__restrict__ stags, int32_t *fstate, uint4 *frows, uint32_t *ftags,
-    uint32_t *blockcounts, double *height, double *inferred, uint32_t *counters, unsigned long long *host_flag, uint32_t seq)
-{
-    __shared__ unsigned long long s_zh[8][WAVE];
-    __shared__ uint32_t s_zf[8][WAVE];
-    __shared__ uint32_t s_cnt[8];
-    __shared__ uint32_t s_eL[8][ENCFUSE_LIST], s_eA[8][ENCFUSE_LIST], s_eh[8][ENCFUSE_LIST], s_et[8][ENCFUSE_LIST], s_em[8][ENCFUSE_LIST];
-    __shared__ int32_t s_ep[8][ENCFUSE_LIST];
+    int32_t *state, uint4 *crows, const uint32_t *__restrict__ stags, const uint32_t *__restrict__ htags, int32_t *fstate, uint4 *frows,
+    uint32_t *ftags, uint32_t *blockcounts, double *height, double *inferred, uint32_t *counters, unsigned long long *host_flag,
+    uint32_t seq)
+{
+    __shared__ unsigned long long s_zh[NWC][WAVE];
+    __shared__ uint32_t s_zf[NWC][WAVE];
+    __shared__ uint32_t s_cnt[NWC];
+    __shared__ uint32_t s_eL[NWC][ENCFUSE_LIST], s_eA[NWC][ENCFUSE_LIST], s_eh[NWC][ENCFUSE_LIST], s_et[NWC][ENCFUSE_LIST], s_em[NWC][ENCFUSE_LIST];
+    __shared__ int32_t s_ep[NWC][ENCFUSE_LIST];
     if (blockIdx.x == 0 && threadIdx.x == 0) {
         const uint32_t any = counters[GVOM_CNT_INGRID] ? 0x80000000u : 0u;
         counters[GVOM_CNT_INGRID] = 0;
@@ -864,6 +866,8 @@
     }
     const gptr_i32 sp = has_prev ? (gptr_i32)prev.state : (gptr_i32)state;
     const gptr_u32 ptags = has_prev ? (gptr_u32)prev.tags : (gptr_u32)stags;
+    const bool hskip = htags != nullptr;
+    const gptr_u32 etags = hskip ? (gptr_u32)htags : (gptr_u32)stags;
     const gptr_v4u prows = has_prev ? (gptr_v4u)prev.rows : (gptr_v4u)crows;
     const int niter = (zs + 4 * nw - 1) / (4 * nw);
     const uint32_t rbase = (M * (uint32_t)nw + (uint32_t)w) * (uint32_t)(niter * 256);
@@ -910,28 +914,31 @@
 #pragma unroll
         for (int k = 0; k < ENCFUSE_MAXIT; ++k) {
             const int szt = ((it0 + k) * nw + w) * 4 + ((lane >> 2) & 3);
-            const bool okt = it0 + k < niter && lane < 32 && szt < zs && (lane < 16 || has_prev);
+            const bool okt = it0 + k < niter && lane < 48 && szt < zs && (lane < 16 || (lane < 32 ? has_prev : hskip));
             const uint32_t ti = ((Q * 4u + (uint32_t)(lane & 3)) * (uint32_t)zs + (uint32_t)(okt ? szt : 0)) * (uint32_t)nseg + seg;
-            tv_[k] = okt ? (lane < 16 ? stags[ti] : ptags[ti]) : 0u;
-        }
-        uint32_t lmv = 0u;
+            tv_[k] = okt ? (lane < 16 ? stags[ti] : (lane < 32 ? ptags[ti] : etags[ti])) : 0u;
+        }
+        uint32_t lmv = 0u, lmh = 0u;
 #pragma unroll
         for (int k = 0; k < ENCFUSE_MAXIT; ++k) {
-            const uint32_t b_ = (uint32_t)__ballot(it0 + k < niter && lane < 32 && tv_[k] != 0u && tv_[k] == (lane < 16 ? P.epoch : prev.epoch));
-            if (lane == k) lmv = b_;
+            const unsigned long long b_ = __ballot(it0 + k < niter && lane < 48 && tv_[k] != 0u && tv_[k] == ((lane >> 4) == 1 ? prev.epoch : P.epoch));
+            if (lane == k) { lmv = (uint32_t)b_; lmh = (hskip ? (uint32_t)(b_ >> 32) : (uint32_t)b_) & 0xffffu; }
         }
         const int kend = min(ENCFUSE_MAXIT, niter - it0);
 #pragma unroll 1
         for (int k = 0; k < kend; ++k) {
             const uint32_t m = (uint32_t)__builtin_amdgcn_readlane((int)lmv, k);
             if (m == 0u) continue;
+            const uint32_t mh_ = (uint32_t)__builtin_amdgcn_readlane((int)lmh, k);
             const int sz = ((it0 + k) * nw + w) * 4 + zl;
             const bool zok = sz < zs;
             const bool live_s = zok && ((m >> (zl * 4 + r)) & 1u);
             const bool live_p = zok && ((m >> (16 + zl * 4 + r)) & 1u);
+            const bool live_h = live_s && ((mh_ >> (zl * 4 + r)) & 1u);
             const uint32_t A0 = acc_idx((int)sx0, (int)sy, zok ? sz : 0, zs, P.sxq);
             const uint32_t L0 = (sy * (uint32_t)zs + (uint32_t)(zok ? sz : 0)) * (uint32_t)xy + sx0;
-            const v4u hv = *(gptr_v4u)(hit + (live_s ? A0 : (uint32_t)(4 * lane)));
+            v4u hv = *(gptr_v4u)(hit + (live_h ? A0 : (uint32_t)(4 * lane)));
+            if (!live_h) hv = (v4u){0u, 0u, 0u, 0u};
             const v4u tv = *(gptr_v4u)(total + (live_s ? A0 : (uint32_t)(4 * lane)));
             const v4i pv = *(gptr_v4i)(sp + (live_p ? L0 : (uint32_t)(4 * lane)));
             const int zw = wrap_sub(zok ? sz : 0, F.om[2], zs);
@@ -939,7 +946,7 @@
             const uint32_t h[4] = {hv.x, hv.y, hv.z, hv.w};
             const uint32_t t[4] = {tv.x + hv.x, tv.y + hv.y, tv.z + hv.z, tv.w + hv.w};
             const int b[4] = {pv.x, pv.y, pv.z, pv.w};
-            const uint32_t any_h = live_s ? (h[0] | h[1] | h[2] | h[3]) : 0u;
+            const uint32_t any_h = live_h ? (h[0] | h[1] | h[2] | h[3]) : 0u;
             const uint32_t any_t = live_s ? (tv.x | tv.y | tv.z | tv.w) : 0u;
             int st[4], c[4], stp[4];
             uint32_t occ = 0, socc = 0;
@@ -1112,13 +1119,17 @@
     *row_cap = (size_t)*nblocks * (size_t)w * (size_t)niter * 256;
 }
 hipError_t gvom_launch_encfuse(hipStream_t s, const ScanParams &P, const FuseParams &F, const MapDesc &prev, int32_t *flink, uint32_t *hit,
-                               uint32_t *total, uint32_t *mh, int32_t *state, uint4 *crows, const uint32_t *stags,
+                               uint32_t *total, uint32_t *mh, int32_t *state, uint4 *crows, const uint32_t *stags, const uint32_t *htags,
                                int32_t *fstate, uint4 *frows, uint32_t *ftags, uint32_t *blockcounts, double *height,
                                double *inferred, uint32_t *counters, unsigned long long *host_flag, uint32_t seq)
 {
     int nw, nblocks; size_t cap;
     gvom_encfuse_shape(P.xy, P.zs, F.nz, &nw, &nblocks, &cap);
-    hipLaunchKernelGGL(k_encfuse, dim3((unsigned)nblocks), dim3(64u * (unsigned)nw), 0, s, P, F, prev, flink, hit, total, mh, state, crows,
-                       stags, fstate, frows, ftags, blockcounts, height, inferred, counters, host_flag, seq);
+    if (nw < 1 || nw > 4) return hipErrorInvalidValue;
+#define ENCFUSE_LAUNCH(NWC) hipLaunchKernelGGL(k_encfuse<NWC>, dim3((unsigned)nblocks), dim3(64u * (unsigned)nw), 0, s, P, F, prev, flink, hit, \
+                                               total, mh, state, crows, stags, htags, fstate, frows, ftags, blockcounts, height, inferred,       \
+                                               counters, host_flag, seq)
+    if (nw == 1) ENCFUSE_LAUNCH(1); else if (nw == 2) ENCFUSE_LAUNCH(2); else ENCFUSE_LAUNCH(4);
+#undef ENCFUSE_LAUNCH
     return hipGetLastError();
 }
diff --git a/g-vom_amd/csrc/gvom_internal.h b/g-vom_amd/csrc/gvom_internal.h
--- a/g-vom_amd/csrc/gvom_internal.h
+++ b/g-vom_amd/csrc/gvom_internal.h
@@ -140,7 +140,7 @@
 
 hipError_t gvom_launch_trace(hipStream_t s, const ScanParams &P, const ShardExchange &X, int dtype, bool big_origin, const void *pts,
                              int64_t stride_elems, int64_t n, void *world, uint32_t *hit,
-                             uint32_t *total, uint32_t *mh, int32_t *state, uint32_t *tags,
+                             uint32_t *total, uint32_t *mh, int32_t *state, uint32_t *tags, uint32_t *htags,
                              uint32_t *counters, double *stat_sums, double *stat_base,
                              uint32_t *stat_rowvox);
 hipError_t gvom_launch_pack(hipStream_t s, const ScanParams &P, uint32_t *total, const uint32_t *tags, uint32_t *send_ids,
@@ -166,7 +166,7 @@
                             uint32_t *ftags, uint32_t *blockcounts, double *height, double *inferred, int *route);
 void gvom_encfuse_shape(int xy, int zs, int nw_override, int *nw, int *nblocks, size_t *row_cap);
 hipError_t gvom_launch_encfuse(hipStream_t s, const ScanParams &P, const FuseParams &F, const MapDesc &prev, int32_t *flink, uint32_t *hit,
-                               uint32_t *total, uint32_t *mh, int32_t *state, uint4 *crows, const uint32_t *stags,
+                               uint32_t *total, uint32_t *mh, int32_t *state, uint4 *crows, const uint32_t *stags, const uint32_t *htags,
                                int32_t *fstate, uint4 *frows, uint32_t *ftags, uint32_t *blockcounts, double *height,
                                double *inferred, uint32_t *counters, unsigned long long *host_flag, uint32_t seq);
 hipError_t gvom_launch_map2d(hipStream_t s, const Map2dParams &P, const int32_t *fstate, const uint32_t *ftags,
diff --git a/g-vom_amd/csrc/gvom_plan.h b/g-vom_amd/csrc/gvom_plan.h
--- /dev/null
+++ b/g-vom_amd/csrc/gvom_plan.h
@@ -0,0 +1,17 @@
+#ifndef GVOM_PLAN_H
+#define GVOM_PLAN_H
+
+struct HandlePlan {
+    bool eager;
+    bool htags;
+};
+
+inline HandlePlan gvom_plan_handle(bool sharded, int buffer_size, int xy, int zs)
+{
+    HandlePlan p;
+    p.eager = !sharded && buffer_size == 1 && xy % 16 == 0 && zs >= 4;
+    p.htags = !sharded;
+    return p;
+}
+
+#endif
diff --git a/g-vom_amd/csrc/gvom_trace.hip b/g-vom_amd/csrc/gvom_trace.hip
--- a/g-vom_amd/csrc/gvom_trace.hip
+++ b/g-vom_amd/csrc/gvom_trace.hip
@@ -121,7 +121,8 @@
 
 __device__ __forceinline__ void endpoint_commit(const ScanParams &P, int lane, long row, bool ingrid, uint32_t L, uint32_t A,
                                                 uint32_t mbits, uint32_t *hit, uint32_t *total, uint32_t *mh, int32_t *state,
-                                                uint32_t *tags, double *stat_sums, double *stat_base, uint32_t *stat_rowvox)
+                                                uint32_t *tags, uint32_t *htags, double *stat_sums, double *stat_base,
+                                                uint32_t *stat_rowvox)
 {
     const uint32_t key = ingrid ? A : (0xFFFFFF00u | (uint32_t)lane);
     const uint32_t leftk = (uint32_t)__builtin_amdgcn_update_dpp((int)~key, (int)key, 0x138 , 0xf, 0xf, false);
@@ -131,7 +132,9 @@
     if (ehead && !GVOM_DBG(P, 4)) {
         const uint32_t run = (uint32_t)__ffsll((long long)~((followers >> lane) >> 1));
         atomicAdd(&hit[A], run);
-        tags[(L / P.xy) * P.nseg + ((L % P.xy) >> 6)] = P.epoch;
+        const uint32_t tile = (L / P.xy) * P.nseg + ((L % P.xy) >> 6);
+        tags[tile] = P.epoch;
+        if (htags) htags[tile] = P.epoch;
         state[L] = (int32_t)row;
         if (stat_sums) {
             for (int m = 0; m < 10; ++m) { stat_sums[(size_t)row * 10 + m] = 0.0; stat_base[(size_t)row * GVOM_BASE_PITCH + m] = 0.0; }
@@ -332,7 +335,7 @@
 template <typename T, bool BIG>
 __device__ __forceinline__ void trace_item(const ScanParams &P, const ShardExchange &X, const T *__restrict__ in, long stride, long n,
                                            T *__restrict__ world, uint32_t *hit, uint32_t *total, uint32_t *mh, int32_t *state,
-                                           uint32_t *tags, uint32_t *counters, double *stat_sums, double *stat_base,
+                                           uint32_t *tags, uint32_t *htags, uint32_t *counters, double *stat_sums, double *stat_base,
                                            uint32_t *stat_rowvox, int row, long bundle, int lane, uint32_t *lck, uint32_t *lcc,
                                            size_t widx, const WalkConsts &C)
 {
@@ -396,7 +399,7 @@
                 }
             }
         }
-        endpoint_commit(P, lane, i, mine, E.L, E.A, E.mbits, hit, total, mh, state, tags, stat_sums, stat_base, stat_rowvox);
+        endpoint_commit(P, lane, i, mine, E.L, E.A, E.mbits, hit, total, mh, state, tags, htags, stat_sums, stat_base, stat_rowvox);
         if (P.ep_row >= 0) { TL_MARK(P, widx, 2); return; }
     }
     int seg = P.ep_row >= 0 ? row - (row > P.ep_row ? 1 : 0) : row;
@@ -447,8 +450,8 @@
 template <typename T, bool BIG, int WPB>
 __global__ __launch_bounds__(64 * WPB) __attribute__((amdgpu_waves_per_eu(8, 8))) void k_trace(
     const ScanParams P, const ShardExchange X, const T *__restrict__ in, long stride, long n, T *__restrict__ world,
-    uint32_t *hit, uint32_t *total, uint32_t *mh, int32_t *state, uint32_t *tags, uint32_t *counters, double *stat_sums,
-    double *stat_base, uint32_t *stat_rowvox)
+    uint32_t *hit, uint32_t *total, uint32_t *mh, int32_t *state, uint32_t *tags, uint32_t *htags, uint32_t *counters,
+    double *stat_sums, double *stat_base, uint32_t *stat_rowvox)
 {
     const int lane = threadIdx.x & (WAVE - 1);
     const int row = (int)blockIdx.y;
@@ -469,7 +472,7 @@
     WC.prof = (P.tl && P.prof_on && (widx & 63) == 0 && row != P.ep_row) ? P.tl + P.tl_words + 8 + (widx >> 6) * 128 : nullptr;
     WC.prof_n = 0;
 #endif
-    trace_item<T, BIG>(P, X, in, stride, n, world, hit, total, mh, state, tags, counters, stat_sums, stat_base, stat_rowvox,
+    trace_item<T, BIG>(P, X, in, stride, n, world, hit, total, mh, state, tags, htags, counters, stat_sums, stat_base, stat_rowvox,
                        row, bundle, lane, lck, lcc, widx, WC);
 }
 
@@ -580,19 +583,19 @@
         const uint32_t sx = L % (uint32_t)P.xy, rz = L / (uint32_t)P.xy;
         A = acc_idx((int)sx, (int)(rz / (uint32_t)P.zs), (int)(rz % (uint32_t)P.zs), P.zs, P.sxq);
     }
-    endpoint_commit(P, lane, row_base + (long)i, live, L, A, mbits, hit, total, mh, state, tags, stat_sums, stat_base, stat_rowvox);
+    endpoint_commit(P, lane, row_base + (long)i, live, L, A, mbits, hit, total, mh, state, tags, nullptr, stat_sums, stat_base, stat_rowvox);
 }
 
 hipError_t gvom_launch_trace(hipStream_t s, const ScanParams &P, const ShardExchange &X, int dtype, bool big_origin, const void *pts,
                              int64_t stride_elems, int64_t n, void *world, uint32_t *hit,
-                             uint32_t *total, uint32_t *mh, int32_t *state, uint32_t *tags,
+                             uint32_t *total, uint32_t *mh, int32_t *state, uint32_t *tags, uint32_t *htags,
                              uint32_t *counters, double *stat_sums, double *stat_base,
                              uint32_t *stat_rowvox)
 {
     if (n <= 0) return hipSuccess;
 #define TRACE_LAUNCH(TT, BB, WW)                                                                             \
     hipLaunchKernelGGL((k_trace<TT, BB, WW>), dim3((unsigned)((n + 64 * WW - 1) / (64 * WW)), (unsigned)P.nsegs + (P.ep_row >= 0 ? 1u : 0u) + ((unsigned)GVOM_DBG(P, 0xF00) >> 8)), dim3(64 * WW), 0, s, P, X, (const TT *)pts, \
-                       (long)stride_elems, (long)n, (TT *)world, hit, total, mh, state, tags, counters,     \
+                       (long)stride_elems, (long)n, (TT *)world, hit, total, mh, state, tags, htags, counters, \
                        stat_sums, stat_base, stat_rowvox)
     if (dtype == 0) { if (big_origin) TRACE_LAUNCH(float, true, 8); else TRACE_LAUNCH(float, false, 8); }
     else { if (big_origin) TRACE_LAUNCH(double, true, 8); else TRACE_LAUNCH(double, false, 8); }
```

Result: slower. 1284 M points/s (-3.4%).
